# baiyang4/D-LSG-Video-Caption

Hardware: AMD Instinct MI355X
Metric: clips/sec (train step, 26x(2048+4096) feats) (higher is better)
Workload: dtype f32; 1 GPU; vocab 1000, dropout on, tf eps 0.952, batch 64/GPU; MSVD-shaped 26x(2048+4096) + 16x2048 regions; train step; batch_per_gpu=64, global_batch=64, parallelism=dp1, launch=hipGraph replay, gemm_arithmetic=fp32

## Files before the change

d-lsg-video-caption_amd/csrc/decstep.hip:

```cpp
#include "common.hpp"
#include "dlsg.h"

using namespace dlsg;

namespace {

constexpr int DT = 1024;
constexpr int MAXW = 2048;
constexpr int MAXP = 72;

template <int V> struct Vec;
template <> struct Vec<4> { using T = float4; };
template <> struct Vec<1> { using T = float; };
template <int V> __device__ __forceinline__ void vload(float (&r)[V], const float* p) {
    if constexpr (V == 4) { const float4 t = *reinterpret_cast<const float4*>(p); r[0] = t.x; r[1] = t.y; r[2] = t.z; r[3] = t.w; }
    else r[0] = *p;
}
template <int V> __device__ __forceinline__ void vstore(float* p, const float (&r)[V]) {
    if constexpr (V == 4) *reinterpret_cast<float4*>(p) = make_float4(r[0], r[1], r[2], r[3]);
    else *p = r[0];
}

__device__ __forceinline__ void block_sum2(float& a, float& b, float* red) {
    a = wave_sum(a); b = wave_sum(b);
    const int lane = threadIdx.x & 63, w = threadIdx.x >> 6;
    __syncthreads();
    if (lane == 0) { red[w] = a; red[16 + w] = b; }
    __syncthreads();
    float ra = 0.f, rb = 0.f;
#pragma unroll
    for (int i = 0; i < DT / 64; ++i) { ra += red[i]; rb += red[16 + i]; }
    a = ra; b = rb;
}

template <int V>
__device__ __forceinline__ void cell_row(int b, int N, const float* slabs, int nslab, int64_t slab_stride, const float* addend,
                                         int64_t ldadd, const float* b_ih, const float* b_hh, const float* c_prev, float* c_out,
                                         float* h_out, float* gates, float p, uint32_t site, uint64_t seed, float* gb, float* hb) {
    float cpv[MAXW / DT];
#pragma unroll
    for (int i = 0; i < MAXW / DT; ++i) {
        const int j = threadIdx.x + i * DT;
        cpv[i] = (c_prev && j < N) ? c_prev[(int64_t)b * N + j] : 0.f;
    }
    for (int col = threadIdx.x * V; col < 4 * N; col += DT * V) {
        float acc[V], t[4][V];
#pragma unroll
        for (int e = 0; e < V; ++e) acc[e] = 0.f;
        const float* sp = slabs + (int64_t)b * 4 * N + col;
        int k = 0;
        for (; k + 4 <= nslab; k += 4) {
#pragma unroll
            for (int u = 0; u < 4; ++u) vload<V>(t[u], sp + (k + u) * slab_stride);
#pragma unroll
// ... 2 lines not shown
                for (int e = 0; e < V; ++e) acc[e] += t[u][e];
        }
        if (k < nslab) {
            const int rem = nslab - k;
#pragma unroll
            for (int u = 0; u < 3; ++u)
                if (u < rem) vload<V>(t[u], sp + (k + u) * slab_stride);
#pragma unroll
            for (int u = 0; u < 3; ++u)
                if (u < rem)
#pragma unroll
                    for (int e = 0; e < V; ++e) acc[e] += t[u][e];
        }
        if (addend) { vload<V>(t[0], addend + (int64_t)b * ldadd + col);
#pragma unroll
            for (int e = 0; e < V; ++e) acc[e] += t[0][e]; }
        if (b_ih) { vload<V>(t[1], b_ih + col);
#pragma unroll
            for (int e = 0; e < V; ++e) acc[e] += t[1][e]; }
        if (b_hh) { vload<V>(t[2], b_hh + col);
#pragma unroll
            for (int e = 0; e < V; ++e) acc[e] += t[2][e]; }
        const bool is_g = (col / N) == 2;
#pragma unroll
        for (int e = 0; e < V; ++e) acc[e] = is_g ? tanhf(acc[e]) : sigmoidf_(acc[e]);
        vstore<V>(gates + (int64_t)b * 4 * N + col, acc);
        vstore<V>(gb + col, acc);
    }
    __syncthreads();
#pragma unroll
    for (int i = 0; i < MAXW / DT; ++i) {
        const int j = threadIdx.x + i * DT;
        if (j >= N) break;
        const float cp = cpv[i];
        const float c = gb[N + j] * cp + gb[j] * gb[2 * N + j];
        float h = gb[3 * N + j] * tanhf(c);
        c_out[(int64_t)b * N + j] = c;
        if (p > 0.f) h *= drop_scale(seed, site, (uint64_t)b * N + j, p);
        h_out[(int64_t)b * N + j] = h;
        hb[j] = h;
    }
    __syncthreads();
}

__device__ __forceinline__ void ln_stats(const float* v, int n, float eps, float* red, float& mean, float& rstd) {
    float s = 0.f;
    for (int j = threadIdx.x; j < n; j += DT) s += v[j];
    mean = block_sum(s, red) / n;
    float q = 0.f;
    for (int j = threadIdx.x; j < n; j += DT) { const float d = v[j] - mean; q += d * d; }
    rstd = rsqrtf(block_sum(q, red) / n + eps);
}

template <int V>
__global__ __launch_bounds__(DT) void dec_mid_fwd_kernel(const dlsg_dec_mid_args a) {
    __shared__ __attribute__((aligned(16))) float gb[4 * MAXW];
    __shared__ __attribute__((aligned(16))) float hb[MAXW];
    __shared__ __attribute__((aligned(16))) float qb[MAXW];
    __shared__ float sc[2 * MAXP], wt[2 * MAXP];
    __shared__ float red[32];
    const int b = blockIdx.x;
    const int bk = a.kv_div > 1 ? b / a.kv_div : b;
    const int Q = a.Q, H = a.H, P = a.P, ns = a.nstream;
    const int lane = threadIdx.x & 63, w = threadIdx.x >> 6;
    const uint64_t seed = a.seed + (a.seed_ptr ? *a.seed_ptr : 0ull);

    cell_row<V>(b, Q, a.slabs, a.nslab, a.slab_stride, a.addend, a.ldadd, a.b_ih, a.b_hh, a.c_prev, a.c, a.h, a.gates, 0.f, 0,
                seed, gb, hb);
    float mean, rstd;
    ln_stats(hb, Q, a.eps, red, mean, rstd);
    if (threadIdx.x == 0) { a.st_q[2 * b] = mean; a.st_q[2 * b + 1] = rstd; }
    for (int j = threadIdx.x; j < Q; j += DT) {
        float v = (hb[j] - mean) * rstd * a.lnq_g[j] + a.lnq_b[j];
        if (a.p_q > 0.f) v *= drop_scale(seed, a.site_q, (uint64_t)b * Q + j, a.p_q);
        a.qcur[(int64_t)b * Q + j] = v;
        qb[j] = v;
    }
    __syncthreads();
    for (int d = w; d < ns * P; d += DT / 64) {
        const int s = d / P, p = d % P;
        const float* kp = a.Kp[s] + ((int64_t)bk * P + p) * Q;
        float acc = 0.f;
#pragma unroll 4
        for (int j = lane * V; j < Q; j += 64 * V) {
            float kv[V];
            vload<V>(kv, kp + j);
#pragma unroll
            for (int e = 0; e < V; ++e) acc += kv[e] * qb[j + e];
        }
        acc = wave_sum(acc);
        if (lane == 0) sc[s * MAXP + p] = acc * a.scale;
    }
    __syncthreads();
    if (threadIdx.x < ns * P) {
        const int s = threadIdx.x / P, p = threadIdx.x % P;
        float m = -INFINITY;
        for (int i = 0; i < P; ++i) m = fmaxf(m, sc[s * MAXP + i]);
        float l = 0.f;
        for (int i = 0; i < P; ++i) l += __expf(sc[s * MAXP + i] - m);
        const float wv = __expf(sc[s * MAXP + p] - m) / l;
        wt[s * MAXP + p] = wv;
        a.alpha[(int64_t)b * ns * P + s * P + p] = wv;
    }
    __syncthreads();
    float* cb = gb;
    for (int it = threadIdx.x * V; it < ns * H; it += DT * V) {
        const int s = it / H, j = it % H;
        const float* vp = a.Vp[s] + (int64_t)bk * P * H + j;
        float acc[V], t[4][V];
#pragma unroll
        for (int e = 0; e < V; ++e) acc[e] = 0.f;
        int p = 0;
        for (; p + 4 <= P; p += 4) {
#pragma unroll
            for (int u = 0; u < 4; ++u) vload<V>(t[u], vp + (int64_t)(p + u) * H);
#pragma unroll
            for (int u = 0; u < 4; ++u)
#pragma unroll
                for (int e = 0; e < V; ++e) acc[e] += wt[s * MAXP + p + u] * t[u][e];
        }
        for (; p < P; ++p) {
            vload<V>(t[0], vp + (int64_t)p * H);
#pragma unroll
            for (int e = 0; e < V; ++e) acc[e] += wt[s * MAXP + p] * t[0][e];
        }
        vstore<V>(a.cpre[s] + (int64_t)b * H + j, acc);
#pragma unroll
        for (int e = 0; e < V; ++e) acc[e] = tanhf(acc[e]);
        vstore<V>(cb + s * MAXW + j, acc);
    }
    __syncthreads();
    float s0 = 0.f, s1 = 0.f;
    for (int j = threadIdx.x; j < H; j += DT) { s0 += cb[j]; if (ns > 1) s1 += cb[MAXW + j]; }
    block_sum2(s0, s1, red);
    const float m0 = s0 / H, m1 = s1 / H;
    float q0 = 0.f, q1 = 0.f;
    for (int j = threadIdx.x; j < H; j += DT) {
        const float d0 = cb[j] - m0; q0 += d0 * d0;
        if (ns > 1) { const float d1 = cb[MAXW + j] - m1; q1 += d1 * d1; }
    }
    block_sum2(q0, q1, red);
    const float r0 = rsqrtf(q0 / H + a.eps), r1 = rsqrtf(q1 / H + a.eps);
    if (threadIdx.x == 0) {
        a.st_c[0][2 * b] = m0; a.st_c[0][2 * b + 1] = r0;
        if (ns > 1) { a.st_c[1][2 * b] = m1; a.st_c[1][2 * b + 1] = r1; }
    }
    for (int it = threadIdx.x; it < ns * H; it += DT) {
        const int s = it / H, j = it % H;
        float v = (cb[s * MAXW + j] - (s ? m1 : m0)) * (s ? r1 : r0) * a.lnc_g[s][j] + a.lnc_b[s][j];
        if (a.p_att[s] > 0.f) v *= drop_scale(seed, a.site_att[s], (uint64_t)b * H + j, a.p_att[s]);
        a.ctx[s][(int64_t)b * H + j] = v;
    }
}

template <int V>
__global__ __launch_bounds__(DT) void dec_tail_fwd_kernel(const dlsg_dec_tail_args a) {
    __shared__ __attribute__((aligned(16))) float gb[4 * MAXW];
    __shared__ __attribute__((aligned(16))) float hb[MAXW];
    __shared__ float red[32];
    const int b = blockIdx.x;
    const int D = a.D;
    const uint64_t seed = a.seed + (a.seed_ptr ? *a.seed_ptr : 0ull);
    constexpr int ND = MAXW / DT;
    float lg[ND], lb[ND];
#pragma unroll
    for (int i = 0; i < ND; ++i) {
        const int j = threadIdx.x + i * DT;
        lg[i] = j < D ? a.ln_g[j] : 0.f; lb[i] = j < D ? a.ln_b[j] : 0.f;
    }
    cell_row<V>(b, D, a.slabs, a.nslab, a.slab_stride, nullptr, 0, a.b_ih, a.b_hh, a.c_prev, a.c, a.hd, a.gates, a.p, a.site,
                seed, gb, hb);
    float mean, rstd;
    ln_stats(hb, D, a.eps, red, mean, rstd);
    if (threadIdx.x == 0) { a.st_l[2 * b] = mean; a.st_l[2 * b + 1] = rstd; }
    const bool sample = a.s_coins != nullptr && a.s_coins[a.s_t] == 0;
    float dv[ND];
#pragma unroll
    for (int i = 0; i < ND; ++i) {
        const int j = threadIdx.x + i * DT;
        dv[i] = 0.f;
        if (j >= D) break;
        dv[i] = tanhf((hb[j] - mean) * rstd * lg[i] + lb[i]);
        a.dout[(int64_t)b * D + j] = dv[i];
    }
    if (!sample) return;
    __syncthreads();
#pragma unroll
    for (int i = 0; i < ND; ++i) {
        const int j = threadIdx.x + i * DT;
        if (j < D) hb[j] = dv[i];
    }
    __syncthreads();
    __shared__ int s_bi[DT / 64];
    __shared__ int64_t s_chosen;
    const int lane = threadIdx.x & 63, w = threadIdx.x >> 6;
    float best = -INFINITY;
    int bidx = 0x7fffffff;
    constexpr int CU4 = 4;
    for (int v0 = w * CU4; v0 < a.s_V; v0 += (DT / 64) * CU4) {
        float acc[CU4];
#pragma unroll
        for (int u = 0; u < CU4; ++u) {
            acc[u] = 0.f;
            const int v = min(v0 + u, a.s_V - 1);
            const float* wr = a.s_W + (int64_t)v * D;
            if (V == 4) {
                for (int j = 4 * lane; j < D; j += 256) {
                    const f32x4 x = *reinterpret_cast<const f32x4*>(hb + j);
                    const f32x4 y = *reinterpret_cast<const f32x4*>(wr + j);
                    acc[u] += x[0] * y[0] + x[1] * y[1] + x[2] * y[2] + x[3] * y[3];
                }
            } else {
                for (int j = lane; j < D; j += 64) acc[u] += hb[j] * wr[j];
            }
        }
#pragma unroll
        for (int u = 0; u < CU4; ++u) {
            const int v = v0 + u;
            float s_ = wave_sum(acc[u]);
            if (a.s_b) s_ += a.s_b[min(v, a.s_V - 1)];
            if (v < a.s_V && (s_ > best || (s_ == best && v < bidx))) { best = s_; bidx = v; }
        }
    }
    if (lane == 0) { red[w] = best; s_bi[w] = bidx; }
    __syncthreads();
    if (threadIdx.x == 0) {
        for (int k = 1; k < DT / 64; ++k)
            if (red[k] > best || (red[k] == best && s_bi[k] < bidx)) { best = red[k]; bidx = s_bi[k]; }
        if (bidx == 0x7fffffff) bidx = 0;
        s_chosen = bidx;
        a.s_ids[b] = bidx;
    }
    __syncthreads();
    const int64_t id = s_chosen;
    for (int j = threadIdx.x; j < a.s_Wd; j += DT) {
        float e = a.s_E[id * a.s_Wd + j];
        if (a.s_p > 0.f) e *= drop_scale(seed, a.s_site, (uint64_t)(a.s_row0 + b) * a.s_Wd + j, a.s_p);
        a.s_we[(int64_t)b * a.s_ldwe + j] = e;
    }
}


template <int N>
__device__ __forceinline__ void block_sumN(float (&v)[N], float* red) {
#pragma unroll
    for (int i = 0; i < N; ++i) v[i] = wave_sum(v[i]);
    const int lane = threadIdx.x & 63, w = threadIdx.x >> 6;
    __syncthreads();
    if (lane == 0)
#pragma unroll
        for (int i = 0; i < N; ++i) red[16 * i + w] = v[i];
    __syncthreads();
#pragma unroll
    for (int i = 0; i < N; ++i) {
        float r = 0.f;
#pragma unroll
        for (int k = 0; k < DT / 64; ++k) r += red[16 * i + k];
        v[i] = r;
    }
}

template <int V>
__global__ __launch_bounds__(DT) void dec_mid_bwd_kernel(const dlsg_dec_mid_bwd_args a) {
    __shared__ __attribute__((aligned(16))) float dxb[3 * MAXW];
    __shared__ __attribute__((aligned(16))) float dcp[2 * MAXW];
    __shared__ __attribute__((aligned(16))) float dqb[2 * MAXW];
    __shared__ float dwb[2 * MAXP], dsb[2 * MAXP], wb[2 * MAXP];
    __shared__ float red[64];
    constexpr int IC = 2 * MAXW / DT, IQ = MAXW / DT;
    const int b = blockIdx.x;
    const int Q = a.Q, H = a.H, D = a.D, P = a.P, ns = a.nstream;
    const int NX = ns * H + Q, WT = NX + D;
    const int lane = threadIdx.x & 63, w = threadIdx.x >> 6;
    const uint64_t seed = a.seed + (a.seed_ptr ? *a.seed_ptr : 0ull);

    float yv[IC], xq[IQ], rec[IQ];
#pragma unroll
    for (int i = 0; i < IC; ++i) {
        const int it = threadIdx.x + i * DT;
        yv[i] = 0.f;
        if (it < ns * H) { const int s = it / H, j = it % H; yv[i] = a.cpre[s][(int64_t)b * H + j]; }
    }
#pragma unroll
    for (int i = 0; i < IQ; ++i) {
        const int j = threadIdx.x + i * DT;
        xq[i] = 0.f; rec[i] = 0.f;
        if (j < Q) {
            xq[i] = a.qh[(int64_t)b * Q + j];
            if (a.rec_slabs) {
                const float* rp = a.rec_slabs + (int64_t)b * a.rec_ld + j;
                int k = 0;
                for (; k + 4 <= a.rec_nslab; k += 4) {
                    const float t0 = rp[(int64_t)k * a.rec_slab_stride], t1 = rp[(int64_t)(k + 1) * a.rec_slab_stride],
                                t2 = rp[(int64_t)(k + 2) * a.rec_slab_stride], t3 = rp[(int64_t)(k + 3) * a.rec_slab_stride];
                    rec[i] += t0; rec[i] += t1; rec[i] += t2; rec[i] += t3;
                }
                for (; k < a.rec_nslab; ++k) rec[i] += rp[(int64_t)k * a.rec_slab_stride];
            }
        }
    }
    if (threadIdx.x < ns * P) {
        const int s = threadIdx.x / P, p = threadIdx.x % P;
        wb[s * MAXP + p] = a.alpha[(int64_t)b * ns * P + threadIdx.x];
    }
    const int ncol = a.write_rec ? WT : NX;
    for (int col = threadIdx.x * V; col < ncol; col += DT * V) {
        float acc[V], t[4][V];
#pragma unroll
        for (int e = 0; e < V; ++e) acc[e] = 0.f;
        const float* sp = a.slabs + (int64_t)b * WT + col;
        int k = 0;
        for (; k + 4 <= a.nslab; k += 4) {
#pragma unroll
            for (int u = 0; u < 4; ++u) vload<V>(t[u], sp + (k + u) * a.slab_stride);
#pragma unroll
            for (int u = 0; u < 4; ++u)
#pragma unroll
                for (int e = 0; e < V; ++e) acc[e] += t[u][e];
        }
        if (k < a.nslab) {
            const int rem = a.nslab - k;
#pragma unroll
            for (int u = 0; u < 3; ++u)
// ... 83 lines not shown
#pragma unroll
                for (int e = 0; e < V; ++e) acc[e] += dsb[s * MAXP + p + u] * t[u][e];
        }
        for (; p < P; ++p) {
            vload<V>(t[0], kp + (int64_t)p * Q);
#pragma unroll
            for (int e = 0; e < V; ++e) acc[e] += dsb[s * MAXP + p] * t[0][e];
        }
        vstore<V>(dqb + s * MAXW + j, acc);
    }
    __syncthreads();
    float gq[IQ], xhq[IQ];
    float s2[2] = {0.f, 0.f};
    const float meanq = a.st_q[2 * b], rstdq = a.st_q[2 * b + 1];
#pragma unroll
    for (int i = 0; i < IQ; ++i) {
        const int j = threadIdx.x + i * DT;
        gq[i] = 0.f; xhq[i] = 0.f;
        if (j < Q) {
            float g = dxb[ns * H + j] + dqb[j];
            if (ns > 1) g += dqb[MAXW + j];
            if (a.p_q > 0.f) g *= drop_scale(seed, a.site_q, (uint64_t)b * Q + j, a.p_q);
            xhq[i] = (xq[i] - meanq) * rstdq;
            float* pq = a.part_q + (int64_t)b * 2 * Q;
            pq[j] = g * xhq[i];
            pq[Q + j] = g;
            gq[i] = g * a.lnq_g[j];
            s2[0] += gq[i]; s2[1] += gq[i] * xhq[i];
        }
    }
    block_sumN<2>(s2, red);
    const float m1 = s2[0] / Q, m2 = s2[1] / Q;
#pragma unroll
    for (int i = 0; i < IQ; ++i) {
        const int j = threadIdx.x + i * DT;
        if (j < Q) {
            const float dh = rstdq * (gq[i] - m1 - xhq[i] * m2) + rec[i];
            const float* gp = a.gates + (int64_t)b * 4 * Q;
            const float ig = gp[j], fg = gp[Q + j], gg = gp[2 * Q + j], og = gp[3 * Q + j];
            const float c = a.c[(int64_t)b * Q + j];
            const float cp = a.c_prev ? a.c_prev[(int64_t)b * Q + j] : 0.f;
            const float tc = tanhf(c);
            const float dc = dh * og * (1.f - tc * tc) + a.dc[(int64_t)b * Q + j];
            float* dgp = a.dgates + (int64_t)b * 4 * Q;
            dgp[j] = dc * gg * ig * (1.f - ig);
            dgp[Q + j] = dc * cp * fg * (1.f - fg);
            dgp[2 * Q + j] = dc * ig * (1.f - gg * gg);
            dgp[3 * Q + j] = dh * tc * og * (1.f - og);
            a.dc[(int64_t)b * Q + j] = dc * fg;
        }
    }
}

constexpr int CG_PC = 8;
template <int V>
__global__ __launch_bounds__(256) void decatt_cache_grads_kernel(const dlsg_decatt_cache_grads_args a) {
    const int b = blockIdx.x, s = blockIdx.y >> 1, kind = blockIdx.y & 1;
    const int N = kind ? a.Q : a.H, P = a.P, nsP = a.nstream * a.P;
    const float* coef = (kind ? a.ds : a.alpha) + (int64_t)b * nsP + s * P;
    const float* src = (kind ? a.qcur : a.dcpre[s]) + (int64_t)b * N;
    float* dst = (kind ? a.dKp[s] : a.dVp[s]) + (int64_t)b * P * N;
    for (int p0 = 0; p0 < P; p0 += CG_PC)
        for (int j = threadIdx.x * V; j < N; j += 256 * V) {
            float acc[CG_PC][V];
#pragma unroll
            for (int p = 0; p < CG_PC; ++p)
#pragma unroll
                for (int e = 0; e < V; ++e) acc[p][e] = 0.f;
#pragma unroll 2
            for (int t = 0; t < a.L; ++t) {
                float x[V];
                vload<V>(x, src + (int64_t)t * a.B * N + j);
                const float* cf = coef + (int64_t)t * a.B * nsP + p0;
#pragma unroll
                for (int p = 0; p < CG_PC; ++p) {
                    const float cv = (p0 + p < P) ? cf[p] : 0.f;
#pragma unroll
                    for (int e = 0; e < V; ++e) acc[p][e] += cv * x[e];
                }
            }
#pragma unroll
            for (int p = 0; p < CG_PC; ++p)
                if (p0 + p < P) vstore<V>(dst + (int64_t)(p0 + p) * N + j, acc[p]);
        }
}

bool vec_ok(const void* p) { return (reinterpret_cast<uintptr_t>(p) & 15) == 0; }

}

extern "C" int dlsg_dec_mid_fwd(const dlsg_dec_mid_args* a, void* stream) {
    if (!a || a->Q < 1 || a->Q > MAXW || a->H < 1 || a->H > MAXW || a->P < 1 || a->P > MAXP || a->nstream < 1 || a->nstream > 2)
        return DLSG_EINVAL;
    if (a->B == 0) return DLSG_OK;
    bool v4 = a->Q % 4 == 0 && a->H % 4 == 0 && a->slab_stride % 4 == 0 && a->ldadd % 4 == 0 && vec_ok(a->slabs) &&
              vec_ok(a->addend) && vec_ok(a->b_ih) && vec_ok(a->b_hh) && vec_ok(a->gates);
    for (int s = 0; s < a->nstream; ++s) v4 = v4 && vec_ok(a->Kp[s]) && vec_ok(a->Vp[s]) && vec_ok(a->cpre[s]);
    hipLaunchKernelGGL(v4 ? dec_mid_fwd_kernel<4> : dec_mid_fwd_kernel<1>, dim3(a->B), dim3(DT), 0,
                       reinterpret_cast<hipStream_t>(stream), *a);
    DLSG_CHECK_LAUNCH();
    return DLSG_OK;
}
extern "C" int dlsg_dec_tail_fwd(const dlsg_dec_tail_args* a, void* stream) {
    if (!a || a->D < 1 || a->D > MAXW) return DLSG_EINVAL;
    if (a->B == 0) return DLSG_OK;
    if (a->s_coins && (!a->s_W || !a->s_E || !a->s_ids || !a->s_we || a->s_V < 1 || a->s_Wd < 1)) return DLSG_EINVAL;
    const bool v4 = a->D % 4 == 0 && a->slab_stride % 4 == 0 && vec_ok(a->slabs) && vec_ok(a->b_ih) && vec_ok(a->b_hh) &&
                    vec_ok(a->gates) && (!a->s_coins || vec_ok(a->s_W));
    hipLaunchKernelGGL(v4 ? dec_tail_fwd_kernel<4> : dec_tail_fwd_kernel<1>, dim3(a->B), dim3(DT), 0,
                       reinterpret_cast<hipStream_t>(stream), *a);
    DLSG_CHECK_LAUNCH();
    return DLSG_OK;
}
extern "C" int dlsg_dec_mid_bwd(const dlsg_dec_mid_bwd_args* a, void* stream) {
    if (!a || a->Q < 1 || a->Q > MAXW || a->H < 1 || a->H > MAXW || a->D < 0 || a->P < 1 || a->P > MAXP || a->nstream < 1 ||
        a->nstream > 2)
        return DLSG_EINVAL;
    if (a->B == 0) return DLSG_OK;
    bool v4 = a->Q % 4 == 0 && a->H % 4 == 0 && a->D % 4 == 0 && a->slab_stride % 4 == 0 && vec_ok(a->slabs) && vec_ok(a->dlh_rec);
    for (int s = 0; s < a->nstream; ++s) v4 = v4 && vec_ok(a->Kp[s]) && vec_ok(a->Vp[s]);
    hipLaunchKernelGGL(v4 ? dec_mid_bwd_kernel<4> : dec_mid_bwd_kernel<1>, dim3(a->B), dim3(DT), 0,
                       reinterpret_cast<hipStream_t>(stream), *a);
    DLSG_CHECK_LAUNCH();
    return DLSG_OK;
}
extern "C" int dlsg_decatt_cache_grads(const dlsg_decatt_cache_grads_args* a, void* stream) {
    if (!a || a->L < 0 || a->P < 1 || a->nstream < 1 || a->nstream > 2) return DLSG_EINVAL;
    if (a->B == 0) return DLSG_OK;
    bool v4 = a->Q % 4 == 0 && a->H % 4 == 0 && vec_ok(a->qcur);
    for (int s = 0; s < a->nstream; ++s) v4 = v4 && vec_ok(a->dcpre[s]) && vec_ok(a->dKp[s]) && vec_ok(a->dVp[s]);
    hipLaunchKernelGGL(v4 ? decatt_cache_grads_kernel<4> : decatt_cache_grads_kernel<1>, dim3(a->B, 2 * a->nstream), dim3(256), 0,
                       reinterpret_cast<hipStream_t>(stream), *a);
    DLSG_CHECK_LAUNCH();
    return DLSG_OK;
}
```

d-lsg-video-caption_amd/csrc/gemm.hip:

```cpp
#include <cstdlib>
#include <mutex>

#include "common.hpp"
#include "dlsg.h"

namespace {

constexpr int NT = 256;

template <int ROWS, bool T, int BK>
struct TileGeom {
    static constexpr int NV = ROWS * BK / 4 / NT;
    static constexpr int LD = T ? (ROWS + 4) : (BK + 4);
    static constexpr int ELEMS = T ? BK * (ROWS + 4) : ROWS * (BK + 4);
    static constexpr int KQ = BK / 4;
};

template <int ROWS, bool T, int BK>
__device__ __forceinline__ void load_tile_fast(const float* __restrict__ base, int64_t ld, int row0, int k0, int rmax,
                                               f32x4 (&regs)[TileGeom<ROWS, T, BK>::NV]) {
    constexpr int NV = TileGeom<ROWS, T, BK>::NV;
#pragma unroll
    for (int j = 0; j < NV; ++j) {
        const int f = threadIdx.x + NT * j;
        const float* ptr;
        if (!T) {
            const int gr = min(row0 + f / (BK / 4), rmax - 1);
            ptr = base + (int64_t)gr * ld + k0 + 4 * (f % (BK / 4));
        } else {
            ptr = base + (int64_t)(k0 + f / (ROWS / 4)) * ld + row0 + 4 * (f % (ROWS / 4));
        }
        regs[j] = *reinterpret_cast<const f32x4*>(ptr);
    }
}
template <int ROWS, bool T, int BK>
__device__ __forceinline__ void load_tile_slow(const float* __restrict__ base, int64_t ld, int row0, int k0, int rmax,
                                               int K, f32x4 (&regs)[TileGeom<ROWS, T, BK>::NV]) {
    constexpr int NV = TileGeom<ROWS, T, BK>::NV;
#pragma unroll
    for (int j = 0; j < NV; ++j) {
        const int f = threadIdx.x + NT * j;
        int gr, gk, nvalid;
        const float* ptr;
        if (!T) {
            const int row = f / (BK / 4), kq = f % (BK / 4);
            gr = row0 + row;
            gk = k0 + 4 * kq;
            ptr = base + (int64_t)gr * ld + gk;
            nvalid = (gr < rmax) ? min(max(K - gk, 0), 4) : 0;
        } else {
            const int k = f / (ROWS / 4), mq = f % (ROWS / 4);
            gk = k0 + k;
            gr = row0 + 4 * mq;
            ptr = base + (int64_t)gk * ld + gr;
            nvalid = (gk < K) ? min(max(rmax - gr, 0), 4) : 0;
        }
        f32x4 v = {0.f, 0.f, 0.f, 0.f};
// ... 300 lines not shown
#pragma unroll
        for (int mi = 0; mi < MI; ++mi) {
            const float* ap = ldsA + (r + 32 * mi) * SLD + 32 * w + 16 * h;
#pragma unroll
            for (int q = 0; q < 4; ++q) {
                const f32x4 v = *reinterpret_cast<const f32x4*>(ap + 4 * q);
                fa[mi][4 * q] = v[0]; fa[mi][4 * q + 1] = v[1]; fa[mi][4 * q + 2] = v[2]; fa[mi][4 * q + 3] = v[3];
            }
        }
        if (!BT) {
            const float* bp = ldsB + r * SLD + 32 * w + 16 * h;
#pragma unroll
            for (int q = 0; q < 4; ++q) {
                const f32x4 v = *reinterpret_cast<const f32x4*>(bp + 4 * q);
                bcur[4 * q] = v[0]; bcur[4 * q + 1] = v[1]; bcur[4 * q + 2] = v[2]; bcur[4 * q + 3] = v[3];
            }
        }
#pragma unroll
        for (int s2 = 0; s2 < 16; ++s2)
#pragma unroll
            for (int mi = 0; mi < MI; ++mi) acc[mi] = __builtin_amdgcn_mfma_f32_32x32x2f32(fa[mi][s2], bcur[s2], acc[mi], 0, 0, 0);
        __syncthreads();
    }
    float* red = lds;
#pragma unroll
    for (int mi = 0; mi < MI; ++mi)
#pragma unroll
        for (int e = 0; e < 16; ++e) red[((w * MI + mi) * 16 + e) * 64 + lane] = acc[mi][e];
    __syncthreads();
    const float* biasp = grp.bias ? grp.bias : p.bias;
    const bool accum = p.flags & DLSG_GEMM_ACCUM, use_bias = (p.flags & DLSG_GEMM_BIAS) && biasp != nullptr;
    const bool do_tanh = p.flags & DLSG_GEMM_TANH;
    if (col < N) {
        const float bv = use_bias ? biasp[col] : 0.f;
#pragma unroll
        for (int mi = 0; mi < MI; ++mi)
#pragma unroll
            for (int ee = 0; ee < 4; ++ee) {
                const int e = 4 * w + ee;
                const int row = 32 * mi + (e & 3) + 8 * (e >> 2) + 4 * h;
                if (row >= M) continue;
                float v = 0.f;
#pragma unroll
                for (int ww = 0; ww < 4; ++ww) v += red[((ww * MI + mi) * 16 + e) * 64 + lane];
                v = p.alpha * v + bv;
                float* cp = C + (int64_t)row * (grp.ldc ? grp.ldc : (int64_t)p.ldc) + col;
                if (accum) v += *cp;
                if (do_tanh) v = tanhf(v);
                *cp = v;
            }
    }
}

constexpr int S2_STAGE = 16;
constexpr int S2_DEPTH = 3;
constexpr int S2_B_BYTES = 32 * 64;
constexpr int s2_lds_bytes(int MI, int NJ) { return 4 * S2_DEPTH * (MI + NJ) * S2_B_BYTES; }

template <int VB>
__device__ __forceinline__ void s2_glds(const char* src, char* dst) {
#if defined(__HIP_DEVICE_COMPILE__)
    typedef __attribute__((address_space(3))) void* lp_t;
    typedef const __attribute__((address_space(1))) void* gp_t;
    __builtin_amdgcn_global_load_lds((gp_t)src, (lp_t)dst, 16, 0, 0);
#endif
}

template <int MI, int NJ, bool BT = false>
__global__ __launch_bounds__(NT) void skinny2_nt_kernel(const KArgs p) {
    constexpr int S2_A_BYTES = MI * S2_B_BYTES;
    constexpr int SLOT = S2_A_BYTES + NJ * S2_B_BYTES;
    extern __shared__ __attribute__((aligned(16))) char s2_lds[];
    if (p.skip_if && *p.skip_if) return;
    const int z = blockIdx.y;
    const int gi = z % p.ngroups, bi = z / p.ngroups;
    const dlsg_gemm_group grp = p.g[gi];
    const float* A = grp.A + (int64_t)bi * p.bsa;
    const float* B = grp.B + (int64_t)bi * p.bsb;
    float* C = grp.C + (int64_t)bi * p.bsc;
    const int K = grp.K, M = p.M, N = grp.N > 0 ? grp.N : p.N;
    const int n0 = blockIdx.x * 32 * NJ;
    if (n0 >= N) return;
    const int lane = threadIdx.x & 63, w = threadIdx.x >> 6;
    const int r = lane & 31, h = lane >> 5;
    char* ring = s2_lds + w * (S2_DEPTH * SLOT);

    const int rho = lane >> 2, sig = lane & 3;
    const float* srcA[2 * MI];
    const float* srcB[2 * NJ];
#pragma unroll
    for (int pc = 0; pc < 2 * MI; ++pc) {
        const int R = 16 * pc + rho;
        srcA[pc] = A + (int64_t)min(R, M - 1) * grp.lda + 4 * (sig ^ ((R >> 2) & 3));
    }
#pragma unroll
    for (int pc = 0; pc < 2 * NJ; ++pc) {
        if (!BT) {
            const int R = 16 * pc + rho;
            srcB[pc] = B + (int64_t)min(n0 + R, N - 1) * grp.ldb + 4 * (sig ^ ((R >> 2) & 3));
        } else {
            const int kr = 8 * (pc & 1) + (lane >> 3), c = n0 + 32 * (pc >> 1) + 4 * (lane & 7);
            srcB[pc] = B + (int64_t)kr * grp.ldb + min(c, N - 4);
        }
    }
    const int nst = (K + S2_STAGE - 1) / S2_STAGE;
    const int mine = (nst - w + 3) / 4;
    auto issue = [&](int i) {
        const int k0 = (4 * i + w) * S2_STAGE;
        char* slot = ring + (i % S2_DEPTH) * SLOT;
        const int koff = (k0 + S2_STAGE <= K) ? k0 : (K - S2_STAGE);
#pragma unroll
        for (int pc = 0; pc < 2 * MI; ++pc) s2_glds<16>(reinterpret_cast<const char*>(srcA[pc] + koff), slot + pc * 1024);
#pragma unroll
        for (int pc = 0; pc < 2 * NJ; ++pc)
            s2_glds<16>(reinterpret_cast<const char*>(BT ? srcB[pc] + (int64_t)koff * grp.ldb : srcB[pc] + koff), slot + S2_A_BYTES + pc * 1024);
    };

    f32x16 acc[MI][NJ];
#pragma unroll
    for (int i = 0; i < MI; ++i)
#pragma unroll
        for (int nj = 0; nj < NJ; ++nj)
#pragma unroll
            for (int e = 0; e < 16; ++e) acc[i][nj][e] = 0.f;

    int offA[MI][2], offB[NJ][2];
#pragma unroll
    for (int q = 0; q < 2; ++q) {
        const int ks = 2 * q + h;
#pragma unroll
        for (int mi = 0; mi < MI; ++mi) {
            const int R = 32 * mi + r;
            offA[mi][q] = (R >> 4) * 1024 + (R & 15) * 64 + ((ks ^ ((R >> 2) & 3)) * 16);
        }
#pragma unroll
        for (int nj = 0; nj < NJ; ++nj) {
            const int R = 32 * nj + r;
            offB[nj][q] = BT ? S2_A_BYTES + nj * 2048 + (4 * ks) * 128 + r * 4
                             : S2_A_BYTES + (R >> 4) * 1024 + (R & 15) * 64 + ((ks ^ ((R >> 2) & 3)) * 16);
        }
    }
    constexpr int PCS = 2 * MI + 2 * NJ;

    if (mine > 0) issue(0);
    if (mine > 1) issue(1);
    for (int i = 0; i < mine; ++i) {
        if (i + 2 < mine) {
            issue(i + 2);
            asm volatile("s_waitcnt vmcnt(%0)" ::"n"(2 * PCS) : "memory");
        } else if (i + 1 < mine) {
            asm volatile("s_waitcnt vmcnt(%0)" ::"n"(PCS) : "memory");
        } else {
            asm volatile("s_waitcnt vmcnt(0)" ::: "memory");
        }
        const char* slot = ring + (i % S2_DEPTH) * SLOT;
        const int k0 = (4 * i + w) * S2_STAGE;
        const bool part = k0 + S2_STAGE > K;
        const int kbase = part ? K - S2_STAGE : k0;
        f32x4 fa[MI][2], fb[NJ][2];
#pragma unroll
        for (int q = 0; q < 2; ++q) {
#pragma unroll
            for (int mi = 0; mi < MI; ++mi) fa[mi][q] = *reinterpret_cast<const f32x4*>(slot + offA[mi][q]);
#pragma unroll
            for (int nj = 0; nj < NJ; ++nj) {
                if (!BT) fb[nj][q] = *reinterpret_cast<const f32x4*>(slot + offB[nj][q]);
                else {
#pragma unroll
                    for (int j = 0; j < 4; ++j) fb[nj][q][j] = *reinterpret_cast<const float*>(slot + offB[nj][q] + j * 128);
                }
            }
        }
        if (part) {
#pragma unroll
            for (int q = 0; q < 2; ++q)
#pragma unroll
                for (int j = 0; j < 4; ++j) {
                    const int k = kbase + 4 * (2 * q + h) + j;
                    const bool keep = k >= k0 && k < K;
#pragma unroll
                    for (int mi = 0; mi < MI; ++mi) fa[mi][q][j] = keep ? fa[mi][q][j] : 0.f;
#pragma unroll
                    for (int nj = 0; nj < NJ; ++nj) fb[nj][q][j] = keep ? fb[nj][q][j] : 0.f;
                }
        }
#pragma unroll
        for (int q = 0; q < 2; ++q)
#pragma unroll
            for (int j = 0; j < 4; ++j)
#pragma unroll
                for (int nj = 0; nj < NJ; ++nj)
#pragma unroll
                    for (int mi = 0; mi < MI; ++mi)
                        acc[mi][nj] = __builtin_amdgcn_mfma_f32_32x32x2f32(fa[mi][q][j], fb[nj][q][j], acc[mi][nj], 0, 0, 0);
    }
    __syncthreads();
    float* red = reinterpret_cast<float*>(s2_lds);
#pragma unroll
    for (int mi = 0; mi < MI; ++mi)
#pragma unroll
        for (int nj = 0; nj < NJ; ++nj)
#pragma unroll
            for (int e = 0; e < 16; ++e) red[(((w * MI + mi) * NJ + nj) * 16 + e) * 64 + lane] = acc[mi][nj][e];
    __syncthreads();
    const float* biasp = grp.bias ? grp.bias : p.bias;
    const bool accum = p.flags & DLSG_GEMM_ACCUM, use_bias = (p.flags & DLSG_GEMM_BIAS) && biasp != nullptr;
    const bool do_tanh = p.flags & DLSG_GEMM_TANH;
#pragma unroll
    for (int nj = 0; nj < NJ; ++nj) {
        const int col = n0 + 32 * nj + r;
        if (col >= N) continue;
        const float bv = use_bias ? biasp[col] : 0.f;
#pragma unroll
        for (int mi = 0; mi < MI; ++mi)
#pragma unroll
            for (int ee = 0; ee < 4; ++ee) {
                const int e = 4 * w + ee;
                const int row = 32 * mi + (e & 3) + 8 * (e >> 2) + 4 * h;
                if (row >= M) continue;
                float v = 0.f;
#pragma unroll
                for (int ww = 0; ww < 4; ++ww) v += red[(((ww * MI + mi) * NJ + nj) * 16 + e) * 64 + lane];
                v = p.alpha * v + bv;
                float* cp = C + (int64_t)row * (grp.ldc ? grp.ldc : (int64_t)p.ldc) + col;
                if (accum) v += *cp;
                if (do_tanh) v = tanhf(v);
                *cp = v;
            }
    }
}

template <int MI>
int launch_skinny_mi(const dlsg_gemm_args* a, const KArgs& k, hipStream_t st) {
    dim3 grid((a->N + 31) / 32, a->ngroups * a->nbatch, 1), block(NT, 1, 1);
    static std::once_flag once;
    std::call_once(once, [] {
        (void)hipFuncSetAttribute(reinterpret_cast<const void*>(&skinny2_nt_kernel<MI, 1>), hipFuncAttributeMaxDynamicSharedMemorySize,
                                  s2_lds_bytes(MI, 1));
        (void)hipFuncSetAttribute(reinterpret_cast<const void*>(&skinny2_nt_kernel<MI, 2>), hipFuncAttributeMaxDynamicSharedMemorySize,
                                  s2_lds_bytes(MI, 2));
        (void)hipFuncSetAttribute(reinterpret_cast<const void*>(&skinny2_nt_kernel<MI, 1, true>), hipFuncAttributeMaxDynamicSharedMemorySize,
                                  s2_lds_bytes(MI, 1));
        (void)hipFuncSetAttribute(reinterpret_cast<const void*>(&skinny2_nt_kernel<MI, 2, true>), hipFuncAttributeMaxDynamicSharedMemorySize,
                                  s2_lds_bytes(MI, 2));
        (void)hipFuncSetAttribute(reinterpret_cast<const void*>(&skinny_kernel<false, MI>), hipFuncAttributeMaxDynamicSharedMemorySize,
                                  skinny_lds_bytes(MI));
        (void)hipFuncSetAttribute(reinterpret_cast<const void*>(&skinny_kernel<true, MI>), hipFuncAttributeMaxDynamicSharedMemorySize,
                                  skinny_lds_bytes(MI));
    });
    if (a->mode == 0) {
        bool ok = a->nbatch == 1;
        for (int i = 0; i < a->ngroups && ok; ++i) {
            const dlsg_gemm_group& g = a->g[i];
            ok = (g.K % 4 == 0) && g.K >= S2_STAGE && (g.lda % 4 == 0) && (g.ldb % 4 == 0) &&
                 ((reinterpret_cast<uintptr_t>(g.A) & 15) == 0) && ((reinterpret_cast<uintptr_t>(g.B) & 15) == 0);
        }
        if (ok) {
            const int wg64 = ((a->N + 63) / 64) * a->ngroups * a->nbatch;
            if (wg64 >= 224) {
                dim3 grid2((a->N + 63) / 64, a->ngroups * a->nbatch, 1);
                hipLaunchKernelGGL((skinny2_nt_kernel<MI, 2>), grid2, block, s2_lds_bytes(MI, 2), st, k);
            } else {
                hipLaunchKernelGGL((skinny2_nt_kernel<MI, 1>), grid, block, s2_lds_bytes(MI, 1), st, k);
            }
        } else {
            hipLaunchKernelGGL((skinny_kernel<false, MI>), grid, block, skinny_lds_bytes(MI), st, k);
        }
    } else {
        bool ok = a->nbatch == 1;
        for (int i = 0; i < a->ngroups && ok; ++i) {
            const dlsg_gemm_group& g = a->g[i];
            const int gn = g.N > 0 ? g.N : a->N;
            ok = (g.K % 4 == 0) && g.K >= S2_STAGE && (g.lda % 4 == 0) && (g.ldb % 4 == 0) && (gn % 4 == 0) && gn >= 4 &&
                 ((reinterpret_cast<uintptr_t>(g.A) & 15) == 0) && ((reinterpret_cast<uintptr_t>(g.B) & 15) == 0);
        }
        if (ok) {
            bool same_n = true;
            for (int i = 0; i < a->ngroups; ++i) same_n = same_n && (a->g[i].N == 0 || a->g[i].N == a->N);
            const int wg64 = ((a->N + 63) / 64) * a->ngroups * a->nbatch;
            if (wg64 >= 224 && same_n) {
                dim3 grid2((a->N + 63) / 64, a->ngroups * a->nbatch, 1);
                hipLaunchKernelGGL((skinny2_nt_kernel<MI, 2, true>), grid2, block, s2_lds_bytes(MI, 2), st, k);
            } else {
                hipLaunchKernelGGL((skinny2_nt_kernel<MI, 1, true>), grid, block, s2_lds_bytes(MI, 1), st, k);
            }
        } else {
            hipLaunchKernelGGL((skinny_kernel<true, MI>), grid, block, skinny_lds_bytes(MI), st, k);
        }
    }
    DLSG_CHECK_LAUNCH();
    return DLSG_OK;
}

int launch_skinny(const dlsg_gemm_args* a, hipStream_t st) {
    KArgs k;
    k.M = a->M; k.N = a->N; k.ldc = a->ldc; k.ngroups = a->ngroups; k.flags = a->flags;
    k.bsa = a->bsa; k.bsb = a->bsb; k.bsc = a->bsc; k.alpha = a->alpha; k.bias = a->bias; k.skip_if = a->skip_if;
    for (int i = 0; i < a->ngroups; ++i) k.g[i] = a->g[i];
    return a->M <= 64 ? launch_skinny_mi<2>(a, k, st) : launch_skinny_mi<4>(a, k, st);
}

template <int BM, int BN, int BK>
int launch(const dlsg_gemm_args* a, hipStream_t st) {
    KArgs k;
    k.M = a->M; k.N = a->N; k.ldc = a->ldc; k.ngroups = a->ngroups; k.flags = a->flags;
    k.bsa = a->bsa; k.bsb = a->bsb; k.bsc = a->bsc; k.alpha = a->alpha; k.bias = a->bias; k.skip_if = a->skip_if;
    for (int i = 0; i < a->ngroups; ++i) k.g[i] = a->g[i];
    const int tiles = ((a->M + BM - 1) / BM) * ((a->N + BN - 1) / BN);
    dim3 grid(tiles, a->ngroups * a->nbatch, 1), block(NT, 1, 1);
    switch (a->mode) {
        case 0:
            if constexpr (BM == 128) hipLaunchKernelGGL((gemm_kernel_w3<BM, BN, false, false, BK>), grid, block, 0, st, k);
            else hipLaunchKernelGGL((gemm_kernel<BM, BN, false, false, BK>), grid, block, 0, st, k);
            break;
        case 1:
            if constexpr (BM == 128) hipLaunchKernelGGL((gemm_kernel_w3<BM, BN, false, true, BK>), grid, block, 0, st, k);
            else hipLaunchKernelGGL((gemm_kernel<BM, BN, false, true, BK>), grid, block, 0, st, k);
            break;
        case 2:
            if constexpr (BM == 128) hipLaunchKernelGGL((gemm_kernel_w3<BM, BN, true, true, BK>), grid, block, 0, st, k);
            else hipLaunchKernelGGL((gemm_kernel<BM, BN, true, true, BK>), grid, block, 0, st, k);
            break;
        default: return DLSG_EINVAL;
    }
    DLSG_CHECK_LAUNCH();
    return DLSG_OK;
}
// ... 124 lines not shown
```

d-lsg-video-caption_amd/csrc/rowops.hip:

```cpp
#include "common.hpp"
#include "dlsg.h"

using namespace dlsg;

namespace {

constexpr int LN_THREADS = 256;
constexpr int LN_MAXPT = 8;

struct RowLnPack { dlsg_rowln_args s[DLSG_ROWLN_MAXMULTI]; };
struct RowLnBwdPack { dlsg_rowln_bwd_args s[DLSG_ROWLN_MAXMULTI]; };

__global__ __launch_bounds__(LN_THREADS) void rowln_fwd_kernel(const RowLnPack pk) {
    __shared__ float red[16];
    const dlsg_rowln_args& a = pk.s[blockIdx.y];
    const int n = a.n;
    const uint64_t seed = a.seed + (a.seed_ptr ? *a.seed_ptr : 0ull);
    float gam[LN_MAXPT], bet[LN_MAXPT];
#pragma unroll
    for (int i = 0; i < LN_MAXPT; ++i) {
        const int j = threadIdx.x + i * LN_THREADS;
        gam[i] = j < n ? a.gamma[j] : 0.f; bet[i] = j < n ? a.beta[j] : 0.f;
    }
    for (int row = blockIdx.x; row < a.rows; row += gridDim.x) {
// ... 310 lines not shown
struct PwFwdSet { dlsg_lstm_pw_args a[2]; };
struct PwBwdSet { dlsg_lstm_pw_bwd_args a[2]; };

__global__ __launch_bounds__(256) void lstm_pw_fwd_kernel(const PwFwdSet set) {
    const dlsg_lstm_pw_args& a = set.a[blockIdx.z];
    const int j = blockIdx.x * blockDim.x + threadIdx.x;
    const int b = blockIdx.y;
    if (j >= a.H) return;
    const int H = a.H;
    float pre[4] = {0.f, 0.f, 0.f, 0.f};
    const float* sp = a.slabs + (int64_t)b * 4 * H + j;
    int k = 0;
    for (; k + 2 <= a.nslab; k += 2) {
        float t[2][4];
#pragma unroll
        for (int u = 0; u < 2; ++u)
#pragma unroll
            for (int g = 0; g < 4; ++g) t[u][g] = sp[(k + u) * a.slab_stride + g * H];
#pragma unroll
        for (int u = 0; u < 2; ++u)
#pragma unroll
            for (int g = 0; g < 4; ++g) pre[g] += t[u][g];
    }
    if (k < a.nslab) {
#pragma unroll
        for (int g = 0; g < 4; ++g) pre[g] += sp[k * a.slab_stride + g * H];
    }
#pragma unroll
    for (int g = 0; g < 4; ++g) {
        const int col = g * H + j;
        float s = pre[g];
        if (a.addend) s += a.addend[(int64_t)b * a.ldadd + col];
        if (a.b_ih) s += a.b_ih[col];
        if (a.b_hh) s += a.b_hh[col];
        pre[g] = s;
    }
    const float ig = sigmoidf_(pre[0]), fg = sigmoidf_(pre[1]), gg = tanhf(pre[2]), og = sigmoidf_(pre[3]);
    const float cp = a.c_prev ? a.c_prev[(int64_t)b * a.ldcp + j] : 0.f;
    const float c = fg * cp + ig * gg;
    const float h = og * tanhf(c);
    a.c[(int64_t)b * a.ldc_ + j] = c;
    if (a.h) a.h[(int64_t)b * a.ldh + j] = h;
    if (a.h2) {
        float h2 = h;
        if (a.p > 0.f) h2 *= drop_scale(a.seed + (a.seed_ptr ? *a.seed_ptr : 0ull), a.site, (uint64_t)b * H + j, a.p);
        a.h2[(int64_t)b * a.ldh2 + j] = h2;
    }
    if (a.gates) {
        float* gp = a.gates + (int64_t)b * a.ldg;
        gp[j] = ig; gp[H + j] = fg; gp[2 * H + j] = gg; gp[3 * H + j] = og;
    }
}

__global__ __launch_bounds__(256) void lstm_pw_bwd_kernel(const PwBwdSet set) {
    const dlsg_lstm_pw_bwd_args& a = set.a[blockIdx.z];
    const int j = blockIdx.x * blockDim.x + threadIdx.x;
    const int b = blockIdx.y;
    if (j >= a.H) return;
    const int H = a.H;
    const float* gp = a.gates + (int64_t)b * a.ldg;
    const float ig = gp[j], fg = gp[H + j], gg = gp[2 * H + j], og = gp[3 * H + j];
    const float c = a.c[(int64_t)b * a.ldc_ + j];
    const float cp = a.c_prev ? a.c_prev[(int64_t)b * a.ldcp + j] : 0.f;
    float dh = a.dh ? a.dh[(int64_t)b * a.lddh + j] : 0.f;
    if (a.dh2 || a.dh3 || a.dh4) {
        float d2 = a.dh2 ? a.dh2[(int64_t)b * a.lddh2 + j] : 0.f;
        if (a.dh3) d2 += a.dh3[(int64_t)b * a.lddh3 + j];
        if (a.dh4) {
            const int ns4 = a.dh4_nslab > 1 ? a.dh4_nslab : 1;
            const float* hp = a.dh4 + (int64_t)b * a.lddh4 + j;
            int k = 0;
            for (; k + 4 <= ns4; k += 4) {
                const float t0 = hp[(int64_t)k * a.dh4_slab_stride], t1 = hp[(int64_t)(k + 1) * a.dh4_slab_stride],
                            t2 = hp[(int64_t)(k + 2) * a.dh4_slab_stride], t3 = hp[(int64_t)(k + 3) * a.dh4_slab_stride];
                d2 += t0; d2 += t1; d2 += t2; d2 += t3;
            }
            for (; k < ns4; ++k) d2 += hp[(int64_t)k * a.dh4_slab_stride];
        }
        if (a.p > 0.f) d2 *= drop_scale(a.seed + (a.seed_ptr ? *a.seed_ptr : 0ull), a.site, (uint64_t)b * H + j, a.p);
        dh += d2;
    }
    const float tc = tanhf(c);
    float dc = dh * og * (1.f - tc * tc);
    if (a.dc_next) dc += a.dc_next[(int64_t)b * a.lddcn + j];
    float* dgp = a.dgates + (int64_t)b * a.lddg;
    dgp[j] = dc * gg * ig * (1.f - ig);
    dgp[H + j] = dc * cp * fg * (1.f - fg);
    dgp[2 * H + j] = dc * ig * (1.f - gg * gg);
    dgp[3 * H + j] = dh * tc * og * (1.f - og);
    if (a.dc_prev) a.dc_prev[(int64_t)b * a.lddcp + j] = dc * fg;
}

__global__ void mean_rows_fwd_kernel(const float* __restrict__ x, float* __restrict__ out, int64_t ldo, int P, int H) {
    const int b = blockIdx.y;
    const int h = blockIdx.x * blockDim.x + threadIdx.x;
    if (h >= H) return;
    float s = 0.f;
    for (int p = 0; p < P; ++p) s += x[((int64_t)b * P + p) * H + h];
    out[(int64_t)b * ldo + h] = s / P;
}
__global__ void mean_rows_bwd_kernel(const float* __restrict__ dout, int64_t lddo, float* __restrict__ dx, int P, int H,
                                     int accum) {
    const int b = blockIdx.y;
    const int h = blockIdx.x * blockDim.x + threadIdx.x;
    if (h >= H) return;
    const float g = dout[(int64_t)b * lddo + h] / P;
    for (int p = 0; p < P; ++p) {
        float* d = dx + ((int64_t)b * P + p) * H + h;
        *d = accum ? *d + g : g;
    }
}

__global__ void embed_fwd_kernel(const float* __restrict__ E, const int64_t* __restrict__ ids, float* __restrict__ out,
                                 int64_t ldo, int W, float p, uint64_t seed, uint32_t site, int64_t row0, const uint64_t* seed_ptr) {
    if (seed_ptr) seed += *seed_ptr;
    const int r = blockIdx.x;
    const int64_t id = ids[r];
    for (int j = threadIdx.x; j < W; j += blockDim.x) {
        float v = E[id * W + j];
        if (p > 0.f) v *= drop_scale(seed, site, (uint64_t)(row0 + r) * W + j, p);
// ... 592 lines not shown
        if (d[i].out_b && !d[i].dup && (d[i].split < 0 || d[i].split > d[i].n)) return DLSG_EINVAL;
        pk.d[i] = d[i];
        maxn = d[i].n > maxn ? d[i].n : maxn;
    }
    hipLaunchKernelGGL(colsum_multi_kernel, dim3((maxn + 63) / 64, count), dim3(1024), 0, ST(stream), pk);
    DLSG_CHECK_LAUNCH();
    return DLSG_OK;
}
extern "C" int64_t dlsg_colsum_ws_floats(int rows, int n) {
    const int chunks = colsum_chunks(rows);
    return chunks > 1 ? (int64_t)chunks * n : 0;
}
extern "C" int dlsg_colsum(const float* part, int64_t ld, int rows, int n, float* out, int accum, float* ws, void* stream) {
    return colsum_launch(part, ld, rows, n, out, nullptr, n, 0, accum, ws, stream);
}
extern "C" int dlsg_colsum2(const float* part, int64_t ld, int rows, int n, float* out_a, float* out_b, int split, int dup,
                            int accum, float* ws, void* stream) {
    if (!out_b || (!dup && (split < 0 || split > n))) return DLSG_EINVAL;
    return colsum_launch(part, ld, rows, n, out_a, out_b, dup ? n : split, dup ? 1 : 0, accum, ws, stream);
}
extern "C" int dlsg_softmax_fwd(const float* x, const float* mask, float* y, int64_t outer, int n, int inner, void* stream) {
    const int64_t lines = outer * inner;
    if (lines == 0) return DLSG_OK;
    hipLaunchKernelGGL(softmax_fwd_kernel, dim3((unsigned)((lines + 3) / 4)), dim3(256), 0, ST(stream), x, mask, y, outer, n,
                       inner);
    DLSG_CHECK_LAUNCH();
    return DLSG_OK;
}
extern "C" int dlsg_softmax_bwd(const float* y, const float* dy, float* dx, int64_t outer, int n, int inner, void* stream) {
    const int64_t lines = outer * inner;
    if (lines == 0) return DLSG_OK;
    hipLaunchKernelGGL(softmax_bwd_kernel, dim3((unsigned)((lines + 3) / 4)), dim3(256), 0, ST(stream), y, dy, dx, outer, n,
                       inner);
    DLSG_CHECK_LAUNCH();
    return DLSG_OK;
}
extern "C" int dlsg_lstm_pw_fwd_n(const dlsg_lstm_pw_args* a, int count, void* stream) {
    if (!a || count < 1 || count > 2 || a[0].H < 1) return DLSG_EINVAL;
    if (count == 2 && (a[1].H != a[0].H || a[1].B != a[0].B)) return DLSG_EINVAL;
    if (a[0].B == 0) return DLSG_OK;
    PwFwdSet set;
    for (int i = 0; i < 2; ++i) set.a[i] = a[i < count ? i : 0];
    hipLaunchKernelGGL(lstm_pw_fwd_kernel, dim3((a[0].H + 255) / 256, a[0].B, count), dim3(256), 0, ST(stream), set);
    DLSG_CHECK_LAUNCH();
    return DLSG_OK;
}
extern "C" int dlsg_lstm_pw_fwd(const dlsg_lstm_pw_args* a, void* stream) { return dlsg_lstm_pw_fwd_n(a, 1, stream); }
extern "C" int dlsg_lstm_pw_bwd_n(const dlsg_lstm_pw_bwd_args* a, int count, void* stream) {
    if (!a || count < 1 || count > 2 || a[0].H < 1) return DLSG_EINVAL;
    if (count == 2 && (a[1].H != a[0].H || a[1].B != a[0].B)) return DLSG_EINVAL;
    if (a[0].B == 0) return DLSG_OK;
    PwBwdSet set;
    for (int i = 0; i < 2; ++i) set.a[i] = a[i < count ? i : 0];
    hipLaunchKernelGGL(lstm_pw_bwd_kernel, dim3((a[0].H + 255) / 256, a[0].B, count), dim3(256), 0, ST(stream), set);
    DLSG_CHECK_LAUNCH();
    return DLSG_OK;
}
extern "C" int dlsg_lstm_pw_bwd(const dlsg_lstm_pw_bwd_args* a, void* stream) { return dlsg_lstm_pw_bwd_n(a, 1, stream); }
extern "C" int dlsg_mean_rows_fwd(const float* x, float* out, int64_t ldo, int B, int P, int H, void* stream) {
    if (B == 0) return DLSG_OK;
    hipLaunchKernelGGL(mean_rows_fwd_kernel, dim3((H + 255) / 256, B), dim3(256), 0, ST(stream), x, out, ldo, P, H);
    DLSG_CHECK_LAUNCH();
    return DLSG_OK;
}
extern "C" int dlsg_mean_rows_bwd(const float* dout, int64_t lddo, float* dx, int B, int P, int H, int accum, void* stream) {
    if (B == 0) return DLSG_OK;
    hipLaunchKernelGGL(mean_rows_bwd_kernel, dim3((H + 255) / 256, B), dim3(256), 0, ST(stream), dout, lddo, dx, P, H, accum);
    DLSG_CHECK_LAUNCH();
    return DLSG_OK;
}
extern "C" int dlsg_embed_fwd(const float* E, const int64_t* ids, float* out, int64_t ldo, int rows, int W, float p,
                              uint64_t seed, uint32_t site, int64_t row0, const uint64_t* seed_ptr, void* stream) {
    if (rows == 0) return DLSG_OK;
    hipLaunchKernelGGL(embed_fwd_kernel, dim3(rows), dim3(128), 0, ST(stream), E, ids, out, ldo, W, p, seed, site, row0, seed_ptr);
    DLSG_CHECK_LAUNCH();
    return DLSG_OK;
}
extern "C" int dlsg_embed_bwd(const float* dout, int64_t lddo, const int64_t* ids, float* dE, int rows, int W, float p,
                              uint64_t seed, uint32_t site, int64_t row0, const uint64_t* seed_ptr, void* stream) {
    if (rows == 0) return DLSG_OK;
    const int threads = W >= 1024 ? 1024 : (W + 63) / 64 * 64;
    hipLaunchKernelGGL(embed_bwd_kernel, dim3(rows), dim3(threads), 0, ST(stream), dout, lddo, ids, dE, rows, W, p, seed, site, row0,
                       seed_ptr);
    DLSG_CHECK_LAUNCH();
    return DLSG_OK;
}
extern "C" int dlsg_select_embed(const float* logits, int64_t ld, int V, const int64_t* captions, int L, int t,
                                 const int32_t* coins, const float* E, int64_t* ids_out, float* out, int64_t ldo, int rows, int W,
                                 float p, uint64_t seed, uint32_t site, int64_t row0, const uint64_t* seed_ptr, int prefilled,
                                 void* stream) {
    if (rows == 0) return DLSG_OK;
    hipLaunchKernelGGL(select_embed_kernel, dim3(rows), dim3(256), 0, ST(stream), logits, ld, V, captions, L, t, coins, E, ids_out,
                       out, ldo, W, p, seed, site, row0, seed_ptr, prefilled);
    DLSG_CHECK_LAUNCH();
    return DLSG_OK;
}
extern "C" int dlsg_sample_embed(const float* logits, int64_t ld, int V, float temperature, const float* E, int64_t* ids_out, float* out,
                                 int64_t ldo, int W, float* logp, int64_t* lens, int t, int64_t end_id, int rows, float p, uint64_t seed,
                                 uint32_t site_word, uint32_t site_sample, int64_t row0, const uint64_t* seed_ptr, void* stream) {
    if (rows == 0) return DLSG_OK;
    if (V < 1 || W < 0 || !(temperature >= 0.f)) return DLSG_EINVAL;
    hipLaunchKernelGGL(sample_embed_kernel, dim3(rows), dim3(256), 0, ST(stream), logits, ld, V, temperature, E, ids_out, out, ldo, W,
                       logp, lens, t, end_id, p, seed, site_word, site_sample, row0, seed_ptr);
    DLSG_CHECK_LAUNCH();
    return DLSG_OK;
}
extern "C" int dlsg_argmax(const float* logits, int64_t ld, int64_t* ids, int rows, int V, void* stream) {
    if (rows == 0) return DLSG_OK;
    hipLaunchKernelGGL(argmax_kernel, dim3(rows), dim3(256), 0, ST(stream), logits, ld, ids, V);
    DLSG_CHECK_LAUNCH();
    return DLSG_OK;
// ... 98 lines not shown
```

d-lsg-video-caption_amd/dlsg_amd/engine.py:

```python
import math

import torch

from .hip import GEMM_NT, GEMM_NN, GEMM_TN, F_ACCUM, F_TANH, F_BF16X3, F_FORCE128

V_SK = 7

SITE_PSL_OBJ, SITE_PSL_MOT, SITE_LSTM, SITE_PE, SITE_SA, SITE_WORD, SITE_QUERY, SITE_ATT1, SITE_ATT2, SITE_LANG = range(1, 11)
STEP_SITE = 64
SITE_SAMPLE = 11


def _empty(ref, *shape, dtype=torch.float32):
    return torch.empty(*shape, dtype=dtype, device=ref.device)


def _zeros(ref, *shape, dtype=torch.float32):
    return torch.zeros(*shape, dtype=dtype, device=ref.device)


def _ksplit_bounds(K, nsplit, align=32):
    nsplit = max(1, min(nsplit, K // 512))
    step = ((K + nsplit - 1) // nsplit + align - 1) // align * align
    out, k = [], 0
# ... 70 lines not shown
            ops.gemm(GEMM_TN, [(dy, x, gout)], flags=_accum_flag(ops, gout))
    if deep and getattr(ops, 'stream_k', False) and all(ops.gemm(GEMM_TN, [it], flags=F_ACCUM, plan_only=True) == V_SK for it in deep):
        parts = {0: [], F_ACCUM: []}
        for it in deep:
            parts[_accum_flag(ops, it[2])].append(it)
        for fl, part in parts.items():
            for i0 in range(0, len(part), 16):
                ops.gemm(GEMM_TN, part[i0:i0 + 16], flags=fl)
        return
    by_shape = {}
    for it in deep:
        by_shape.setdefault((it[0].shape, it[1].shape), []).append(it)
    ks = DEEP_TN_CHUNKS
    per_launch = max(1, min(2, 16 // ks))
    for grp in by_shape.values():
        for i0 in range(0, len(grp), per_launch):
            part = grp[i0:i0 + per_launch]
            rows = part[0][0].shape[0]
            step = ((rows + ks - 1) // ks + 31) // 32 * 32
            bounds = [(k, min(rows, k + step)) for k in range(0, rows, step)]
            assert len(bounds) * len(part) <= 16
            slabs = [_empty(ref, len(bounds), gout.shape[0], gout.shape[1]) for _, _, gout in part]
            ops.gemm(GEMM_TN, [(dy[k0:k1], x[k0:k1], sl[i]) for (dy, x, _), sl in zip(part, slabs)
                               for i, (k0, k1) in enumerate(bounds)])
            for (_, _, gout), sl in zip(part, slabs):
                ops.slab_reduce(sl, gout, flags=_accum_always(ops, gout))


def _accum_flag_peek(ops, gout):
    seen = getattr(ops, 'grad_written', None)
    if seen is None or (gout.data_ptr(), tuple(gout.shape), tuple(gout.stride())) in seen:
        return F_ACCUM
    return 0


def gemm_nn_multi(ops, dy, Ws, out, ref):
    M, Nn = dy.shape
    widths = [W.shape[1] for W in Ws]
    tot = sum(widths)
    assert out.shape[1] == tot
    ns = _nsplit_for(M, tot, 1)
    ns = max(1, min(ns, 16 // len(Ws)))
    bounds = _bwd_bounds(Nn, M, ns)
    slabs = _empty(ref, len(bounds), M, tot)
    groups, c0 = [], 0
    for W, wd in zip(Ws, widths):
        for i, (k0, k1) in enumerate(bounds):
            groups.append((dy[:, k0:k1], W[k0:k1, :], slabs[i][:, c0:c0 + wd]))
        c0 += wd
    ops.gemm(GEMM_NN, groups)
    ops.slab_reduce(slabs, out)


def gemm_nn_multi_slabs(ops, dy, Ws, width, ref):
    M, Nn = dy.shape
    widths = [W.shape[1] for W in Ws]
    tot = sum(widths)
    assert tot <= width
    ns = _nsplit_for(M, tot, 1)
    ns = max(1, min(ns, 16 // len(Ws)))
    bounds = _bwd_bounds(Nn, M, ns)
    if M <= SKINNY_M and len(set(widths)) > 1:
        wmin = min(widths)
        if all(wd % wmin == 0 for wd in widths) and (tot // wmin) * len(bounds) <= 16:
            Ws = [W[:, c:c + wmin] for W, wd in zip(Ws, widths) for c in range(0, wd, wmin)]
            widths = [wmin] * len(Ws)
    slabs = _empty(ref, len(bounds), M, width)
    groups, c0 = [], 0
    for W, wd in zip(Ws, widths):
        for i, (k0, k1) in enumerate(bounds):
            groups.append((dy[:, k0:k1], W[k0:k1, :], slabs[i][:, c0:c0 + wd]))
        c0 += wd
    ops.gemm(GEMM_NN, groups)
    return slabs


def tn_grouped(ops, items, defer=None):
    if defer is not None:
        defer.extend(items)
        return
    by_m = {}
    for dy, x, gout in items:
        by_m.setdefault((dy.shape[1], dy.shape[0]), []).append((dy, x, gout))
    for grp in by_m.values():
        waves, seen = [[]], [set()]
        for it in grp:
            key = (it[2].data_ptr(), tuple(it[2].shape))
            for w_, sn in zip(waves, seen):
                if key not in sn and len(w_) < 16:
                    w_.append(it); sn.add(key)
                    break
            else:
                waves.append([it]); seen.append({key})
        for w_ in waves:
            first = [it for it in w_ if _accum_flag_peek(ops, it[2]) == 0]
            rest = [it for it in w_ if _accum_flag_peek(ops, it[2]) != 0]
            for it in first:
                _accum_flag(ops, it[2])
            if first:
                ops.gemm(GEMM_TN, first, flags=0)
            if rest:
                ops.gemm(GEMM_TN, rest, flags=F_ACCUM)


def gemm_bucketed(ops, mode, groups, flags=0):
    by_m = {}
    for g in groups:
        by_m.setdefault(g[2].shape[-2], []).append(g)
    for grp in by_m.values():
        for i in range(0, len(grp), 16):
            ops.gemm(mode, grp[i:i + 16], flags=flags)


def lin(ops, x, W, out, bias=None, tanh=False, accum=False, skip_if=None):
    ops.gemm(GEMM_NT, [(x, W, out)], flags=(F_TANH if tanh else 0) | (F_ACCUM if accum else 0), bias=bias, skip_if=skip_if)


class Grads(object):

    def __init__(self, named_params, arena, offsets):
        self.arena, self.offsets = arena, offsets
        self.views = {}
        for name, p in named_params:
            o = offsets[name]
            self.views[name] = arena[o:o + p.numel()].view(p.shape)
# ... 558 lines not shown


class DecPlan(object):

    def __init__(self, dec, n_global):
        self.H, self.W = dec.visual_hidden_size, dec.word_size
        self.Q, self.D = dec.query_hidden_size, dec.decode_hidden_size
        self.G = n_global
        self.ns = 2 if dec.multi_modal else 1
        self.q_lang = (0, self.D)
        self.q_glob = (self.D, self.D + self.G)
        self.q_word = (self.D + self.G, self.D + self.G + self.W)
        self.l_ctx = [(i * self.H, (i + 1) * self.H) for i in range(self.ns)]
        self.l_q = (self.ns * self.H, self.ns * self.H + self.Q)


def _att_modules(dec):
    return [dec.context_att] + ([dec.context_att_2] if dec.multi_modal else [])


def dec_prepare(ops, dec, mems, sv, training, seed):
    s = sv['dec'] = {}
    gsrc = sv['dec_gsrc']
    ref = mems[0]
    B = ref.shape[0]
    H = dec.visual_hidden_size
    plan = DecPlan(dec, H * len(gsrc))
    Q = plan.Q
    if sv.get('step_feats') is not None:
        gfeat = sv['step_feats']
        assert gfeat.shape == (B, plan.G), (tuple(gfeat.shape), (B, plan.G))
    else:
        gfeat = _empty(ref, B, plan.G)
        for i, g in enumerate(gsrc):
            ops.mean_rows_fwd(g, gfeat[:, i * H:(i + 1) * H])
    Wq = dec.query_lstm.weight_ih
    gq = _empty(ref, B, 4 * Q)
    lin(ops, gfeat, Wq[:, plan.q_glob[0]:plan.q_glob[1]], gq)
    atts = _att_modules(dec)
    m2s = [mem.reshape(mem.shape[0] * mem.shape[1], H) for mem in mems]
    Kc = [_empty(ref, m2.shape[0], H) for m2 in m2s]
    Vc = [_empty(ref, m2.shape[0], H) for m2 in m2s]
    kps = [_empty(ref, m2.shape[0], Q) for m2 in m2s]
    vps = [_empty(ref, m2.shape[0], H) for m2 in m2s]
    gemm_bucketed(ops, GEMM_NT, [g for att, m2, K, V in zip(atts, m2s, Kc, Vc) for g in ((m2, att.K.weight, K), (m2, att.V.weight, V))])
    gemm_bucketed(ops, GEMM_NN, [(K, att.Q.weight, kp) for att, K, kp in zip(atts, Kc, kps)])
    gemm_bucketed(ops, GEMM_NT, [(V, att.output_layer[0].weight, vp) for att, V, vp in zip(atts, Vc, vps)])
    Kp = [kp.view(mem.shape[0], mem.shape[1], Q) for kp, mem in zip(kps, mems)]
    Vp = [vp.view(mem.shape[0], mem.shape[1], H) for vp, mem in zip(vps, mems)]
    s.update(plan=plan, gfeat=gfeat, gq=gq, K=Kc, V=Vc, Kp=Kp, Vp=Vp, mems=mems)
    return s


def dec_step(ops, dec, s, t, ref, training, seed, B, word_dropout=True, sample=None):
    plan = s['plan']
    H, Q, D = plan.H, plan.Q, plan.D
    ql, ll = dec.query_lstm, dec.lang_lstm
    pd = dec.p_drop if training else 0.0
    site = STEP_SITE * (t + 1)
    segs = [(s['WE'][t], ql.weight_ih[:, plan.q_word[0]:plan.q_word[1]])]
    if t > 0 or s.get('warm', False):
        segs += [(s['LHP'][t], ql.weight_ih[:, plan.q_lang[0]:plan.q_lang[1]]), (s['QH'][t], ql.weight_hh)]
    slabs = seg_gemm_nt(ops, segs, B, 4 * Q, ref)
    ns = plan.ns
    lnq = dec.query_lstm_layernorm
    atts = _att_modules(dec)
    ops.dec_mid_fwd(slabs, s['gq'], ql.bias_ih, ql.bias_hh, s['QC'][t], s['QC'][t + 1], s['QH'][t + 1], s['GQ'][t],
                    (lnq.weight, lnq.bias), s['QCUR'][t], s['ST_Q'][t], pd, site + SITE_QUERY, s['Kp'], s['Vp'],
                    [(a.output_layer[2].weight, a.output_layer[2].bias) for a in atts],
                    [s['CPRE'][i][t] for i in range(ns)], [s['CTX'][i][t] for i in range(ns)],
                    [s['ST_C'][i][t] for i in range(ns)], s['ALPHA'][t],
                    [a.dropout if training else 0.0 for a in atts], [site + SITE_ATT1 + i for i in range(ns)],
                    1.0 / math.sqrt(H), seed=seed, **({'kv_div': s['kv_div']} if s.get('kv_div', 1) > 1 else {}))
    segs = [(s['CTX'][i][t], ll.weight_ih[:, plan.l_ctx[i][0]:plan.l_ctx[i][1]]) for i in range(ns)]
    segs.append((s['QCUR'][t], ll.weight_ih[:, plan.l_q[0]:plan.l_q[1]]))
    if t > 0 or s.get('warm', False):
        segs.append((s['LHP'][t], ll.weight_hh))
    slabs = seg_gemm_nt(ops, segs, B, 4 * D, ref)
    lnl = dec.lang_lstm_layernorm
    ops.dec_tail_fwd(slabs, ll.bias_ih, ll.bias_hh, s['LC'][t], s['LC'][t + 1], s['LHP'][t + 1], s['GL'][t],
                     (lnl.weight, lnl.bias), s['DOUT'][t], s['ST_L'][t], pd, site + SITE_LANG, seed=seed,
                     **({'sample': sample} if sample is not None else {}))


def plan_D(s):
    return s['plan'].D


def dec_logits(ops, dec, s, t0, t1, skip_if=None):
    plan = s['plan']
    D = plan.D
    B = s['LHP'].shape[1]
    V = dec.vocab_size
    n = (t1 - t0) * B
    lin(ops, s['DOUT'][t0:t1].view(n, D), dec.word_restore.weight, s['LOGITS'][t0:t1].view(n, V), dec.word_restore.bias,
        skip_if=skip_if)


def dec_alloc(dec, s, ref, B, L):
    plan = s['plan']
    H, W, Q, D, ns = plan.H, plan.W, plan.Q, plan.D, plan.ns
    V = dec.vocab_size
    P = s['Kp'][0].shape[1]
    zst = _zeros(ref, (L + 1) * B * (2 * D + 2 * Q))
    o = 0
    for key, wd in (('LHP', D), ('QH', Q), ('QC', Q), ('LC', D)):
        s[key] = zst[o:o + (L + 1) * B * wd].view(L + 1, B, wd)
        o += (L + 1) * B * wd
    s['WE'] = _empty(ref, L + 1, B, W)
    s['IDS'] = _zeros(ref, L + 1, B, dtype=torch.int64)
    s['QCUR'] = _empty(ref, L, B, Q)
    s['ST_Q'] = _empty(ref, L, B, 2)
    s['CPRE'] = [_empty(ref, L, B, H) for _ in range(ns)]
    s['CTX'] = [_empty(ref, L, B, H) for _ in range(ns)]
    s['ST_C'] = [_empty(ref, L, B, 2) for _ in range(ns)]
    s['GQ'] = _empty(ref, L, B, 4 * Q)
    s['GL'] = _empty(ref, L, B, 4 * D)
    s['ALPHA'] = _empty(ref, L, B, ns * P)
    s['DOUT'] = _empty(ref, L, B, D)
    s['ST_L'] = _empty(ref, L, B, 2)
    s['LOGITS'] = _empty(ref, L, B, V)


def dec_fwd(ops, dec, mems, sv, captions, L, coins, training, seed, dev_coins=None):
    s = dec_prepare(ops, dec, mems, sv, training, seed)
    ref = mems[0]
    B = ref.shape[0]
    dec_alloc(dec, s, ref, B, L)
    E = dec.word_embed.weight
    pw = dec.p_drop if training else 0.0
    ids = s['IDS']
    ids[0].fill_(dec.vocab('<start>'))
    s['pw'] = pw
    if dev_coins is not None:
        ops.embed_fwd(E, ids[0], s['WE'][0], p=pw, seed=seed, site=SITE_WORD, row0=0)
        pre = captions is not None and L > 1
        if pre:
            ids[1:L].copy_(captions[:, :L - 1].t())
            ops.embed_fwd(E, ids[1:L].reshape(-1), s['WE'][1:L].view((L - 1) * B, -1), p=pw, seed=seed, site=SITE_WORD, row0=B)
        fused_sample = pre and getattr(ops, 'dec_tail_sample_supported', None) is not None and \
            ops.dec_tail_sample_supported(dec.vocab_size, plan_D(s))
        for t in range(L):
            if fused_sample and t + 1 < L:
                dec_step(ops, dec, s, t, ref, training, seed, B,
                         sample=dict(coins=dev_coins, t=t, W=dec.word_restore.weight, b=dec.word_restore.bias, E=E, ids_out=ids[t + 1],
                                     we_out=s['WE'][t + 1], p=pw, site=SITE_WORD, row0=(t + 1) * B))
                continue
            dec_step(ops, dec, s, t, ref, training, seed, B)
            if t + 1 < L:
                dec_logits(ops, dec, s, t, t + 1, skip_if=dev_coins[t:t + 1])
                ops.select_embed(s['LOGITS'][t], captions, t, dev_coins, E, ids[t + 1], s['WE'][t + 1], p=pw, seed=seed,
                                 site=SITE_WORD, row0=(t + 1) * B, prefilled=pre)
        dec_logits(ops, dec, s, 0, L)
        return s
    if captions is not None:
        tf_steps = [i for i in range(L) if coins[i]]
        for i in tf_steps:
            ids[i + 1].copy_(captions[:, i])
    ops.embed_fwd(E, ids.view(-1), s['WE'].view((L + 1) * B, -1), p=pw, seed=seed, site=SITE_WORD)
    for t in range(L):
        dec_step(ops, dec, s, t, ref, training, seed, B)
        if not coins[t]:
            dec_logits(ops, dec, s, t, t + 1)
            ops.argmax(s['LOGITS'][t], ids[t + 1])
            ops.embed_fwd(E, ids[t + 1], s['WE'][t + 1], p=pw, seed=seed, site=SITE_WORD, row0=(t + 1) * B)
    if any(coins[t] for t in range(L)):
        dec_logits(ops, dec, s, 0, L)
    return s


def dec_sample(ops, dec, mems, sv, L, training, seed, temperature):
    s = dec_prepare(ops, dec, mems, sv, training, seed)
    ref = mems[0]
    B = ref.shape[0]
    dec_alloc(dec, s, ref, B, L)
    E = dec.word_embed.weight
    pw = dec.p_drop if training else 0.0
    ids = s['IDS']
    ids[0].fill_(dec.vocab('<start>'))
    s['pw'] = pw
    s['LOGP'] = _empty(ref, L, B)
    s['LENS'] = torch.full((B,), L, dtype=torch.int64, device=ref.device)
    end = dec.vocab('<end>')
    ops.embed_fwd(E, ids[0], s['WE'][0], p=pw, seed=seed, site=SITE_WORD, row0=0)
    for t in range(L):
        dec_step(ops, dec, s, t, ref, training, seed, B)
        dec_logits(ops, dec, s, t, t + 1)
        ops.sample_embed(s['LOGITS'][t], E, ids[t + 1], s['WE'][t + 1], s['LOGP'][t], s['LENS'], t, end, temperature=temperature,
                         p=pw, seed=seed, site=SITE_WORD, site_sample=SITE_SAMPLE, row0=(t + 1) * B)
    return s


def dec_bwd(ops, dec, sv, G, dlogits_tm, seed, training, dalpha_tm=None):
    s = sv['dec']
    plan = s['plan']
    H, W, Q, D, ns = plan.H, plan.W, plan.Q, plan.D, plan.ns
    L, B, V = dlogits_tm.shape
    ref = dlogits_tm
    ql, ll = dec.query_lstm, dec.lang_lstm
    pd = dec.p_drop if training else 0.0
    n = L * B
    dl2 = dlogits_tm.view(n, V)
    tn_grouped(ops, [(dl2, s['DOUT'].view(n, D), G['decoder.word_restore.weight'])], sv.get('tn_defer'))
    ops.colsum(dl2, G['decoder.word_restore.bias'], accum=True)
    ddout = _empty(ref, n, D)
    k32 = V // 32 * 32
    if V - k32 and k32 >= 4096 and getattr(ops, 'stream_k', False):
        ops.gemm(GEMM_NN, [(dl2[:, :k32], dec.word_restore.weight[:k32], ddout)])
        ops.gemm(GEMM_NN, [(dl2[:, k32:], dec.word_restore.weight[k32:], ddout)], flags=F_ACCUM)
    else:
        ops.gemm(GEMM_NN, [(dl2, dec.word_restore.weight, ddout)])
    lnl = dec.lang_lstm_layernorm
    nb = ops.rowln_bwd_nblk(n)
    part = _empty(ref, nb, 2, D)
    dLHo = _empty(ref, L, B, D)
    ops.rowln_bwd(ddout, s['LHP'][1:].view(n, D), lnl.weight, lnl.bias, dLHo.view(n, D), stats=s['ST_L'].view(n, 2),
                  post_tanh=1, dgb_part=part)
    ln_grads(ops, part, G, 'decoder.lang_lstm_layernorm', D)

    dGQ = _empty(ref, L, B, 4 * Q)
    dGL = _empty(ref, L, B, 4 * D)
    dQC = _zeros(ref, B, Q)
    dLC = _zeros(ref, B, D)
    dLHrec = _empty(ref, B, D)
    P = s['Kp'][0].shape[1]
    dCPRE = [_empty(ref, L, B, H) for _ in range(ns)]
    dS = _empty(ref, L, B, ns * P)
    atts = _att_modules(dec)
    part_q = _empty(ref, L, B, 2, Q)
    part_c = [_empty(ref, L, B, 2, H) for _ in range(ns)]
    lnq = dec.query_lstm_layernorm
    lnc_g = [att.output_layer[2].weight for att in atts]
    p_att = [att.dropout if training else 0.0 for att in atts]
    scale = 1.0 / math.sqrt(H)
    Wl_in = ll.weight_ih
    Wq_rec = [ql.weight_hh, ql.weight_ih[:, plan.q_lang[0]:plan.q_lang[1]]]
    wx = ns * H + Q + D
    ql_slabs = None
    for t in range(L - 1, -1, -1):
        site = STEP_SITE * (t + 1)
        rec = t < L - 1
        ops.lstm_pw_bwd(s['GL'][t], s['LC'][t + 1], dGL[t], B, D, c_prev=s['LC'][t], dh2=dLHo[t],
                        dh3=dLHrec if rec else None, dh4=ql_slabs[:, :, Q:] if rec else None, dc_next=dLC, dc_prev=dLC,
                        p=pd, site=site + SITE_LANG, seed=seed)
        xl_slabs = gemm_nn_multi_slabs(ops, dGL[t], [Wl_in, ll.weight_hh] if t > 0 else [Wl_in], wx, ref)
        ops.dec_mid_bwd(xl_slabs, dLHrec if t > 0 else None, [s['CPRE'][i][t] for i in range(ns)],
                        [s['ST_C'][i][t] for i in range(ns)], lnc_g, [part_c[i][t] for i in range(ns)],
                        [dCPRE[i][t] for i in range(ns)], p_att, [site + SITE_ATT1 + i for i in range(ns)], s['Kp'], s['Vp'],
                        s['ALPHA'][t], dalpha_tm[t] if dalpha_tm is not None else None, dS[t], s['QH'][t + 1], s['ST_Q'][t],
                        lnq.weight, part_q[t], pd, site + SITE_QUERY, ql_slabs[:, :, :Q] if rec else None, s['GQ'][t],
                        s['QC'][t + 1], s['QC'][t], dQC, dGQ[t], scale, seed=seed)
        if t > 0:
            ql_slabs = gemm_nn_multi_slabs(ops, dGQ[t], Wq_rec, Q + D, ref)
    dKp = [torch.empty_like(k) for k in s['Kp']]
    dVp = [torch.empty_like(v) for v in s['Vp']]
    ops.decatt_cache_grads(s['ALPHA'], dS, s['QCUR'], dCPRE, dKp, dVp)
    ln_grads(ops, part_q.view(L * B, 2, Q), G, 'decoder.query_lstm_layernorm', Q)
    att_names = ['decoder.context_att', 'decoder.context_att_2']
    for i in range(ns):
        ln_grads(ops, part_c[i].view(L * B, 2, H), G, att_names[i] + '.output_layer.2', H)
    dgq2, dgl2 = dGQ.view(n, 4 * Q), dGL.view(n, 4 * D)
    Gq_ih, Gl_ih = G['decoder.query_lstm.weight_ih'], G['decoder.lang_lstm.weight_ih']
    dgq_sum = _empty(ref, B, 4 * Q)
    ops.slab_reduce(dGQ, dgq_sum)
    lhp, qh = s['LHP'][:L].view(n, D), s['QH'][:L].view(n, Q)
    tn_grouped(ops, [(dgq2, lhp, Gq_ih[:, plan.q_lang[0]:plan.q_lang[1]]),
                     (dgq2, s['WE'][:L].view(n, W), Gq_ih[:, plan.q_word[0]:plan.q_word[1]]),
                     (dgq2, qh, G['decoder.query_lstm.weight_hh'])] +
               [(dgl2, s['CTX'][i].view(n, H), Gl_ih[:, plan.l_ctx[i][0]:plan.l_ctx[i][1]]) for i in range(ns)] +
               [(dgl2, s['QCUR'].view(n, Q), Gl_ih[:, plan.l_q[0]:plan.l_q[1]]),
                (dgl2, lhp, G['decoder.lang_lstm.weight_hh'])], sv.get('tn_defer'))
    gq_glob = Gq_ih[:, plan.q_glob[0]:plan.q_glob[1]]
    ops.gemm(GEMM_TN, [(dgq_sum, s['gfeat'], gq_glob)], flags=_accum_always(ops, gq_glob))
    ops.colsum2(dgq2, G['decoder.query_lstm.bias_ih'], G['decoder.query_lstm.bias_hh'], accum=True)
    ops.colsum2(dgl2, G['decoder.lang_lstm.bias_ih'], G['decoder.lang_lstm.bias_hh'], accum=True)
    dWE = _empty(ref, n, W)
    Wword = ql.weight_ih[:, plan.q_word[0]:plan.q_word[1]]
    if n >= 512 and 4 * Q >= 2048:
        kb = [(k, min(4 * Q, k + 1024)) for k in range(0, 4 * Q, 1024)]
        sl = _empty(ref, len(kb), n, W)
        ops.gemm(GEMM_NN, [(dgq2[:, k0:k1], Wword[k0:k1], sl[i]) for i, (k0, k1) in enumerate(kb)])
        ops.slab_reduce(sl, dWE)
    else:
        ops.gemm(GEMM_NN, [(dgq2, Wword, dWE)])
    ops.embed_bwd(dWE, s['IDS'][:L].view(-1), G['decoder.word_embed.weight'], p=s['pw'], seed=seed, site=SITE_WORD)
    dgfeat = _empty(ref, B, plan.G)
    gemm_nn_split(ops, dgq_sum, ql.weight_ih[:, plan.q_glob[0]:plan.q_glob[1]], dgfeat, ref)
    m2s = [mem.reshape(mem.shape[0] * mem.shape[1], H) for mem in s['mems']]
    dkps = [dKp[i].view(m2s[i].shape[0], Q) for i in range(ns)]
    dvps = [dVp[i].view(m2s[i].shape[0], H) for i in range(ns)]
    dKs = [_empty(ref, m2.shape[0], H) for m2 in m2s]
    dVs = [_empty(ref, m2.shape[0], H) for m2 in m2s]
    dms = [_empty(ref, m2.shape[0], H) for m2 in m2s]
    R = range(ns)
    tn_grouped(ops, [g for i in R for g in ((s['K'][i], dkps[i], G[att_names[i] + '.Q.weight']),
                                            (dvps[i], s['V'][i], G[att_names[i] + '.output_layer.0.weight']))], sv.get('tn_defer'))
    gemm_bucketed(ops, GEMM_NT, [(dkps[i], atts[i].Q.weight, dKs[i]) for i in R])
    gemm_bucketed(ops, GEMM_NN, [(dvps[i], atts[i].output_layer[0].weight, dVs[i]) for i in R])
    tn_grouped(ops, [g for i in R for g in ((dKs[i], m2s[i], G[att_names[i] + '.K.weight']),
                                            (dVs[i], m2s[i], G[att_names[i] + '.V.weight']))], sv.get('tn_defer'))
    gemm_bucketed(ops, GEMM_NN, [(dKs[i], atts[i].K.weight, dms[i]) for i in R])
    gemm_bucketed(ops, GEMM_NN, [(dVs[i], atts[i].V.weight, dms[i]) for i in R], flags=F_ACCUM)
    dmems = [dms[i].view(s['mems'][i].shape) for i in R]
    return dmems, dgfeat
# ... 1 lines not shown
```

d-lsg-video-caption_amd/dlsg_amd/hip.py:

```python
import ctypes as C
import os

import torch

from . import abi

_HERE = os.path.dirname(os.path.abspath(__file__))
LIB_PATH = os.path.join(_HERE, 'libdlsg_hip.so')

_D = abi.defines
ABI_VERSION = _D['DLSG_ABI_VERSION']
MAXG = _D['DLSG_GEMM_MAXG']
GEMM_NT, GEMM_NN, GEMM_TN = _D['DLSG_GEMM_NT'], _D['DLSG_GEMM_NN'], _D['DLSG_GEMM_TN']
F_ACCUM, F_BIAS, F_TANH = _D['DLSG_GEMM_ACCUM'], _D['DLSG_GEMM_BIAS'], _D['DLSG_GEMM_TANH']
F_FORCE64, F_FORCE128, F_TILE256, F_BF16X3 = (_D['DLSG_GEMM_' + n] for n in ('FORCE64', 'FORCE128', 'TILE256', 'BF16X3'))
F_SK, F_NOSK, F_SK_BM128, F_SK_BM256, F_SK_BN128, F_SK_NOXMAP = (_D['DLSG_GEMM_' + n] for n in (
    'SK', 'NOSK', 'SK_BM128', 'SK_BM256', 'SK_BN128', 'SK_NOXMAP'))
F_SK_GIVEAWAY = _D['DLSG_GEMM_SK_GIVEAWAY']

i64, u32, u64, f32 = C.c_int64, C.c_uint32, C.c_uint64, C.c_float


def load_library(path=LIB_PATH):
    if not os.path.exists(path):
# ... 94 lines not shown
                med = ms[len(ms) // 2] if len(ms) % 2 else 0.5 * (ms[len(ms) // 2 - 1] + ms[len(ms) // 2])
                shapes[shp]['ms_total'] = med * len(ms)
            out[key] = dict(launches=len(rec), ms_total=sum(d['ms_total'] for d in shapes.values()),
                            work_total=float(sum(r[2] for r in rec)), shapes=shapes)
        return out

    @staticmethod
    def _stream():
        return C.c_void_p(torch.cuda.current_stream().cuda_stream)

    launches = 0

    def _check(self, rc, what):
        self.launches += 1
        if rc != 0:
            raise RuntimeError('%s failed with code %d' % (what, rc))

    stream_k = True
    sk_cu_budget = 0

    _gemm_ws = {}
    _capture_streams = {}

    @classmethod
    def capture_stream(cls, dev):
        dev = torch.device(dev)
        idx = dev.index if dev.index is not None else torch.cuda.current_device()
        st = cls._capture_streams.get(idx)
        if st is None:
            st = cls._capture_streams[idx] = torch.cuda.Stream(device=idx)
        return st

    def _gemm_workspace(self, dev):
        key = (dev.index, torch.cuda.current_stream(dev).cuda_stream)
        ws = HipOps._gemm_ws.get(key)
        if ws is None:
            n = int(self.lib.dlsg_gemm_ws_bytes())
            if n <= 0:
                raise RuntimeError('dlsg_gemm_ws_bytes() failed: no device?')
            if torch.cuda.is_current_stream_capturing():
                return None
            ws = HipOps._gemm_ws[key] = torch.zeros((n + 3) // 4, dtype=torch.float32, device=dev)
        return ws

    def device_cus(self):
        n = int(self.lib.dlsg_gemm_ws_bytes())
        return max(0, (n - 16384) // (2 * 256 * 256 * 4))

    def comm_rehearsal(self, view, workgroups, passes):
        self._check(self.lib.dlsg_comm_rehearsal(_p(view), i64(view.numel()), int(workgroups), int(passes), self._stream()),
                    'dlsg_comm_rehearsal')

    def gemm(self, mode, groups, alpha=1.0, flags=0, bias=None, skip_if=None, plan_only=False):
        a = abi.dlsg_gemm_args()
        A0, B0, C0 = groups[0][:3]
        batched = A0.dim() == 3
        if batched:
            nb = C0.size(0)
            a.bsa, a.bsb, a.bsc = A0.stride(0), B0.stride(0), C0.stride(0)
        else:
            nb = 1
            a.bsa = a.bsb = a.bsc = 0
        M = C0.shape[-2]
        N = max(g[2].shape[-1] for g in groups)
        a.mode, a.M, a.N, a.ldc = mode, M, N, C0.stride(-2)
        a.ngroups, a.nbatch, a.alpha = len(groups), nb, alpha
        gbias = any(len(g) > 3 and g[3] is not None for g in groups)
        a.flags = flags | self.extra_flags | (F_BIAS if (bias is not None or gbias) else 0)
        a.bias = _p(bias)
        a.skip_if = _p(skip_if)
        if (self.stream_k or (flags & F_SK)) and not ((flags | self.extra_flags) & F_NOSK):
            ws = self._gemm_workspace(C0.device)
            if ws is not None:
                a.ws, a.ws_bytes = _p(ws), ws.numel() * 4
                a.cu_budget = int(self.sk_cu_budget)
        assert len(groups) <= MAXG
        for i, grp_ in enumerate(groups):
            A, B, Cc = grp_[:3]
            Ng = Cc.shape[-1]
            if mode == GEMM_TN:
                K = A.shape[-2]
                assert A.shape[-1] == M and B.shape[-2] == K and B.shape[-1] == Ng, (A.shape, B.shape, Cc.shape)
            elif mode == GEMM_NN:
                K = A.shape[-1]
                assert A.shape[-2] == M and B.shape[-2] == K and B.shape[-1] == Ng, (A.shape, B.shape, Cc.shape)
            else:
                K = A.shape[-1]
                assert A.shape[-2] == M and B.shape[-1] == K and B.shape[-2] == Ng, (A.shape, B.shape, Cc.shape)
            for t in (A, B, Cc):
                assert t.dtype == torch.float32 and (t.stride(-1) == 1 or t.size(-1) == 1), (t.shape, t.stride())
            assert Cc.shape[-2] == M
            if batched:
                assert (A.stride(0), B.stride(0), Cc.stride(0)) == (a.bsa, a.bsb, a.bsc)
            g = a.g[i]
            g.A, g.B, g.C = _p(A), _p(B), _p(Cc)
            g.lda, g.ldb, g.K, g.N = A.stride(-2), B.stride(-2), K, (Ng if Ng != N else 0)
            g.bias = _p(grp_[3]) if len(grp_) > 3 else None
            g.ldc = Cc.stride(-2) if Cc.stride(-2) != a.ldc else 0
        if plan_only:
            return int(self.lib.dlsg_gemm_variant(C.byref(a)))
        e0 = None
        if self.flop_count is not None:
            self.flop_count += 2.0 * M * nb * sum(grp_[2].shape[-1] * a.g[i].K for i, grp_ in enumerate(groups))
        if self.prof is not None:
            flops = 2.0 * M * nb * sum(grp_[2].shape[-1] * a.g[i].K for i, grp_ in enumerate(groups))
            if flops >= self.prof_min_flops:
                e0 = self._prof_begin()
        self._check(self.lib.dlsg_gemm(C.byref(a), self._stream()), 'dlsg_gemm')
        if e0 is not None:
            x3 = bool(a.flags & F_BF16X3)
            if x3:
                tiles_l = ((M + 127) // 128) * ((N + 127) // 128) * nb * len(groups)
                if a.flags & (F_FORCE64 | F_FORCE128):
                    variant = '64x64' if a.flags & F_FORCE64 else '128x128'
                elif M <= 64 and mode != GEMM_TN and N >= 64:
                    variant = 'skinny_64x32'
                else:
                    variant = '128x128' if tiles_l >= 1000 else '64x64'
            else:
                v = self.lib.dlsg_gemm_variant(C.byref(a))
                variant = {0: '64x64', 1: '128x64', 2: '128x128', 3: 'skinny_64x32' if M <= 64 else 'skinny_128x32', 4: '256x256',
                           5: '256x128', 6: '256x256+rest', 7: 'streamk_256x256'}[v]
            ks = sorted(set(a.g[i].K for i in range(len(groups))))
            ns_ = sorted(set(grp_[2].shape[-1] for grp_ in groups))
            shape = '%s M=%d N=%s K=%s groups=%d batch=%d' % (('NT', 'NN', 'TN')[mode], M, '/'.join(map(str, ns_)), '/'.join(map(str, ks)),
                                                              len(groups), nb)
            ob = 0
            for i, grp_ in enumerate(groups):
                Ng = grp_[2].shape[-1]
                Kg = a.g[i].K
                ob += 4 * nb * (M * Kg + Ng * Kg + M * Ng * (2 if (a.flags & F_ACCUM) else 1))
            self._prof_end('gemm_%s_mfma_%s_%s' % ('bf16x3' if x3 else 'f32', variant, ('nt', 'nn', 'tn')[mode]), e0, flops, shape, ob)

    def slab_reduce(self, slabs, out, bias=None, flags=0):
        S, rows, n = slabs.shape
        assert slabs.stride(2) == 1 and slabs.stride(1) == n
        self._check(self.lib.dlsg_slab_reduce(_p(slabs), S, i64(slabs.stride(0)), _p(bias), _p(out), i64(rows), n,
                                              int(out.stride(0)), flags | (F_BIAS if bias is not None else 0),
                                              self._stream()), 'dlsg_slab_reduce')

    def _rowln_args(self, x, gamma, beta, y, stats, res, pe, pre_tanh, post_tanh, p1, site1, p2, site2, seed, eps):
        a = abi.dlsg_rowln_args()
        _chk2(x)
        a.x, a.ldx = _p(x), x.stride(0)
        a.res, a.ldres = _p(res), (res.stride(0) if res is not None else 0)
        a.gamma, a.beta = _p(gamma), _p(beta)
        a.y, a.ldy = _p(y), (y.stride(0) if y is not None else 0)
        a.stats = _p(stats)
        a.pe, a.pe_rows = _p(pe), (pe.size(0) if pe is not None else 1)
        a.rows, a.n = x.size(0), x.size(1)
        a.pre_tanh, a.post_tanh, a.eps = pre_tanh, post_tanh, eps
        a.p1, a.p2, a.site1, a.site2 = p1, p2, site1, site2
        a.seed, a.seed_ptr = _seed(seed)
        return a

    def rowln_fwd(self, x, gamma, beta, y, stats=None, res=None, pe=None, pre_tanh=0, post_tanh=0, p1=0.0, site1=0,
                  p2=0.0, site2=0, seed=0, eps=1e-5):
        a = self._rowln_args(x, gamma, beta, y, stats, res, pe, pre_tanh, post_tanh, p1, site1, p2, site2, seed, eps)
        self._check(self.lib.dlsg_rowln_fwd(C.byref(a), self._stream()), 'dlsg_rowln_fwd')

    def rowln_fwd_multi(self, items):
        n = len(items)
        if n == 1:
            return self.rowln_fwd(**items[0])
        arr = (abi.dlsg_rowln_args * n)()
        for i, it in enumerate(items):
            d = dict(stats=None, res=None, pe=None, pre_tanh=0, post_tanh=0, p1=0.0, site1=0, p2=0.0, site2=0, seed=0, eps=1e-5)
            d.update(it)
            arr[i] = self._rowln_args(d['x'], d['gamma'], d['beta'], d['y'], d['stats'], d['res'], d['pe'], d['pre_tanh'],
                                      d['post_tanh'], d['p1'], d['site1'], d['p2'], d['site2'], d['seed'], d['eps'])
        self._check(self.lib.dlsg_rowln_fwd_multi(arr, n, self._stream()), 'dlsg_rowln_fwd_multi')

    def rowln_bwd_multi(self, items):
        n = len(items)
        if n == 1:
            return self.rowln_bwd(**items[0])
        arr = (abi.dlsg_rowln_bwd_args * n)()
        for i, it in enumerate(items):
            d = dict(stats=None, res=None, pe=None, pre_tanh=0, post_tanh=0, p1=0.0, site1=0, p2=0.0, site2=0, seed=0, eps=1e-5,
                     dgb_part=None, accum_dx=False)
            d.update(it)
            b = arr[i]
            b.f = self._rowln_args(d['x'], d['gamma'], d['beta'], None, d['stats'], d['res'], d['pe'], d['pre_tanh'], d['post_tanh'],
                                   d['p1'], d['site1'], d['p2'], d['site2'], d['seed'], d['eps'])
            b.dy, b.lddy, b.dx, b.lddx = _p(d['dy']), d['dy'].stride(0), _p(d['dx']), d['dx'].stride(0)
# ... 195 lines not shown
            self._psl_bwd_args(arr[i], **it)
        self._check(self.lib.dlsg_latent_psl_bwd_multi(arr, n, self._stream()), 'dlsg_latent_psl_bwd_multi')

    def sa_core_supported(self, T, D):
        return T <= 32 and D % 64 == 0

    def sa_core_fwd(self, K, Q, V, w, out, scale, mask=None):
        B, T, D = K.shape
        for t in (K, Q, V, w, out):
            _chkc(t)
        a = abi.dlsg_sa_core_args()
        a.K, a.Q, a.V, a.mask, a.w, a.out = _p(K), _p(Q), _p(V), _p(mask), _p(w), _p(out)
        a.B, a.T, a.D, a.scale = B, T, D, scale
        self._check(self.lib.dlsg_sa_core_fwd(C.byref(a), self._stream()), 'dlsg_sa_core_fwd')

    def sa_core_bwd(self, w, K, Q, V, dout, dK, dQ, dV, scale):
        B, T, D = K.shape
        for t in (w, K, Q, V, dout, dK, dQ, dV):
            _chkc(t)
        a = abi.dlsg_sa_core_bwd_args()
        a.w, a.K, a.Q, a.V, a.dout, a.dK, a.dQ, a.dV = _p(w), _p(K), _p(Q), _p(V), _p(dout), _p(dK), _p(dQ), _p(dV)
        a.B, a.T, a.D, a.scale = B, T, D, scale
        self._check(self.lib.dlsg_sa_core_bwd(C.byref(a), self._stream()), 'dlsg_sa_core_bwd')

    def _decatt_args(self, Kp, Vp, q, c, alpha, scale):
        a = abi.dlsg_decatt_args()
        ns = len(Kp)
        B, P, Q = Kp[0].shape
        H = Vp[0].shape[2]
        for s in range(ns):
            a.Kp[s], a.Vp[s] = Kp[s].data_ptr(), Vp[s].data_ptr()
            if c is not None:
                a.c[s] = c[s].data_ptr()
        a.q, a.ldq = _p(q), q.stride(0)
        a.ldc = c[0].stride(0) if c is not None else 0
        a.alpha = _p(alpha)
        a.B, a.P, a.Q, a.H, a.nstream, a.scale = B, P, Q, H, ns, scale
        return a

    def decatt_fwd(self, Kp, Vp, q, c, alpha, scale):
        a = self._decatt_args(Kp, Vp, q, c, alpha, scale)
        self._check(self.lib.dlsg_decatt_fwd(C.byref(a), self._stream()), 'dlsg_decatt_fwd')

    def decatt_bwd(self, Kp, Vp, q, alpha, dc, dKp, dVp, dq, scale, accum_dq=False, dalpha=None):
        b = abi.dlsg_decatt_bwd_args()
        b.f = self._decatt_args(Kp, Vp, q, None, alpha, scale)
        for s in range(len(Kp)):
            b.dc[s], b.dKp[s], b.dVp[s] = dc[s].data_ptr(), dKp[s].data_ptr(), dVp[s].data_ptr()
        b.lddc = dc[0].stride(0)
        b.dalpha = _p(dalpha)
        b.dq, b.lddq, b.accum_dq = _p(dq), dq.stride(0), int(accum_dq)
        self._check(self.lib.dlsg_decatt_bwd(C.byref(b), self._stream()), 'dlsg_decatt_bwd')

    def dec_mid_fwd(self, slabs, addend, b_ih, b_hh, c_prev, c, h, gates, lnq, qcur, st_q, p_q, site_q, Kp, Vp, lnc, cpre,
                    ctx, st_c, alpha, p_att, site_att, scale, seed=0, eps=1e-5, kv_div=1):
        a = abi.dlsg_dec_mid_args()
        a.kv_div = kv_div
        assert Kp[0].size(0) * max(1, kv_div) == c.size(0), (Kp[0].shape, c.shape, kv_div)
        a.slabs, a.nslab, a.slab_stride = _p(slabs), slabs.size(0), slabs.stride(0)
        a.addend, a.ldadd = _p(addend), (addend.stride(0) if addend is not None else 0)
        a.b_ih, a.b_hh, a.c_prev, a.c, a.h, a.gates = _p(b_ih), _p(b_hh), _p(c_prev), _p(c), _p(h), _p(gates)
        a.lnq_g, a.lnq_b, a.qcur, a.st_q, a.p_q, a.site_q = _p(lnq[0]), _p(lnq[1]), _p(qcur), _p(st_q), p_q, site_q
        ns = len(Kp)
        for i in range(ns):
            _chkc(Kp[i]); _chkc(Vp[i]); _chkc(cpre[i]); _chkc(ctx[i])
            a.Kp[i], a.Vp[i] = Kp[i].data_ptr(), Vp[i].data_ptr()
            a.lnc_g[i], a.lnc_b[i] = lnc[i][0].data_ptr(), lnc[i][1].data_ptr()
            a.cpre[i], a.ctx[i], a.st_c[i] = cpre[i].data_ptr(), ctx[i].data_ptr(), st_c[i].data_ptr()
            a.p_att[i], a.site_att[i] = p_att[i], site_att[i]
        for t in (c, h, gates, qcur, alpha):
            _chkc(t)
        a.alpha = _p(alpha)
        a.B, a.Q, a.H, a.P, a.nstream = c.size(0), c.size(1), Vp[0].size(2), Kp[0].size(1), ns
        a.scale, a.eps = scale, eps
        a.seed, a.seed_ptr = _seed(seed)
        self._check(self.lib.dlsg_dec_mid_fwd(C.byref(a), self._stream()), 'dlsg_dec_mid_fwd')

    DEC_TAIL_SAMPLE_MAX_WEIGHTS = 1 << 21

    def dec_tail_sample_supported(self, V, D):
        return V * D <= self.DEC_TAIL_SAMPLE_MAX_WEIGHTS

    def dec_tail_fwd(self, slabs, b_ih, b_hh, c_prev, c, hd, gates, ln, dout, st_l, p, site, seed=0, eps=1e-5, sample=None):
        a = abi.dlsg_dec_tail_args()
        if sample is not None:
            sm = sample
            for t_ in (sm['W'], sm['E'], sm['ids_out']):
                _chkc(t_)
            assert sm['W'].shape[1] == c.size(1) and sm['we_out'].stride(1) == 1 and sm['ids_out'].dtype == torch.int64
            a.s_coins, a.s_t, a.s_V = _p(sm['coins']), int(sm['t']), sm['W'].shape[0]
            a.s_W, a.s_b, a.s_E, a.s_Wd = _p(sm['W']), _p(sm.get('b')), _p(sm['E']), sm['E'].shape[1]
            a.s_site, a.s_ids, a.s_we, a.s_ldwe = sm.get('site', 0), _p(sm['ids_out']), _p(sm['we_out']), sm['we_out'].stride(0)
            a.s_row0, a.s_p = int(sm.get('row0', 0)), float(sm.get('p', 0.0))
        a.slabs, a.nslab, a.slab_stride = _p(slabs), slabs.size(0), slabs.stride(0)
        a.b_ih, a.b_hh, a.c_prev, a.c, a.hd, a.gates = _p(b_ih), _p(b_hh), _p(c_prev), _p(c), _p(hd), _p(gates)
        for t in (c, hd, gates, dout):
            _chkc(t)
        a.ln_g, a.ln_b, a.dout, a.st_l, a.p, a.site = _p(ln[0]), _p(ln[1]), _p(dout), _p(st_l), p, site
        a.B, a.D, a.eps = c.size(0), c.size(1), eps
        a.seed, a.seed_ptr = _seed(seed)
        self._check(self.lib.dlsg_dec_tail_fwd(C.byref(a), self._stream()), 'dlsg_dec_tail_fwd')

    def dec_mid_bwd(self, slabs, dlh_rec, cpre, st_c, lnc_g, part_c, dcpre, p_att, site_att, Kp, Vp, alpha, dalpha, ds, qh,
                    st_q, lnq_g, part_q, p_q, site_q, rec_slabs, gates, c, c_prev, dc, dgates, scale, seed=0):
        a = abi.dlsg_dec_mid_bwd_args()
        ns = len(Kp)
        B, Q = c.shape
        H, P = Vp[0].size(2), Kp[0].size(1)
        D = slabs.size(2) - ns * H - Q
        _chkc(slabs)
        a.slabs, a.nslab, a.slab_stride = _p(slabs), slabs.size(0), slabs.stride(0)
        a.write_rec, a.dlh_rec = int(dlh_rec is not None), _p(dlh_rec)
        for i in range(ns):
            for t in (cpre[i], part_c[i], dcpre[i], Kp[i], Vp[i]):
                _chkc(t)
            a.cpre[i], a.st_c[i], a.lnc_g[i] = cpre[i].data_ptr(), st_c[i].data_ptr(), lnc_g[i].data_ptr()
            a.part_c[i], a.dcpre[i] = part_c[i].data_ptr(), dcpre[i].data_ptr()
            a.p_att[i], a.site_att[i] = p_att[i], site_att[i]
            a.Kp[i], a.Vp[i] = Kp[i].data_ptr(), Vp[i].data_ptr()
        for t in (alpha, ds, qh, part_q, gates, c, dc, dgates) + ((dlh_rec,) if dlh_rec is not None else ()):
            _chkc(t)
        a.alpha, a.dalpha, a.ds = _p(alpha), _p(dalpha), _p(ds)
        a.qh, a.st_q, a.lnq_g, a.part_q, a.p_q, a.site_q = _p(qh), _p(st_q), _p(lnq_g), _p(part_q), p_q, site_q
        if rec_slabs is not None:
            a.rec_slabs, a.rec_nslab = _p(rec_slabs), rec_slabs.size(0)
            a.rec_slab_stride, a.rec_ld = rec_slabs.stride(0), rec_slabs.stride(1)
        a.gates, a.c, a.c_prev, a.dc, a.dgates = _p(gates), _p(c), _p(c_prev), _p(dc), _p(dgates)
        a.B, a.Q, a.H, a.D, a.P, a.nstream, a.scale = B, Q, H, D, P, ns, scale
        a.seed, a.seed_ptr = _seed(seed)
        self._check(self.lib.dlsg_dec_mid_bwd(C.byref(a), self._stream()), 'dlsg_dec_mid_bwd')

    def decatt_cache_grads(self, alpha, ds, qcur, dcpre, dKp, dVp):
        a = abi.dlsg_decatt_cache_grads_args()
        L, B, Q = qcur.shape
        ns = len(dKp)
        for t in (alpha, ds, qcur):
            _chkc(t)
        a.alpha, a.ds, a.qcur = _p(alpha), _p(ds), _p(qcur)
        for i in range(ns):
            for t in (dcpre[i], dKp[i], dVp[i]):
                _chkc(t)
            a.dcpre[i], a.dKp[i], a.dVp[i] = dcpre[i].data_ptr(), dKp[i].data_ptr(), dVp[i].data_ptr()
        a.L, a.B, a.Q, a.H, a.P, a.nstream = L, B, Q, dVp[0].size(2), dKp[0].size(1), ns
        self._check(self.lib.dlsg_decatt_cache_grads(C.byref(a), self._stream()), 'dlsg_decatt_cache_grads')

    def _persist_word(self, dev):
        w = getattr(self, '_persist_err', None)
        if w is None or w.device != dev:
            w = self._persist_err = torch.zeros(1, dtype=torch.int32, device=dev)
        return w

    guard_word = _persist_word

    def persist_word_or_none(self):
        return getattr(self, '_persist_err', None)

    def check_persistent(self, code=None):
        w = getattr(self, '_persist_err', None)
        if w is None:
            return
        if code is None:
            code = int(w.item())
        if code:
            w.zero_()
            self.persistent_bilstm = False
            self.persist_timeouts = getattr(self, 'persist_timeouts', 0) + 1
            raise RuntimeError('persistent kernel hand-off timed out (code %d): the launch was not co-resident on this device.  '
                               'No parameter was updated by the steps since; the BiLSTM now runs step by step '
                               '(ops.persistent_bilstm = False)%s.  The critic\'s LSTM has no step-by-step form: GAN training needs '
                               'the device to itself.  Is the GPU shared with another process?' % (code, ''))

    persistent_bilstm = True
    persistent_bilstm_bwd = True

    def bilstm_supported(self, B, T, H):
        return self.persistent_bilstm and bool(self.lib.dlsg_bilstm_supported(B, T, H))

    def bilstm_fwd(self, xg, w_hh, b_ih, b_hh, out, hprev, c, gates):
        B, T, H2 = out.shape
        H = H2 // 2
        a = abi.dlsg_bilstm_args()
        dev = out.device
# ... 71 lines not shown

    def lstm_seq_bwd(self, As, Cs, W, dHs, dAs, dCs, DA, DH, DC):
        return self._lstm_seq(1, W, As=As, Cs=Cs, dHs=dHs, dAs=dAs, dCs=dCs, DA=DA, DH=DH, DC=DC)

    def lstm_seq_bwd2(self, As, Cs, W, DH, DC, ubar, gA, gC, gDH, gDHprev, gDC):
        return self._lstm_seq(2, W, As=As, Cs=Cs, DH=DH, DC=DC, addend=ubar, gA=gA, gC=gC, gDH=gDH, gDC=gDC, gDHprev=gDHprev)

    @staticmethod
    def _pw_fwd_args(a, slabs, c, B, H, addend=None, b_ih=None, b_hh=None, c_prev=None, h=None, h2=None, gates=None,
                     p=0.0, site=0, seed=0):
        if slabs is not None:
            a.slabs, a.nslab, a.slab_stride = _p(slabs), slabs.size(0), slabs.stride(0)
        else:
            a.slabs, a.nslab, a.slab_stride = None, 0, 0
        a.addend, a.ldadd = _p(addend), (addend.stride(0) if addend is not None else 0)
        a.b_ih, a.b_hh = _p(b_ih), _p(b_hh)
        a.c_prev, a.ldcp = _p(c_prev), (c_prev.stride(0) if c_prev is not None else 0)
        a.c, a.ldc_ = _p(c), c.stride(0)
        a.h, a.ldh = _p(h), (h.stride(0) if h is not None else 0)
        a.h2, a.ldh2 = _p(h2), (h2.stride(0) if h2 is not None else 0)
        a.gates, a.ldg = _p(gates), (gates.stride(0) if gates is not None else 0)
        a.B, a.H, a.p, a.site = B, H, p, site
        a.seed, a.seed_ptr = _seed(seed)

    def lstm_pw_fwd(self, slabs, c, B, H, **kw):
        a = abi.dlsg_lstm_pw_args()
        self._pw_fwd_args(a, slabs, c, B, H, **kw)
        self._check(self.lib.dlsg_lstm_pw_fwd(C.byref(a), self._stream()), 'dlsg_lstm_pw_fwd')

    def lstm_pw_fwd_multi(self, calls):
        arr = (abi.dlsg_lstm_pw_args * len(calls))()
        for a, kw in zip(arr, calls):
            self._pw_fwd_args(a, **kw)
        self._check(self.lib.dlsg_lstm_pw_fwd_n(arr, len(calls), self._stream()), 'dlsg_lstm_pw_fwd_n')

    @staticmethod
    def _pw_bwd_args(a, gates, c, dgates, B, H, c_prev=None, dh=None, dh2=None, dc_next=None, dc_prev=None, p=0.0,
                     site=0, seed=0, dh3=None, dh4=None):
        a.gates, a.ldg, a.c, a.ldc_ = _p(gates), gates.stride(0), _p(c), c.stride(0)
        a.c_prev, a.ldcp = _p(c_prev), (c_prev.stride(0) if c_prev is not None else 0)
        a.dh, a.lddh = _p(dh), (dh.stride(0) if dh is not None else 0)
        a.dh2, a.lddh2 = _p(dh2), (dh2.stride(0) if dh2 is not None else 0)
        a.dh3, a.lddh3 = _p(dh3), (dh3.stride(0) if dh3 is not None else 0)
        if dh4 is not None and dh4.dim() == 3:
            a.dh4, a.lddh4, a.dh4_nslab, a.dh4_slab_stride = _p(dh4), dh4.stride(1), dh4.size(0), dh4.stride(0)
        else:
            a.dh4, a.lddh4 = _p(dh4), (dh4.stride(0) if dh4 is not None else 0)
        a.dc_next, a.lddcn = _p(dc_next), (dc_next.stride(0) if dc_next is not None else 0)
        a.dgates, a.lddg = _p(dgates), dgates.stride(0)
        a.dc_prev, a.lddcp = _p(dc_prev), (dc_prev.stride(0) if dc_prev is not None else 0)
        a.B, a.H, a.p, a.site = B, H, p, site
        a.seed, a.seed_ptr = _seed(seed)

    def lstm_pw_bwd(self, gates, c, dgates, B, H, **kw):
        a = abi.dlsg_lstm_pw_bwd_args()
        self._pw_bwd_args(a, gates, c, dgates, B, H, **kw)
        self._check(self.lib.dlsg_lstm_pw_bwd(C.byref(a), self._stream()), 'dlsg_lstm_pw_bwd')

    def lstm_pw_bwd_multi(self, calls):
        arr = (abi.dlsg_lstm_pw_bwd_args * len(calls))()
        for a, kw in zip(arr, calls):
            self._pw_bwd_args(a, **kw)
        self._check(self.lib.dlsg_lstm_pw_bwd_n(arr, len(calls), self._stream()), 'dlsg_lstm_pw_bwd_n')

    def mean_rows_fwd(self, x, out):
        B, P, H = x.shape
        self._check(self.lib.dlsg_mean_rows_fwd(_p(x), _p(out), i64(out.stride(0)), B, P, H, self._stream()), 'mean_rows_fwd')

    def mean_rows_bwd(self, dout, dx, accum=False):
        B, P, H = dx.shape
        self._check(self.lib.dlsg_mean_rows_bwd(_p(dout), i64(dout.stride(0)), _p(dx), B, P, H, int(accum), self._stream()),
                    'mean_rows_bwd')

    def embed_fwd(self, E, ids, out, p=0.0, seed=0, site=0, row0=0):
        rows, W = out.shape
        sd, sp = _seed(seed)
        self._check(self.lib.dlsg_embed_fwd(_p(E), _p(ids), _p(out), i64(out.stride(0)), rows, W, f32(p), u64(sd), u32(site),
                                            i64(row0), sp, self._stream()), 'embed_fwd')

    def select_embed(self, logits, captions, t, coins, E, ids_out, out, p=0.0, seed=0, site=0, row0=0, prefilled=False):
        rows, V = logits.shape
        sd, sp = _seed(seed)
        self._check(self.lib.dlsg_select_embed(_p(logits), i64(logits.stride(0)), V, _p(captions), captions.shape[1], int(t),
                                               _p(coins), _p(E), _p(ids_out), _p(out), i64(out.stride(0)), rows, out.shape[1],
                                               f32(p), u64(sd), u32(site), i64(row0), sp, int(bool(prefilled)), self._stream()), 'select_embed')

    def embed_bwd(self, dout, ids, dE, p=0.0, seed=0, site=0, row0=0):
        rows, W = dout.shape
        sd, sp = _seed(seed)
        self._check(self.lib.dlsg_embed_bwd(_p(dout), i64(dout.stride(0)), _p(ids), _p(dE), rows, W, f32(p), u64(sd),
                                            u32(site), i64(row0), sp, self._stream()), 'embed_bwd')

    def argmax(self, logits, ids):
        rows, V = logits.shape
        self._check(self.lib.dlsg_argmax(_p(logits), i64(logits.stride(0)), _p(ids), rows, V, self._stream()), 'argmax')

    def sample_embed(self, logits, E, ids_out, out, logp, lens, t, end_id, temperature=1.0, p=0.0, seed=0, site=0, site_sample=0,
                     row0=0):
        rows, V = logits.shape
        assert E.shape[0] >= V and E.is_contiguous() and ids_out.numel() == rows and logp.numel() == rows and lens.numel() == rows
        assert ids_out.dtype == torch.int64 and lens.dtype == torch.int64 and out.shape == (rows, E.shape[1])
        sd, sp = _seed(seed)
        self._check(self.lib.dlsg_sample_embed(_p(logits), i64(logits.stride(0)), V, f32(temperature), _p(E), _p(ids_out), _p(out),
                                               i64(out.stride(0)), out.shape[1], _p(logp), _p(lens), int(t), i64(end_id), rows, f32(p),
                                               u64(sd), u32(site), u32(site_sample), i64(row0), sp, self._stream()), 'sample_embed')

    def copy2d(self, src, dst, accum=False):
        rows, n = src.shape
        self._check(self.lib.dlsg_copy2d(_p(src), i64(src.stride(0)), _p(dst), i64(dst.stride(0)), rows, n, int(accum),
# ... 342 lines not shown
```

include/dlsg.h:

```cpp
#ifndef DLSG_H
#define DLSG_H
#include <stdint.h>
#ifdef __cplusplus
extern "C" {
#endif

#define DLSG_ABI_VERSION 8
int dlsg_abi_version(void);

#define DLSG_OK 0
#define DLSG_EINVAL (-1)
#define DLSG_ELAUNCH (-2)
#define DLSG_EALIGN (-3)
#define DLSG_ENOCOMM (-4)
int dlsg_struct_size(int which);

#define DLSG_GEMM_NT 0
#define DLSG_GEMM_NN 1
#define DLSG_GEMM_TN 2
#define DLSG_GEMM_MAXG 16
#define DLSG_GEMM_ACCUM 1
#define DLSG_GEMM_BIAS 2
#define DLSG_GEMM_TANH 4
#define DLSG_GEMM_FORCE64 256
// ... 139 lines not shown
    const float* K; const float* Q; const float* V; const float* mask;
    float* w; float* out;
    int32_t B, T, D; float scale;
} dlsg_sa_core_args;
int dlsg_sa_core_fwd(const dlsg_sa_core_args* a, void* stream);
typedef struct {
    const float* w; const float* K; const float* Q; const float* V; const float* dout;
    float* dK; float* dQ; float* dV;
    int32_t B, T, D; float scale;
} dlsg_sa_core_bwd_args;
int dlsg_sa_core_bwd(const dlsg_sa_core_bwd_args* a, void* stream);

int dlsg_softmax_fwd(const float* x, const float* mask, float* y, int64_t outer, int n, int inner, void* stream);
int dlsg_softmax_bwd(const float* y, const float* dy, float* dx, int64_t outer, int n, int inner, void* stream);

typedef struct {
    const float* Kp[2]; const float* Vp[2];
    const float* q; int64_t ldq;
    float* c[2]; int64_t ldc;
    float* alpha;
    int32_t B, P, Q, H, nstream;
    float scale;
} dlsg_decatt_args;
int dlsg_decatt_fwd(const dlsg_decatt_args* a, void* stream);
typedef struct {
    dlsg_decatt_args f;
    const float* dc[2]; int64_t lddc;
    const float* dalpha;
    float* dKp[2]; float* dVp[2];
    float* dq; int64_t lddq; int32_t accum_dq;
} dlsg_decatt_bwd_args;
int dlsg_decatt_bwd(const dlsg_decatt_bwd_args* a, void* stream);

typedef struct {
    const float* slabs; int32_t nslab; int32_t pad_; int64_t slab_stride;
    const float* addend; int64_t ldadd;
    const float* b_ih; const float* b_hh;
    const float* c_prev;
    float* c; float* h; float* gates;
    const float* lnq_g; const float* lnq_b;
    float* qcur; float* st_q;
    float p_q; uint32_t site_q;
    const float* Kp[2]; const float* Vp[2];
    const float* lnc_g[2]; const float* lnc_b[2];
    float* cpre[2]; float* ctx[2]; float* st_c[2];
    float* alpha;
    float p_att[2]; uint32_t site_att[2];
    int32_t B, Q, H, P, nstream;
    float scale, eps;
    int32_t kv_div;
    uint64_t seed; const uint64_t* seed_ptr;
} dlsg_dec_mid_args;
int dlsg_dec_mid_fwd(const dlsg_dec_mid_args* a, void* stream);
typedef struct {
    const float* slabs; int32_t nslab; int32_t pad_; int64_t slab_stride;
    const float* b_ih; const float* b_hh;
    const float* c_prev; float* c; float* hd; float* gates;
    const float* ln_g; const float* ln_b;
    float* dout; float* st_l;
    float p; uint32_t site;
    int32_t B, D;
    float eps;
    uint64_t seed; const uint64_t* seed_ptr;
    const int32_t* s_coins; int32_t s_t; int32_t s_V;
    const float* s_W; const float* s_b;
    const float* s_E; int32_t s_Wd; uint32_t s_site;
    int64_t* s_ids; float* s_we; int64_t s_ldwe;
    int64_t s_row0; float s_p; float pad2_;
} dlsg_dec_tail_args;
int dlsg_dec_tail_fwd(const dlsg_dec_tail_args* a, void* stream);
typedef struct {
    const float* slabs; int32_t nslab; int32_t write_rec; int64_t slab_stride;
    float* dlh_rec;
    const float* cpre[2]; const float* st_c[2]; const float* lnc_g[2];
    float* part_c[2];
    float* dcpre[2];
    float p_att[2]; uint32_t site_att[2];
    const float* Kp[2]; const float* Vp[2];
    const float* alpha; const float* dalpha;
    float* ds;
    const float* qh; const float* st_q; const float* lnq_g;
    float* part_q;
    float p_q; uint32_t site_q;
    const float* rec_slabs; int32_t rec_nslab; int32_t pad_; int64_t rec_slab_stride; int64_t rec_ld;
    const float* gates; const float* c; const float* c_prev;
    float* dc;
    float* dgates;
    int32_t B, Q, H, D, P, nstream;
    float scale; float pad2_;
    uint64_t seed; const uint64_t* seed_ptr;
} dlsg_dec_mid_bwd_args;
int dlsg_dec_mid_bwd(const dlsg_dec_mid_bwd_args* a, void* stream);
typedef struct {
    const float* alpha; const float* ds;
    const float* qcur;
    const float* dcpre[2];
    float* dKp[2]; float* dVp[2];
    int32_t L, B, Q, H, P, nstream;
} dlsg_decatt_cache_grads_args;
int dlsg_decatt_cache_grads(const dlsg_decatt_cache_grads_args* a, void* stream);

typedef struct {
    const float* slabs; int32_t nslab; int32_t pad_; int64_t slab_stride;
    const float* addend; int64_t ldadd;
    const float* b_ih; const float* b_hh;
    const float* c_prev; int64_t ldcp;
    float* c; int64_t ldc_;
    float* h; int64_t ldh;
    float* h2; int64_t ldh2;
    float* gates; int64_t ldg;
    int32_t B, H;
    float p; uint32_t site; uint64_t seed;
    const uint64_t* seed_ptr;
} dlsg_lstm_pw_args;
int dlsg_lstm_pw_fwd(const dlsg_lstm_pw_args* a, void* stream);
int dlsg_lstm_pw_fwd_n(const dlsg_lstm_pw_args* a, int count, void* stream);
typedef struct {
    const float* gates; int64_t ldg;
    const float* c; int64_t ldc_;
    const float* c_prev; int64_t ldcp;
    const float* dh; int64_t lddh;
    const float* dh2; int64_t lddh2;
    const float* dh3; int64_t lddh3;
    const float* dh4; int64_t lddh4;
    int32_t dh4_nslab; int32_t pad4_; int64_t dh4_slab_stride;
    const float* dc_next; int64_t lddcn;
    float* dgates; int64_t lddg;
    float* dc_prev; int64_t lddcp;
    int32_t B, H;
    float p; uint32_t site; uint64_t seed;
    const uint64_t* seed_ptr;
} dlsg_lstm_pw_bwd_args;
int dlsg_lstm_pw_bwd(const dlsg_lstm_pw_bwd_args* a, void* stream);
int dlsg_lstm_pw_bwd_n(const dlsg_lstm_pw_bwd_args* a, int count, void* stream);

int dlsg_mean_rows_fwd(const float* x, float* out, int64_t ldo, int B, int P, int H, void* stream);
int dlsg_mean_rows_bwd(const float* dout, int64_t lddo, float* dx, int B, int P, int H, int accum, void* stream);
int dlsg_embed_fwd(const float* E, const int64_t* ids, float* out, int64_t ldo, int rows, int W, float p, uint64_t seed,
                   uint32_t site, int64_t row0, const uint64_t* seed_ptr, void* stream);
int dlsg_embed_bwd(const float* dout, int64_t lddo, const int64_t* ids, float* dE, int rows, int W, float p,
                   uint64_t seed, uint32_t site, int64_t row0, const uint64_t* seed_ptr, void* stream);
int dlsg_select_embed(const float* logits, int64_t ld, int V, const int64_t* captions, int L, int t, const int32_t* coins,
                      const float* E, int64_t* ids_out, float* out, int64_t ldo, int rows, int W, float p, uint64_t seed,
                      uint32_t site, int64_t row0, const uint64_t* seed_ptr, int prefilled, void* stream);
int dlsg_argmax(const float* logits, int64_t ld, int64_t* ids, int rows, int V, void* stream);
int dlsg_sample_embed(const float* logits, int64_t ld, int V, float temperature, const float* E, int64_t* ids_out, float* out,
                      int64_t ldo, int W, float* logp, int64_t* lens, int t, int64_t end_id, int rows, float p, uint64_t seed,
                      uint32_t site_word, uint32_t site_sample, int64_t row0, const uint64_t* seed_ptr, void* stream);
int dlsg_copy2d(const float* src, int64_t lds, float* dst, int64_t ldd, int rows, int n, int accum, void* stream);
int dlsg_dropout(const float* x, int64_t ldx, float* y, int64_t ldy, int rows, int n, float p, uint64_t seed,
                 uint32_t site, const uint64_t* seed_ptr, void* stream);
int dlsg_fill(float* dst, int64_t n, float value, void* stream);
int dlsg_gather_rows(const float* src, int64_t lds, const int64_t* idx, float* dst, int64_t ldd, int rows, int n, void* stream);
int dlsg_permute_tb(const float* src, float* dst, int T, int B, int n, void* stream);

#define DLSG_CRIT_C 512
#define DLSG_CRIT_LMAX 32
#define DLSG_CRIT_TMAX 8

int dlsg_crit_embed_mix(const float* proj_tm, const int64_t* ids, const float* W, const float* bias, const float* eps, float* h,
                        int ng, int B, int L, int V, void* stream);
int dlsg_crit_embed_mix_bwd(const float* ch, const float* eps, float* dhr, float* dhf_tm, int ng, int B, int L, void* stream);
int dlsg_crit_vocab_scatter(const float* dhr, const int64_t* ids, float* dW, int rows, int V, void* stream);

int dlsg_crit_relu_taps(const float* x, const float* ref, const float* bias, float bias_scale, float* y, float* taps, int n, int L,
                        void* stream);
int dlsg_crit_relu_taps_bwd(const float* dy, const float* dtaps, const float* ref, float* dx, int n, int L, void* stream);

#define DLSG_CLN_MAXG 4
typedef struct {
    const float* x[DLSG_CLN_MAXG]; const float* gamma[DLSG_CLN_MAXG]; const float* beta[DLSG_CLN_MAXG];
    float* y[DLSG_CLN_MAXG];
    const float* dy[3][DLSG_CLN_MAXG]; float* dx[DLSG_CLN_MAXG];
    float* dgamma[DLSG_CLN_MAXG]; float* dbeta[DLSG_CLN_MAXG]; const float* extra[DLSG_CLN_MAXG];
    const float* U[DLSG_CLN_MAXG]; float* gx[DLSG_CLN_MAXG]; float* gdy[DLSG_CLN_MAXG]; float* gpart[DLSG_CLN_MAXG];
    float* ws;
    int32_t rows, N, groups, pre_tanh, ndy, acc_lo, acc_hi;
    int32_t defer;
    float eps, p_pre, p_post; uint32_t site_pre, site_post, pad2_;
    uint64_t seed; const uint64_t* seed_ptr; int64_t row0;
} dlsg_cln_args;
int64_t dlsg_cln_ws_floats(int rows, int N);
int dlsg_cln_fwd(const dlsg_cln_args* a, void* stream);
int dlsg_cln_bwd(const dlsg_cln_args* a, void* stream);
int dlsg_cln_bwd2(const dlsg_cln_args* a, void* stream);

typedef struct {
// ... 177 lines not shown
```

Before: 4978 clips/s.

## Co-schedule skinny GEMM tiles with decoder step row kernels in one launch

Refactors the decoder mid/tail forward and mid backward kernels into per-row device functions that use a single LDS buffer. New fused 'co' kernels launch B row blocks plus skinny GEMM tile blocks in the same grid, so an independent small-M GEMM runs on the idle CUs while the latency-bound per-row decoder work proceeds. It also adds a pw_bwd variant that reads recurrent slabs. Dynamic LDS is sized to the larger of the row and GEMM needs, which may lower occupancy, and correctness depends on the co-tenant GEMM being independent of the row kernel's outputs.

```diff
diff --git a/d-lsg-video-caption_amd/csrc/decstep.hip b/d-lsg-video-caption_amd/csrc/decstep.hip
--- a/d-lsg-video-caption_amd/csrc/decstep.hip
+++ b/d-lsg-video-caption_amd/csrc/decstep.hip
@@ -1,5 +1,6 @@
 #include "common.hpp"
 #include "dlsg.h"
+#include "skinny_tile.hpp"
 
 using namespace dlsg;
 
@@ -108,14 +109,15 @@
     rstd = rsqrtf(block_sum(q, red) / n + eps);
 }
 
-template <int V>
-__global__ __launch_bounds__(DT) void dec_mid_fwd_kernel(const dlsg_dec_mid_args a) {
-    __shared__ __attribute__((aligned(16))) float gb[4 * MAXW];
-    __shared__ __attribute__((aligned(16))) float hb[MAXW];
-    __shared__ __attribute__((aligned(16))) float qb[MAXW];
-    __shared__ float sc[2 * MAXP], wt[2 * MAXP];
-    __shared__ float red[32];
-    const int b = blockIdx.x;
+constexpr int MID_FWD_LDS = 4 * MAXW + MAXW + MAXW + 4 * MAXP + 32;
+template <int V>
+__device__ __forceinline__ void dec_mid_fwd_row(const dlsg_dec_mid_args& a, const int b, float* lds) {
+    float* gb = lds;
+    float* hb = gb + 4 * MAXW;
+    float* qb = hb + MAXW;
+    float* sc = qb + MAXW;
+    float* wt = sc + 2 * MAXP;
+    float* red = wt + 2 * MAXP;
     const int bk = a.kv_div > 1 ? b / a.kv_div : b;
     const int Q = a.Q, H = a.H, P = a.P, ns = a.nstream;
     const int lane = threadIdx.x & 63, w = threadIdx.x >> 6;
@@ -210,11 +212,19 @@
 }
 
 template <int V>
-__global__ __launch_bounds__(DT) void dec_tail_fwd_kernel(const dlsg_dec_tail_args a) {
-    __shared__ __attribute__((aligned(16))) float gb[4 * MAXW];
-    __shared__ __attribute__((aligned(16))) float hb[MAXW];
-    __shared__ float red[32];
-    const int b = blockIdx.x;
+__global__ __launch_bounds__(DT) void dec_mid_fwd_kernel(const dlsg_dec_mid_args a) {
+    __shared__ __attribute__((aligned(16))) float lds[MID_FWD_LDS];
+    dec_mid_fwd_row<V>(a, blockIdx.x, lds);
+}
+
+constexpr int TAIL_FWD_LDS = 4 * MAXW + MAXW + 32 + DT / 64 + 4;
+template <int V>
+__device__ __forceinline__ void dec_tail_fwd_row(const dlsg_dec_tail_args& a, const int b, float* lds) {
+    float* gb = lds;
+    float* hb = gb + 4 * MAXW;
+    float* red = hb + MAXW;
+    int* s_bi = reinterpret_cast<int*>(red + 32);
+    int64_t& s_chosen = *reinterpret_cast<int64_t*>(s_bi + DT / 64);
     const int D = a.D;
     const uint64_t seed = a.seed + (a.seed_ptr ? *a.seed_ptr : 0ull);
     constexpr int ND = MAXW / DT;
@@ -247,8 +257,6 @@
         if (j < D) hb[j] = dv[i];
     }
     __syncthreads();
-    __shared__ int s_bi[DT / 64];
-    __shared__ int64_t s_chosen;
     const int lane = threadIdx.x & 63, w = threadIdx.x >> 6;
     float best = -INFINITY;
     int bidx = 0x7fffffff;
@@ -296,6 +304,11 @@
     }
 }
 
+template <int V>
+__global__ __launch_bounds__(DT) void dec_tail_fwd_kernel(const dlsg_dec_tail_args a) {
+    __shared__ __attribute__((aligned(16))) float lds[TAIL_FWD_LDS];
+    dec_tail_fwd_row<V>(a, blockIdx.x, lds);
+}
 
 template <int N>
 __device__ __forceinline__ void block_sumN(float (&v)[N], float* red) {
@@ -316,15 +329,17 @@
     }
 }
 
-template <int V>
-__global__ __launch_bounds__(DT) void dec_mid_bwd_kernel(const dlsg_dec_mid_bwd_args a) {
-    __shared__ __attribute__((aligned(16))) float dxb[3 * MAXW];
-    __shared__ __attribute__((aligned(16))) float dcp[2 * MAXW];
-    __shared__ __attribute__((aligned(16))) float dqb[2 * MAXW];
-    __shared__ float dwb[2 * MAXP], dsb[2 * MAXP], wb[2 * MAXP];
-    __shared__ float red[64];
+constexpr int MID_BWD_LDS = 7 * MAXW + 6 * MAXP + 64;
+template <int V>
+__device__ __forceinline__ void dec_mid_bwd_row(const dlsg_dec_mid_bwd_args& a, const int b, float* lds) {
+    float* dxb = lds;
+    float* dcp = dxb + 3 * MAXW;
+    float* dqb = dcp + 2 * MAXW;
+    float* dwb = dqb + 2 * MAXW;
+    float* dsb = dwb + 2 * MAXP;
+    float* wb = dsb + 2 * MAXP;
+    float* red = wb + 2 * MAXP;
     constexpr int IC = 2 * MAXW / DT, IQ = MAXW / DT;
-    const int b = blockIdx.x;
     const int Q = a.Q, H = a.H, D = a.D, P = a.P, ns = a.nstream;
     const int NX = ns * H + Q, WT = NX + D;
     const int lane = threadIdx.x & 63, w = threadIdx.x >> 6;
@@ -514,6 +529,12 @@
     }
 }
 
+template <int V>
+__global__ __launch_bounds__(DT) void dec_mid_bwd_kernel(const dlsg_dec_mid_bwd_args a) {
+    __shared__ __attribute__((aligned(16))) float lds[MID_BWD_LDS];
+    dec_mid_bwd_row<V>(a, blockIdx.x, lds);
+}
+
 constexpr int CG_PC = 8;
 template <int V>
 __global__ __launch_bounds__(256) void decatt_cache_grads_kernel(const dlsg_decatt_cache_grads_args a) {
@@ -549,43 +570,118 @@
 
 bool vec_ok(const void* p) { return (reinterpret_cast<uintptr_t>(p) & 15) == 0; }
 
-}
-
-extern "C" int dlsg_dec_mid_fwd(const dlsg_dec_mid_args* a, void* stream) {
+constexpr int CO_MAX_M = 64;
+constexpr int co_lds_bytes(int row_floats, int MI) {
+    return row_floats * 4 > skinny::s2_lds_bytes(MI, 1) ? row_floats * 4 : skinny::s2_lds_bytes(MI, 1);
+}
+extern __shared__ __attribute__((aligned(16))) char co_lds[];
+
+template <int MI>
+__global__ __launch_bounds__(DT) void dec_mid_fwd_co_kernel(const dlsg_dec_mid_args a, const skinny::CoArgs co) {
+    if ((int)blockIdx.x < a.B) dec_mid_fwd_row<4>(a, blockIdx.x, reinterpret_cast<float*>(co_lds));
+    else skinny::co_tile<MI, false>(co, blockIdx.x - a.B, co_lds);
+}
+template <int MI>
+__global__ __launch_bounds__(DT) void dec_tail_fwd_co_kernel(const dlsg_dec_tail_args a, const skinny::CoArgs co) {
+    if ((int)blockIdx.x < a.B) dec_tail_fwd_row<4>(a, blockIdx.x, reinterpret_cast<float*>(co_lds));
+    else skinny::co_tile<MI, false>(co, blockIdx.x - a.B, co_lds);
+}
+template <int MI>
+__global__ __launch_bounds__(DT) void dec_mid_bwd_co_kernel(const dlsg_dec_mid_bwd_args a, const skinny::CoArgs co) {
+    if ((int)blockIdx.x < a.B) dec_mid_bwd_row<4>(a, blockIdx.x, reinterpret_cast<float*>(co_lds));
+    else skinny::co_tile<MI, true>(co, blockIdx.x - a.B, co_lds);
+}
+
+int device_cus() {
+    static const int cus = [] {
+        int dev = 0, n = 0;
+        if (hipGetDevice(&dev) != hipSuccess || hipDeviceGetAttribute(&n, hipDeviceAttributeMultiprocessorCount, dev) != hipSuccess) n = 0;
+        return n;
+    }();
+    return cus;
+}
+
+template <typename K, typename A>
+int launch_co(K kern, int lds_bytes, const A& a, const skinny::CoArgs& c, int B, void* stream) {
+    static const hipError_t attr =
+        hipFuncSetAttribute(reinterpret_cast<const void*>(kern), hipFuncAttributeMaxDynamicSharedMemorySize, lds_bytes);
+    if (attr != hipSuccess) return DLSG_ELAUNCH;
+    hipLaunchKernelGGL(kern, dim3(B + c.ntn * c.ngroups), dim3(DT), lds_bytes, reinterpret_cast<hipStream_t>(stream), a, c);
+    DLSG_CHECK_LAUNCH();
+    return DLSG_OK;
+}
+
+int mid_fwd_check(const dlsg_dec_mid_args* a, bool* v4_out) {
     if (!a || a->Q < 1 || a->Q > MAXW || a->H < 1 || a->H > MAXW || a->P < 1 || a->P > MAXP || a->nstream < 1 || a->nstream > 2)
         return DLSG_EINVAL;
-    if (a->B == 0) return DLSG_OK;
     bool v4 = a->Q % 4 == 0 && a->H % 4 == 0 && a->slab_stride % 4 == 0 && a->ldadd % 4 == 0 && vec_ok(a->slabs) &&
               vec_ok(a->addend) && vec_ok(a->b_ih) && vec_ok(a->b_hh) && vec_ok(a->gates);
     for (int s = 0; s < a->nstream; ++s) v4 = v4 && vec_ok(a->Kp[s]) && vec_ok(a->Vp[s]) && vec_ok(a->cpre[s]);
+    *v4_out = v4;
+    return DLSG_OK;
+}
+int tail_fwd_check(const dlsg_dec_tail_args* a, bool* v4_out) {
+    if (!a || a->D < 1 || a->D > MAXW) return DLSG_EINVAL;
+    if (a->B != 0 && a->s_coins && (!a->s_W || !a->s_E || !a->s_ids || !a->s_we || a->s_V < 1 || a->s_Wd < 1)) return DLSG_EINVAL;
+    *v4_out = a->D % 4 == 0 && a->slab_stride % 4 == 0 && vec_ok(a->slabs) && vec_ok(a->b_ih) && vec_ok(a->b_hh) &&
+              vec_ok(a->gates) && (!a->s_coins || vec_ok(a->s_W));
+    return DLSG_OK;
+}
+int mid_bwd_check(const dlsg_dec_mid_bwd_args* a, bool* v4_out) {
+    if (!a || a->Q < 1 || a->Q > MAXW || a->H < 1 || a->H > MAXW || a->D < 0 || a->P < 1 || a->P > MAXP || a->nstream < 1 ||
+        a->nstream > 2)
+        return DLSG_EINVAL;
+    bool v4 = a->Q % 4 == 0 && a->H % 4 == 0 && a->D % 4 == 0 && a->slab_stride % 4 == 0 && vec_ok(a->slabs) && vec_ok(a->dlh_rec);
+    for (int s = 0; s < a->nstream; ++s) v4 = v4 && vec_ok(a->Kp[s]) && vec_ok(a->Vp[s]);
+    *v4_out = v4;
+    return DLSG_OK;
+}
+
+}
+
+extern "C" int dlsg_dec_mid_fwd(const dlsg_dec_mid_args* a, void* stream) {
+    bool v4;
+    if (mid_fwd_check(a, &v4) != DLSG_OK) return DLSG_EINVAL;
+    if (a->B == 0) return DLSG_OK;
     hipLaunchKernelGGL(v4 ? dec_mid_fwd_kernel<4> : dec_mid_fwd_kernel<1>, dim3(a->B), dim3(DT), 0,
                        reinterpret_cast<hipStream_t>(stream), *a);
     DLSG_CHECK_LAUNCH();
     return DLSG_OK;
 }
 extern "C" int dlsg_dec_tail_fwd(const dlsg_dec_tail_args* a, void* stream) {
-    if (!a || a->D < 1 || a->D > MAXW) return DLSG_EINVAL;
+    bool v4;
+    if (tail_fwd_check(a, &v4) != DLSG_OK) return DLSG_EINVAL;
     if (a->B == 0) return DLSG_OK;
-    if (a->s_coins && (!a->s_W || !a->s_E || !a->s_ids || !a->s_we || a->s_V < 1 || a->s_Wd < 1)) return DLSG_EINVAL;
-    const bool v4 = a->D % 4 == 0 && a->slab_stride % 4 == 0 && vec_ok(a->slabs) && vec_ok(a->b_ih) && vec_ok(a->b_hh) &&
-                    vec_ok(a->gates) && (!a->s_coins || vec_ok(a->s_W));
     hipLaunchKernelGGL(v4 ? dec_tail_fwd_kernel<4> : dec_tail_fwd_kernel<1>, dim3(a->B), dim3(DT), 0,
                        reinterpret_cast<hipStream_t>(stream), *a);
     DLSG_CHECK_LAUNCH();
     return DLSG_OK;
 }
 extern "C" int dlsg_dec_mid_bwd(const dlsg_dec_mid_bwd_args* a, void* stream) {
-    if (!a || a->Q < 1 || a->Q > MAXW || a->H < 1 || a->H > MAXW || a->D < 0 || a->P < 1 || a->P > MAXP || a->nstream < 1 ||
-        a->nstream > 2)
-        return DLSG_EINVAL;
+    bool v4;
+    if (mid_bwd_check(a, &v4) != DLSG_OK) return DLSG_EINVAL;
     if (a->B == 0) return DLSG_OK;
-    bool v4 = a->Q % 4 == 0 && a->H % 4 == 0 && a->D % 4 == 0 && a->slab_stride % 4 == 0 && vec_ok(a->slabs) && vec_ok(a->dlh_rec);
-    for (int s = 0; s < a->nstream; ++s) v4 = v4 && vec_ok(a->Kp[s]) && vec_ok(a->Vp[s]);
     hipLaunchKernelGGL(v4 ? dec_mid_bwd_kernel<4> : dec_mid_bwd_kernel<1>, dim3(a->B), dim3(DT), 0,
                        reinterpret_cast<hipStream_t>(stream), *a);
     DLSG_CHECK_LAUNCH();
     return DLSG_OK;
 }
+
+#define DLSG_CO_ENTRY(NAME, ARGS, CHECK, KERN, ROW_LDS, BT)                                                             \
+    extern "C" int NAME##_co(const ARGS* a, const dlsg_gemm_args* co, void* stream) {                                  \
+        bool v4;                                                                                                       \
+        if (CHECK(a, &v4) != DLSG_OK) return DLSG_EINVAL;                                                              \
+        skinny::CoArgs c;                                                                                              \
+        if (a->B > 0 && v4 && co && co->M <= CO_MAX_M && skinny::co_fill(co, BT, a->B, device_cus(), &c))              \
+            return launch_co(KERN<2>, co_lds_bytes(ROW_LDS, 2), *a, c, a->B, stream);                                  \
+        const int rc = NAME(a, stream);                                                                                \
+        return (rc != DLSG_OK || !co) ? rc : dlsg_gemm(co, stream);                                                    \
+    }
+DLSG_CO_ENTRY(dlsg_dec_mid_fwd, dlsg_dec_mid_args, mid_fwd_check, dec_mid_fwd_co_kernel, MID_FWD_LDS, false)
+DLSG_CO_ENTRY(dlsg_dec_tail_fwd, dlsg_dec_tail_args, tail_fwd_check, dec_tail_fwd_co_kernel, TAIL_FWD_LDS, false)
+DLSG_CO_ENTRY(dlsg_dec_mid_bwd, dlsg_dec_mid_bwd_args, mid_bwd_check, dec_mid_bwd_co_kernel, MID_BWD_LDS, true)
+#undef DLSG_CO_ENTRY
+
 extern "C" int dlsg_decatt_cache_grads(const dlsg_decatt_cache_grads_args* a, void* stream) {
     if (!a || a->L < 0 || a->P < 1 || a->nstream < 1 || a->nstream > 2) return DLSG_EINVAL;
     if (a->B == 0) return DLSG_OK;
diff --git a/d-lsg-video-caption_amd/csrc/gemm.hip b/d-lsg-video-caption_amd/csrc/gemm.hip
--- a/d-lsg-video-caption_amd/csrc/gemm.hip
+++ b/d-lsg-video-caption_amd/csrc/gemm.hip
@@ -3,6 +3,7 @@
 
 #include "common.hpp"
 #include "dlsg.h"
+#include "skinny_tile.hpp"
 
 namespace {
 
@@ -409,182 +410,21 @@
     }
 }
 
-constexpr int S2_STAGE = 16;
-constexpr int S2_DEPTH = 3;
-constexpr int S2_B_BYTES = 32 * 64;
-constexpr int s2_lds_bytes(int MI, int NJ) { return 4 * S2_DEPTH * (MI + NJ) * S2_B_BYTES; }
-
-template <int VB>
-__device__ __forceinline__ void s2_glds(const char* src, char* dst) {
-#if defined(__HIP_DEVICE_COMPILE__)
-    typedef __attribute__((address_space(3))) void* lp_t;
-    typedef const __attribute__((address_space(1))) void* gp_t;
-    __builtin_amdgcn_global_load_lds((gp_t)src, (lp_t)dst, 16, 0, 0);
-#endif
-}
+using skinny::S2_STAGE;
+using skinny::s2_lds_bytes;
 
 template <int MI, int NJ, bool BT = false>
 __global__ __launch_bounds__(NT) void skinny2_nt_kernel(const KArgs p) {
-    constexpr int S2_A_BYTES = MI * S2_B_BYTES;
-    constexpr int SLOT = S2_A_BYTES + NJ * S2_B_BYTES;
     extern __shared__ __attribute__((aligned(16))) char s2_lds[];
     if (p.skip_if && *p.skip_if) return;
     const int z = blockIdx.y;
     const int gi = z % p.ngroups, bi = z / p.ngroups;
     const dlsg_gemm_group grp = p.g[gi];
-    const float* A = grp.A + (int64_t)bi * p.bsa;
-    const float* B = grp.B + (int64_t)bi * p.bsb;
-    float* C = grp.C + (int64_t)bi * p.bsc;
-    const int K = grp.K, M = p.M, N = grp.N > 0 ? grp.N : p.N;
+    const int N = grp.N > 0 ? grp.N : p.N;
     const int n0 = blockIdx.x * 32 * NJ;
     if (n0 >= N) return;
-    const int lane = threadIdx.x & 63, w = threadIdx.x >> 6;
-    const int r = lane & 31, h = lane >> 5;
-    char* ring = s2_lds + w * (S2_DEPTH * SLOT);
-
-    const int rho = lane >> 2, sig = lane & 3;
-    const float* srcA[2 * MI];
-    const float* srcB[2 * NJ];
-#pragma unroll
-    for (int pc = 0; pc < 2 * MI; ++pc) {
-        const int R = 16 * pc + rho;
-        srcA[pc] = A + (int64_t)min(R, M - 1) * grp.lda + 4 * (sig ^ ((R >> 2) & 3));
-    }
-#pragma unroll
-    for (int pc = 0; pc < 2 * NJ; ++pc) {
-        if (!BT) {
-            const int R = 16 * pc + rho;
-            srcB[pc] = B + (int64_t)min(n0 + R, N - 1) * grp.ldb + 4 * (sig ^ ((R >> 2) & 3));
-        } else {
-            const int kr = 8 * (pc & 1) + (lane >> 3), c = n0 + 32 * (pc >> 1) + 4 * (lane & 7);
-            srcB[pc] = B + (int64_t)kr * grp.ldb + min(c, N - 4);
-        }
-    }
-    const int nst = (K + S2_STAGE - 1) / S2_STAGE;
-    const int mine = (nst - w + 3) / 4;
-    auto issue = [&](int i) {
-        const int k0 = (4 * i + w) * S2_STAGE;
-        char* slot = ring + (i % S2_DEPTH) * SLOT;
-        const int koff = (k0 + S2_STAGE <= K) ? k0 : (K - S2_STAGE);
-#pragma unroll
-        for (int pc = 0; pc < 2 * MI; ++pc) s2_glds<16>(reinterpret_cast<const char*>(srcA[pc] + koff), slot + pc * 1024);
-#pragma unroll
-        for (int pc = 0; pc < 2 * NJ; ++pc)
-            s2_glds<16>(reinterpret_cast<const char*>(BT ? srcB[pc] + (int64_t)koff * grp.ldb : srcB[pc] + koff), slot + S2_A_BYTES + pc * 1024);
-    };
-
-    f32x16 acc[MI][NJ];
-#pragma unroll
-    for (int i = 0; i < MI; ++i)
-#pragma unroll
-        for (int nj = 0; nj < NJ; ++nj)
-#pragma unroll
-            for (int e = 0; e < 16; ++e) acc[i][nj][e] = 0.f;
-
-    int offA[MI][2], offB[NJ][2];
-#pragma unroll
-    for (int q = 0; q < 2; ++q) {
-        const int ks = 2 * q + h;
-#pragma unroll
-        for (int mi = 0; mi < MI; ++mi) {
-            const int R = 32 * mi + r;
-            offA[mi][q] = (R >> 4) * 1024 + (R & 15) * 64 + ((ks ^ ((R >> 2) & 3)) * 16);
-        }
-#pragma unroll
-        for (int nj = 0; nj < NJ; ++nj) {
-            const int R = 32 * nj + r;
-            offB[nj][q] = BT ? S2_A_BYTES + nj * 2048 + (4 * ks) * 128 + r * 4
-                             : S2_A_BYTES + (R >> 4) * 1024 + (R & 15) * 64 + ((ks ^ ((R >> 2) & 3)) * 16);
-        }
-    }
-    constexpr int PCS = 2 * MI + 2 * NJ;
-
-    if (mine > 0) issue(0);
-    if (mine > 1) issue(1);
-    for (int i = 0; i < mine; ++i) {
-        if (i + 2 < mine) {
-            issue(i + 2);
-            asm volatile("s_waitcnt vmcnt(%0)" ::"n"(2 * PCS) : "memory");
-        } else if (i + 1 < mine) {
-            asm volatile("s_waitcnt vmcnt(%0)" ::"n"(PCS) : "memory");
-        } else {
-            asm volatile("s_waitcnt vmcnt(0)" ::: "memory");
-        }
-        const char* slot = ring + (i % S2_DEPTH) * SLOT;
-        const int k0 = (4 * i + w) * S2_STAGE;
-        const bool part = k0 + S2_STAGE > K;
-        const int kbase = part ? K - S2_STAGE : k0;
-        f32x4 fa[MI][2], fb[NJ][2];
-#pragma unroll
-        for (int q = 0; q < 2; ++q) {
-#pragma unroll
-            for (int mi = 0; mi < MI; ++mi) fa[mi][q] = *reinterpret_cast<const f32x4*>(slot + offA[mi][q]);
-#pragma unroll
-            for (int nj = 0; nj < NJ; ++nj) {
-                if (!BT) fb[nj][q] = *reinterpret_cast<const f32x4*>(slot + offB[nj][q]);
-                else {
-#pragma unroll
-                    for (int j = 0; j < 4; ++j) fb[nj][q][j] = *reinterpret_cast<const float*>(slot + offB[nj][q] + j * 128);
-                }
-            }
-        }
-        if (part) {
-#pragma unroll
-            for (int q = 0; q < 2; ++q)
-#pragma unroll
-                for (int j = 0; j < 4; ++j) {
-                    const int k = kbase + 4 * (2 * q + h) + j;
-                    const bool keep = k >= k0 && k < K;
-#pragma unroll
-                    for (int mi = 0; mi < MI; ++mi) fa[mi][q][j] = keep ? fa[mi][q][j] : 0.f;
-#pragma unroll
-                    for (int nj = 0; nj < NJ; ++nj) fb[nj][q][j] = keep ? fb[nj][q][j] : 0.f;
-                }
-        }
-#pragma unroll
-        for (int q = 0; q < 2; ++q)
-#pragma unroll
-            for (int j = 0; j < 4; ++j)
-#pragma unroll
-                for (int nj = 0; nj < NJ; ++nj)
-#pragma unroll
-                    for (int mi = 0; mi < MI; ++mi)
-                        acc[mi][nj] = __builtin_amdgcn_mfma_f32_32x32x2f32(fa[mi][q][j], fb[nj][q][j], acc[mi][nj], 0, 0, 0);
-    }
-    __syncthreads();
-    float* red = reinterpret_cast<float*>(s2_lds);
-#pragma unroll
-    for (int mi = 0; mi < MI; ++mi)
-#pragma unroll
-        for (int nj = 0; nj < NJ; ++nj)
-#pragma unroll
-            for (int e = 0; e < 16; ++e) red[(((w * MI + mi) * NJ + nj) * 16 + e) * 64 + lane] = acc[mi][nj][e];
-    __syncthreads();
-    const float* biasp = grp.bias ? grp.bias : p.bias;
-    const bool accum = p.flags & DLSG_GEMM_ACCUM, use_bias = (p.flags & DLSG_GEMM_BIAS) && biasp != nullptr;
-    const bool do_tanh = p.flags & DLSG_GEMM_TANH;
-#pragma unroll
-    for (int nj = 0; nj < NJ; ++nj) {
-        const int col = n0 + 32 * nj + r;
-        if (col >= N) continue;
-        const float bv = use_bias ? biasp[col] : 0.f;
-#pragma unroll
-        for (int mi = 0; mi < MI; ++mi)
-#pragma unroll
-            for (int ee = 0; ee < 4; ++ee) {
-                const int e = 4 * w + ee;
-                const int row = 32 * mi + (e & 3) + 8 * (e >> 2) + 4 * h;
-                if (row >= M) continue;
-                float v = 0.f;
-#pragma unroll
-                for (int ww = 0; ww < 4; ++ww) v += red[(((ww * MI + mi) * NJ + nj) * 16 + e) * 64 + lane];
-                v = p.alpha * v + bv;
-                float* cp = C + (int64_t)row * (grp.ldc ? grp.ldc : (int64_t)p.ldc) + col;
-                if (accum) v += *cp;
-                if (do_tanh) v = tanhf(v);
-                *cp = v;
-            }
-    }
+    skinny::tile_body<MI, NJ, BT>(grp, grp.A + (int64_t)bi * p.bsa, grp.B + (int64_t)bi * p.bsb, grp.C + (int64_t)bi * p.bsc, p.M, N,
+                                  p.ldc, p.alpha, p.bias, p.flags, n0, threadIdx.x >> 6, threadIdx.x & 63, s2_lds);
 }
 
 template <int MI>
@@ -609,8 +449,7 @@
         bool ok = a->nbatch == 1;
         for (int i = 0; i < a->ngroups && ok; ++i) {
             const dlsg_gemm_group& g = a->g[i];
-            ok = (g.K % 4 == 0) && g.K >= S2_STAGE && (g.lda % 4 == 0) && (g.ldb % 4 == 0) &&
-                 ((reinterpret_cast<uintptr_t>(g.A) & 15) == 0) && ((reinterpret_cast<uintptr_t>(g.B) & 15) == 0);
+            ok = skinny::group_ok(g, 0, false);
         }
         if (ok) {
             const int wg64 = ((a->N + 63) / 64) * a->ngroups * a->nbatch;
@@ -628,8 +467,7 @@
         for (int i = 0; i < a->ngroups && ok; ++i) {
             const dlsg_gemm_group& g = a->g[i];
             const int gn = g.N > 0 ? g.N : a->N;
-            ok = (g.K % 4 == 0) && g.K >= S2_STAGE && (g.lda % 4 == 0) && (g.ldb % 4 == 0) && (gn % 4 == 0) && gn >= 4 &&
-                 ((reinterpret_cast<uintptr_t>(g.A) & 15) == 0) && ((reinterpret_cast<uintptr_t>(g.B) & 15) == 0);
+            ok = skinny::group_ok(g, gn, true);
         }
         if (ok) {
             bool same_n = true;
diff --git a/d-lsg-video-caption_amd/csrc/rowops.hip b/d-lsg-video-caption_amd/csrc/rowops.hip
--- a/d-lsg-video-caption_amd/csrc/rowops.hip
+++ b/d-lsg-video-caption_amd/csrc/rowops.hip
@@ -386,7 +386,9 @@
     }
 }
 
-__global__ __launch_bounds__(256) void lstm_pw_bwd_kernel(const PwBwdSet set) {
+struct PwRec { const float* slabs; int n; int64_t stride, ld; };
+template <bool REC>
+__global__ __launch_bounds__(256) void lstm_pw_bwd_kernel(const PwBwdSet set, const PwRec rec) {
     const dlsg_lstm_pw_bwd_args& a = set.a[blockIdx.z];
     const int j = blockIdx.x * blockDim.x + threadIdx.x;
     const int b = blockIdx.y;
@@ -397,9 +399,21 @@
     const float c = a.c[(int64_t)b * a.ldc_ + j];
     const float cp = a.c_prev ? a.c_prev[(int64_t)b * a.ldcp + j] : 0.f;
     float dh = a.dh ? a.dh[(int64_t)b * a.lddh + j] : 0.f;
-    if (a.dh2 || a.dh3 || a.dh4) {
+    if (a.dh2 || a.dh3 || a.dh4 || REC) {
         float d2 = a.dh2 ? a.dh2[(int64_t)b * a.lddh2 + j] : 0.f;
         if (a.dh3) d2 += a.dh3[(int64_t)b * a.lddh3 + j];
+        if (REC) {
+            const float* rp = rec.slabs + (int64_t)b * rec.ld + j;
+            float d3 = 0.f;
+            int k = 0;
+            for (; k + 4 <= rec.n; k += 4) {
+                const float t0 = rp[(int64_t)k * rec.stride], t1 = rp[(int64_t)(k + 1) * rec.stride],
+                            t2 = rp[(int64_t)(k + 2) * rec.stride], t3 = rp[(int64_t)(k + 3) * rec.stride];
+                d3 += t0; d3 += t1; d3 += t2; d3 += t3;
+            }
+            for (; k < rec.n; ++k) d3 += rp[(int64_t)k * rec.stride];
+            d2 += d3;
+        }
         if (a.dh4) {
             const int ns4 = a.dh4_nslab > 1 ? a.dh4_nslab : 1;
             const float* hp = a.dh4 + (int64_t)b * a.lddh4 + j;
@@ -1098,11 +1112,23 @@
     if (a[0].B == 0) return DLSG_OK;
     PwBwdSet set;
     for (int i = 0; i < 2; ++i) set.a[i] = a[i < count ? i : 0];
-    hipLaunchKernelGGL(lstm_pw_bwd_kernel, dim3((a[0].H + 255) / 256, a[0].B, count), dim3(256), 0, ST(stream), set);
+    hipLaunchKernelGGL(lstm_pw_bwd_kernel<false>, dim3((a[0].H + 255) / 256, a[0].B, count), dim3(256), 0, ST(stream), set, PwRec{});
     DLSG_CHECK_LAUNCH();
     return DLSG_OK;
 }
 extern "C" int dlsg_lstm_pw_bwd(const dlsg_lstm_pw_bwd_args* a, void* stream) { return dlsg_lstm_pw_bwd_n(a, 1, stream); }
+extern "C" int dlsg_lstm_pw_bwd_rec(const dlsg_lstm_pw_bwd_args* a, const float* rec_slabs, int rec_nslab, int64_t rec_slab_stride,
+                                    int64_t rec_ld, void* stream) {
+    if (!rec_slabs || rec_nslab < 1) return dlsg_lstm_pw_bwd(a, stream);
+    if (!a || a->H < 1) return DLSG_EINVAL;
+    if (a->B == 0) return DLSG_OK;
+    PwBwdSet set;
+    set.a[0] = set.a[1] = *a;
+    hipLaunchKernelGGL(lstm_pw_bwd_kernel<true>, dim3((a->H + 255) / 256, a->B, 1), dim3(256), 0, ST(stream), set,
+                       PwRec{rec_slabs, rec_nslab, rec_slab_stride, rec_ld});
+    DLSG_CHECK_LAUNCH();
+    return DLSG_OK;
+}
 extern "C" int dlsg_mean_rows_fwd(const float* x, float* out, int64_t ldo, int B, int P, int H, void* stream) {
     if (B == 0) return DLSG_OK;
     hipLaunchKernelGGL(mean_rows_fwd_kernel, dim3((H + 255) / 256, B), dim3(256), 0, ST(stream), x, out, ldo, P, H);
diff --git a/d-lsg-video-caption_amd/csrc/skinny_tile.hpp b/d-lsg-video-caption_amd/csrc/skinny_tile.hpp
--- /dev/null
+++ b/d-lsg-video-caption_amd/csrc/skinny_tile.hpp
@@ -0,0 +1,216 @@
+#pragma once
+#include <hip/hip_runtime.h>
+
+#include "common.hpp"
+#include "dlsg.h"
+
+namespace skinny {
+
+constexpr int S2_STAGE = 16;
+constexpr int S2_DEPTH = 3;
+constexpr int S2_B_BYTES = 32 * 64;
+constexpr int s2_lds_bytes(int MI, int NJ) { return 4 * S2_DEPTH * (MI + NJ) * S2_B_BYTES; }
+
+inline bool group_ok(const dlsg_gemm_group& g, int gn, bool bt) {
+    return (g.K % 4 == 0) && g.K >= S2_STAGE && (g.lda % 4 == 0) && (g.ldb % 4 == 0) && (!bt || ((gn % 4 == 0) && gn >= 4)) &&
+           ((reinterpret_cast<uintptr_t>(g.A) & 15) == 0) && ((reinterpret_cast<uintptr_t>(g.B) & 15) == 0);
+}
+
+template <int VB>
+__device__ __forceinline__ void s2_glds(const char* src, char* dst) {
+#if defined(__HIP_DEVICE_COMPILE__)
+    typedef __attribute__((address_space(3))) void* lp_t;
+    typedef const __attribute__((address_space(1))) void* gp_t;
+    __builtin_amdgcn_global_load_lds((gp_t)src, (lp_t)dst, 16, 0, 0);
+#endif
+}
+
+template <int MI, int NJ, bool BT>
+__device__ __forceinline__ void tile_body(const dlsg_gemm_group& grp, const float* A, const float* B, float* C, int M, int N,
+                                          int ldc0, float alpha, const float* bias0, int flags, int n0, int w, int lane,
+                                          char* s2_lds) {
+    constexpr int S2_A_BYTES = MI * S2_B_BYTES;
+    constexpr int SLOT = S2_A_BYTES + NJ * S2_B_BYTES;
+    const int K = grp.K;
+    const int r = lane & 31, h = lane >> 5;
+    char* ring = s2_lds + w * (S2_DEPTH * SLOT);
+
+    const int rho = lane >> 2, sig = lane & 3;
+    const float* srcA[2 * MI];
+    const float* srcB[2 * NJ];
+#pragma unroll
+    for (int pc = 0; pc < 2 * MI; ++pc) {
+        const int R = 16 * pc + rho;
+        srcA[pc] = A + (int64_t)min(R, M - 1) * grp.lda + 4 * (sig ^ ((R >> 2) & 3));
+    }
+#pragma unroll
+    for (int pc = 0; pc < 2 * NJ; ++pc) {
+        if (!BT) {
+            const int R = 16 * pc + rho;
+            srcB[pc] = B + (int64_t)min(n0 + R, N - 1) * grp.ldb + 4 * (sig ^ ((R >> 2) & 3));
+        } else {
+            const int kr = 8 * (pc & 1) + (lane >> 3), c = n0 + 32 * (pc >> 1) + 4 * (lane & 7);
+            srcB[pc] = B + (int64_t)kr * grp.ldb + min(c, N - 4);
+        }
+    }
+    const int nst = (K + S2_STAGE - 1) / S2_STAGE;
+    const int mine = (nst - w + 3) / 4;
+    auto issue = [&](int i) {
+        const int k0 = (4 * i + w) * S2_STAGE;
+        char* slot = ring + (i % S2_DEPTH) * SLOT;
+        const int koff = (k0 + S2_STAGE <= K) ? k0 : (K - S2_STAGE);
+#pragma unroll
+        for (int pc = 0; pc < 2 * MI; ++pc) s2_glds<16>(reinterpret_cast<const char*>(srcA[pc] + koff), slot + pc * 1024);
+#pragma unroll
+        for (int pc = 0; pc < 2 * NJ; ++pc)
+            s2_glds<16>(reinterpret_cast<const char*>(BT ? srcB[pc] + (int64_t)koff * grp.ldb : srcB[pc] + koff), slot + S2_A_BYTES + pc * 1024);
+    };
+
+    f32x16 acc[MI][NJ];
+#pragma unroll
+    for (int i = 0; i < MI; ++i)
+#pragma unroll
+        for (int nj = 0; nj < NJ; ++nj)
+#pragma unroll
+            for (int e = 0; e < 16; ++e) acc[i][nj][e] = 0.f;
+
+    int offA[MI][2], offB[NJ][2];
+#pragma unroll
+    for (int q = 0; q < 2; ++q) {
+        const int ks = 2 * q + h;
+#pragma unroll
+        for (int mi = 0; mi < MI; ++mi) {
+            const int R = 32 * mi + r;
+            offA[mi][q] = (R >> 4) * 1024 + (R & 15) * 64 + ((ks ^ ((R >> 2) & 3)) * 16);
+        }
+#pragma unroll
+        for (int nj = 0; nj < NJ; ++nj) {
+            const int R = 32 * nj + r;
+            offB[nj][q] = BT ? S2_A_BYTES + nj * 2048 + (4 * ks) * 128 + r * 4
+                             : S2_A_BYTES + (R >> 4) * 1024 + (R & 15) * 64 + ((ks ^ ((R >> 2) & 3)) * 16);
+        }
+    }
+    constexpr int PCS = 2 * MI + 2 * NJ;
+
+    if (mine > 0) issue(0);
+    if (mine > 1) issue(1);
+    for (int i = 0; i < mine; ++i) {
+        if (i + 2 < mine) {
+            issue(i + 2);
+            asm volatile("s_waitcnt vmcnt(%0)" ::"n"(2 * PCS) : "memory");
+        } else if (i + 1 < mine) {
+            asm volatile("s_waitcnt vmcnt(%0)" ::"n"(PCS) : "memory");
+        } else {
+            asm volatile("s_waitcnt vmcnt(0)" ::: "memory");
+        }
+        const char* slot = ring + (i % S2_DEPTH) * SLOT;
+        const int k0 = (4 * i + w) * S2_STAGE;
+        const bool part = k0 + S2_STAGE > K;
+        const int kbase = part ? K - S2_STAGE : k0;
+        f32x4 fa[MI][2], fb[NJ][2];
+#pragma unroll
+        for (int q = 0; q < 2; ++q) {
+#pragma unroll
+            for (int mi = 0; mi < MI; ++mi) fa[mi][q] = *reinterpret_cast<const f32x4*>(slot + offA[mi][q]);
+#pragma unroll
+            for (int nj = 0; nj < NJ; ++nj) {
+                if (!BT) fb[nj][q] = *reinterpret_cast<const f32x4*>(slot + offB[nj][q]);
+                else {
+#pragma unroll
+                    for (int j = 0; j < 4; ++j) fb[nj][q][j] = *reinterpret_cast<const float*>(slot + offB[nj][q] + j * 128);
+                }
+            }
+        }
+        if (part) {
+#pragma unroll
+            for (int q = 0; q < 2; ++q)
+#pragma unroll
+                for (int j = 0; j < 4; ++j) {
+                    const int k = kbase + 4 * (2 * q + h) + j;
+                    const bool keep = k >= k0 && k < K;
+#pragma unroll
+                    for (int mi = 0; mi < MI; ++mi) fa[mi][q][j] = keep ? fa[mi][q][j] : 0.f;
+#pragma unroll
+                    for (int nj = 0; nj < NJ; ++nj) fb[nj][q][j] = keep ? fb[nj][q][j] : 0.f;
+                }
+        }
+#pragma unroll
+        for (int q = 0; q < 2; ++q)
+#pragma unroll
+            for (int j = 0; j < 4; ++j)
+#pragma unroll
+                for (int nj = 0; nj < NJ; ++nj)
+#pragma unroll
+                    for (int mi = 0; mi < MI; ++mi)
+                        acc[mi][nj] = __builtin_amdgcn_mfma_f32_32x32x2f32(fa[mi][q][j], fb[nj][q][j], acc[mi][nj], 0, 0, 0);
+    }
+    __syncthreads();
+    float* red = reinterpret_cast<float*>(s2_lds);
+#pragma unroll
+    for (int mi = 0; mi < MI; ++mi)
+#pragma unroll
+        for (int nj = 0; nj < NJ; ++nj)
+#pragma unroll
+            for (int e = 0; e < 16; ++e) red[(((w * MI + mi) * NJ + nj) * 16 + e) * 64 + lane] = acc[mi][nj][e];
+    __syncthreads();
+    const float* biasp = grp.bias ? grp.bias : bias0;
+    const bool accum = flags & DLSG_GEMM_ACCUM, use_bias = (flags & DLSG_GEMM_BIAS) && biasp != nullptr;
+    const bool do_tanh = flags & DLSG_GEMM_TANH;
+#pragma unroll
+    for (int nj = 0; nj < NJ; ++nj) {
+        const int col = n0 + 32 * nj + r;
+        if (col >= N) continue;
+        const float bv = use_bias ? biasp[col] : 0.f;
+#pragma unroll
+        for (int mi = 0; mi < MI; ++mi)
+#pragma unroll
+            for (int ee = 0; ee < 4; ++ee) {
+                const int e = 4 * w + ee;
+                const int row = 32 * mi + (e & 3) + 8 * (e >> 2) + 4 * h;
+                if (row >= M) continue;
+                float v = 0.f;
+#pragma unroll
+                for (int ww = 0; ww < 4; ++ww) v += red[(((ww * MI + mi) * NJ + nj) * 16 + e) * 64 + lane];
+                v = alpha * v + bv;
+                float* cp = C + (int64_t)row * (grp.ldc ? grp.ldc : (int64_t)ldc0) + col;
+                if (accum) v += *cp;
+                if (do_tanh) v = tanhf(v);
+                *cp = v;
+            }
+    }
+}
+
+struct CoArgs {
+    int M, N, ldc, ngroups, flags, ntn;
+    float alpha;
+    const float* bias;
+    dlsg_gemm_group g[DLSG_GEMM_MAXG];
+};
+
+template <int MI, bool BT>
+__device__ __forceinline__ void co_tile(const CoArgs& p, int tile, char* lds) {
+    const int w = threadIdx.x >> 6, lane = threadIdx.x & 63;
+    if (w >= 4) return;
+    const int gi = tile / p.ntn;
+    const dlsg_gemm_group grp = p.g[gi];
+    const int N = grp.N > 0 ? grp.N : p.N;
+    const int n0 = (tile % p.ntn) * 32;
+    if (n0 >= N) return;
+    tile_body<MI, 1, BT>(grp, grp.A, grp.B, grp.C, p.M, N, p.ldc, p.alpha, p.bias, p.flags, n0, w, lane, lds);
+}
+
+inline bool co_fill(const dlsg_gemm_args* a, bool bt, int rows, int cus, CoArgs* out) {
+    if (!a || a->mode != (bt ? DLSG_GEMM_NN : DLSG_GEMM_NT) || a->nbatch != 1 || a->ngroups < 1 || a->ngroups > DLSG_GEMM_MAXG) return false;
+    if (a->M < 1 || a->M > 128 || a->N < 64 || a->skip_if) return false;
+    if (a->flags & ~(DLSG_GEMM_ACCUM | DLSG_GEMM_BIAS | DLSG_GEMM_TANH)) return false;
+    for (int i = 0; i < a->ngroups; ++i)
+        if (!group_ok(a->g[i], a->g[i].N > 0 ? a->g[i].N : a->N, bt)) return false;
+    const int ntn = (a->N + 31) / 32;
+    if (rows + ntn * a->ngroups > cus) return false;
+    out->M = a->M; out->N = a->N; out->ldc = a->ldc; out->ngroups = a->ngroups; out->flags = a->flags; out->ntn = ntn;
+    out->alpha = a->alpha; out->bias = a->bias;
+    for (int i = 0; i < a->ngroups; ++i) out->g[i] = a->g[i];
+    return true;
+}
+
+}
diff --git a/d-lsg-video-caption_amd/dlsg_amd/engine.py b/d-lsg-video-caption_amd/dlsg_amd/engine.py
--- a/d-lsg-video-caption_amd/dlsg_amd/engine.py
+++ b/d-lsg-video-caption_amd/dlsg_amd/engine.py
@@ -146,11 +146,12 @@
     ops.slab_reduce(slabs, out)
 
 
-def gemm_nn_multi_slabs(ops, dy, Ws, width, ref):
+def gemm_nn_multi_slabs(ops, dy, Ws, width, ref, hold_last=False):
     M, Nn = dy.shape
     widths = [W.shape[1] for W in Ws]
     tot = sum(widths)
     assert tot <= width
+    last_width = widths[-1]
     ns = _nsplit_for(M, tot, 1)
     ns = max(1, min(ns, 16 // len(Ws)))
     bounds = _bwd_bounds(Nn, M, ns)
@@ -165,6 +166,10 @@
         for i, (k0, k1) in enumerate(bounds):
             groups.append((dy[:, k0:k1], W[k0:k1, :], slabs[i][:, c0:c0 + wd]))
         c0 += wd
+    if hold_last:
+        nheld = (last_width // widths[-1]) * len(bounds)
+        ops.gemm(GEMM_NN, groups[:-nheld])
+        return slabs, groups[-nheld:]
     ops.gemm(GEMM_NN, groups)
     return slabs
 
@@ -829,17 +834,36 @@
     return s
 
 
-def dec_step(ops, dec, s, t, ref, training, seed, B, word_dropout=True, sample=None):
+def _cotenant(ops, B, N, ngroups=1):
+    f = getattr(ops, 'dec_cotenant_supported', None)
+    return f is not None and bool(f(B, (N + 31) // 32 * ngroups))
+
+
+def dec_step(ops, dec, s, t, ref, training, seed, B, word_dropout=True, sample=None, ahead=False):
     plan = s['plan']
     H, Q, D = plan.H, plan.Q, plan.D
     ql, ll = dec.query_lstm, dec.lang_lstm
     pd = dec.p_drop if training else 0.0
     site = STEP_SITE * (t + 1)
+    rec = t > 0 or s.get('warm', False)
     segs = [(s['WE'][t], ql.weight_ih[:, plan.q_word[0]:plan.q_word[1]])]
-    if t > 0 or s.get('warm', False):
+    if rec:
         segs += [(s['LHP'][t], ql.weight_ih[:, plan.q_lang[0]:plan.q_lang[1]]), (s['QH'][t], ql.weight_hh)]
-    slabs = seg_gemm_nt(ops, segs, B, 4 * Q, ref)
+    early = s.pop('q_ahead', None)
+    if early is not None and early[0] == t and rec and early[1].shape == (len(segs), B, 4 * Q):
+        slabs = early[1]
+        ops.gemm(GEMM_NT, [(a, b, slabs[i]) for i, (a, b) in enumerate(segs[:-1])])
+    else:
+        slabs = seg_gemm_nt(ops, segs, B, 4 * Q, ref)
     ns = plan.ns
+    lsegs = [(s['CTX'][i][t], ll.weight_ih[:, plan.l_ctx[i][0]:plan.l_ctx[i][1]]) for i in range(ns)]
+    lsegs.append((s['QCUR'][t], ll.weight_ih[:, plan.l_q[0]:plan.l_q[1]]))
+    lrec = None
+    if rec:
+        lsegs.append((s['LHP'][t], ll.weight_hh))
+        if _cotenant(ops, B, 4 * D):
+            lslabs = _empty(ref, len(lsegs), B, 4 * D)
+            lrec = lsegs[-1] + (lslabs[len(lsegs) - 1],)
     lnq = dec.query_lstm_layernorm
     atts = _att_modules(dec)
     ops.dec_mid_fwd(slabs, s['gq'], ql.bias_ih, ql.bias_hh, s['QC'][t], s['QC'][t + 1], s['QH'][t + 1], s['GQ'][t],
@@ -848,16 +872,21 @@
                     [s['CPRE'][i][t] for i in range(ns)], [s['CTX'][i][t] for i in range(ns)],
                     [s['ST_C'][i][t] for i in range(ns)], s['ALPHA'][t],
                     [a.dropout if training else 0.0 for a in atts], [site + SITE_ATT1 + i for i in range(ns)],
-                    1.0 / math.sqrt(H), seed=seed, **({'kv_div': s['kv_div']} if s.get('kv_div', 1) > 1 else {}))
-    segs = [(s['CTX'][i][t], ll.weight_ih[:, plan.l_ctx[i][0]:plan.l_ctx[i][1]]) for i in range(ns)]
-    segs.append((s['QCUR'][t], ll.weight_ih[:, plan.l_q[0]:plan.l_q[1]]))
-    if t > 0 or s.get('warm', False):
-        segs.append((s['LHP'][t], ll.weight_hh))
-    slabs = seg_gemm_nt(ops, segs, B, 4 * D, ref)
+                    1.0 / math.sqrt(H), seed=seed, **({'kv_div': s['kv_div']} if s.get('kv_div', 1) > 1 else {}),
+                    **({'co': (GEMM_NT, [lrec])} if lrec is not None else {}))
+    if lrec is not None:
+        ops.gemm(GEMM_NT, [(a, b, lslabs[i]) for i, (a, b) in enumerate(lsegs[:-1])])
+        slabs = lslabs
+    else:
+        slabs = seg_gemm_nt(ops, lsegs, B, 4 * D, ref)
+    kw = {'sample': sample} if sample is not None else {}
+    if ahead and _cotenant(ops, B, 4 * Q):
+        qnext = _empty(ref, 3, B, 4 * Q)
+        kw['co'] = (GEMM_NT, [(s['QH'][t + 1], ql.weight_hh, qnext[2])])
+        s['q_ahead'] = (t + 1, qnext)
     lnl = dec.lang_lstm_layernorm
     ops.dec_tail_fwd(slabs, ll.bias_ih, ll.bias_hh, s['LC'][t], s['LC'][t + 1], s['LHP'][t + 1], s['GL'][t],
-                     (lnl.weight, lnl.bias), s['DOUT'][t], s['ST_L'][t], pd, site + SITE_LANG, seed=seed,
-                     **({'sample': sample} if sample is not None else {}))
+                     (lnl.weight, lnl.bias), s['DOUT'][t], s['ST_L'][t], pd, site + SITE_LANG, seed=seed, **kw)
 
 
 def plan_D(s):
@@ -921,9 +950,9 @@
             if fused_sample and t + 1 < L:
                 dec_step(ops, dec, s, t, ref, training, seed, B,
                          sample=dict(coins=dev_coins, t=t, W=dec.word_restore.weight, b=dec.word_restore.bias, E=E, ids_out=ids[t + 1],
-                                     we_out=s['WE'][t + 1], p=pw, site=SITE_WORD, row0=(t + 1) * B))
+                                     we_out=s['WE'][t + 1], p=pw, site=SITE_WORD, row0=(t + 1) * B), ahead=True)
                 continue
-            dec_step(ops, dec, s, t, ref, training, seed, B)
+            dec_step(ops, dec, s, t, ref, training, seed, B, ahead=t + 1 < L)
             if t + 1 < L:
                 dec_logits(ops, dec, s, t, t + 1, skip_if=dev_coins[t:t + 1])
                 ops.select_embed(s['LOGITS'][t], captions, t, dev_coins, E, ids[t + 1], s['WE'][t + 1], p=pw, seed=seed,
@@ -936,7 +965,7 @@
             ids[i + 1].copy_(captions[:, i])
     ops.embed_fwd(E, ids.view(-1), s['WE'].view((L + 1) * B, -1), p=pw, seed=seed, site=SITE_WORD)
     for t in range(L):
-        dec_step(ops, dec, s, t, ref, training, seed, B)
+        dec_step(ops, dec, s, t, ref, training, seed, B, ahead=t + 1 < L)
         if not coins[t]:
             dec_logits(ops, dec, s, t, t + 1)
             ops.argmax(s['LOGITS'][t], ids[t + 1])
@@ -961,7 +990,7 @@
     end = dec.vocab('<end>')
     ops.embed_fwd(E, ids[0], s['WE'][0], p=pw, seed=seed, site=SITE_WORD, row0=0)
     for t in range(L):
-        dec_step(ops, dec, s, t, ref, training, seed, B)
+        dec_step(ops, dec, s, t, ref, training, seed, B, ahead=t + 1 < L)
         dec_logits(ops, dec, s, t, t + 1)
         ops.sample_embed(s['LOGITS'][t], E, ids[t + 1], s['WE'][t + 1], s['LOGP'][t], s['LENS'], t, end, temperature=temperature,
                          p=pw, seed=seed, site=SITE_WORD, site_sample=SITE_SAMPLE, row0=(t + 1) * B)
@@ -1014,19 +1043,27 @@
     Wq_rec = [ql.weight_hh, ql.weight_ih[:, plan.q_lang[0]:plan.q_lang[1]]]
     wx = ns * H + Q + D
     ql_slabs = None
+    co_bwd = L > 1 and _cotenant(ops, B, D, len(_bwd_bounds(4 * D, B, 1)))
+    lh_slabs = None
     for t in range(L - 1, -1, -1):
         site = STEP_SITE * (t + 1)
         rec = t < L - 1
         ops.lstm_pw_bwd(s['GL'][t], s['LC'][t + 1], dGL[t], B, D, c_prev=s['LC'][t], dh2=dLHo[t],
-                        dh3=dLHrec if rec else None, dh4=ql_slabs[:, :, Q:] if rec else None, dc_next=dLC, dc_prev=dLC,
-                        p=pd, site=site + SITE_LANG, seed=seed)
-        xl_slabs = gemm_nn_multi_slabs(ops, dGL[t], [Wl_in, ll.weight_hh] if t > 0 else [Wl_in], wx, ref)
-        ops.dec_mid_bwd(xl_slabs, dLHrec if t > 0 else None, [s['CPRE'][i][t] for i in range(ns)],
+                        dh3=dLHrec if rec and not co_bwd else None, dh4=ql_slabs[:, :, Q:] if rec else None, dc_next=dLC, dc_prev=dLC,
+                        p=pd, site=site + SITE_LANG, seed=seed, **({'rec': lh_slabs} if rec and co_bwd else {}))
+        held = None
+        if co_bwd and t > 0:
+            xl_slabs, held = gemm_nn_multi_slabs(ops, dGL[t], [Wl_in, ll.weight_hh], wx, ref, hold_last=True)
+            lh_slabs = xl_slabs[:, :, ns * H + Q:]
+        else:
+            xl_slabs = gemm_nn_multi_slabs(ops, dGL[t], [Wl_in, ll.weight_hh] if t > 0 else [Wl_in], wx, ref)
+        ops.dec_mid_bwd(xl_slabs, dLHrec if t > 0 and not co_bwd else None, [s['CPRE'][i][t] for i in range(ns)],
                         [s['ST_C'][i][t] for i in range(ns)], lnc_g, [part_c[i][t] for i in range(ns)],
                         [dCPRE[i][t] for i in range(ns)], p_att, [site + SITE_ATT1 + i for i in range(ns)], s['Kp'], s['Vp'],
                         s['ALPHA'][t], dalpha_tm[t] if dalpha_tm is not None else None, dS[t], s['QH'][t + 1], s['ST_Q'][t],
                         lnq.weight, part_q[t], pd, site + SITE_QUERY, ql_slabs[:, :, :Q] if rec else None, s['GQ'][t],
-                        s['QC'][t + 1], s['QC'][t], dQC, dGQ[t], scale, seed=seed)
+                        s['QC'][t + 1], s['QC'][t], dQC, dGQ[t], scale, seed=seed,
+                        **({'co': (GEMM_NN, held)} if held is not None else {}))
         if t > 0:
             ql_slabs = gemm_nn_multi_slabs(ops, dGQ[t], Wq_rec, Q + D, ref)
     dKp = [torch.empty_like(k) for k in s['Kp']]
diff --git a/d-lsg-video-caption_amd/dlsg_amd/hip.py b/d-lsg-video-caption_amd/dlsg_amd/hip.py
--- a/d-lsg-video-caption_amd/dlsg_amd/hip.py
+++ b/d-lsg-video-caption_amd/dlsg_amd/hip.py
@@ -170,6 +170,21 @@
                     'dlsg_comm_rehearsal')
 
     def gemm(self, mode, groups, alpha=1.0, flags=0, bias=None, skip_if=None, plan_only=False):
+        a, M, N, nb = self._gemm_args(mode, groups, alpha, flags, bias, skip_if)
+        if plan_only:
+            return int(self.lib.dlsg_gemm_variant(C.byref(a)))
+        e0 = None
+        if self.flop_count is not None:
+            self.flop_count += 2.0 * M * nb * sum(grp_[2].shape[-1] * a.g[i].K for i, grp_ in enumerate(groups))
+        if self.prof is not None:
+            flops = 2.0 * M * nb * sum(grp_[2].shape[-1] * a.g[i].K for i, grp_ in enumerate(groups))
+            if flops >= self.prof_min_flops:
+                e0 = self._prof_begin()
+        self._check(self.lib.dlsg_gemm(C.byref(a), self._stream()), 'dlsg_gemm')
+        if e0 is not None:
+            self._gemm_prof_end(a, mode, groups, M, N, nb, e0, flops)
+
+    def _gemm_args(self, mode, groups, alpha=1.0, flags=0, bias=None, skip_if=None):
         a = abi.dlsg_gemm_args()
         A0, B0, C0 = groups[0][:3]
         batched = A0.dim() == 3
@@ -215,40 +230,32 @@
             g.lda, g.ldb, g.K, g.N = A.stride(-2), B.stride(-2), K, (Ng if Ng != N else 0)
             g.bias = _p(grp_[3]) if len(grp_) > 3 else None
             g.ldc = Cc.stride(-2) if Cc.stride(-2) != a.ldc else 0
-        if plan_only:
-            return int(self.lib.dlsg_gemm_variant(C.byref(a)))
-        e0 = None
-        if self.flop_count is not None:
-            self.flop_count += 2.0 * M * nb * sum(grp_[2].shape[-1] * a.g[i].K for i, grp_ in enumerate(groups))
-        if self.prof is not None:
-            flops = 2.0 * M * nb * sum(grp_[2].shape[-1] * a.g[i].K for i, grp_ in enumerate(groups))
-            if flops >= self.prof_min_flops:
-                e0 = self._prof_begin()
-        self._check(self.lib.dlsg_gemm(C.byref(a), self._stream()), 'dlsg_gemm')
-        if e0 is not None:
-            x3 = bool(a.flags & F_BF16X3)
-            if x3:
-                tiles_l = ((M + 127) // 128) * ((N + 127) // 128) * nb * len(groups)
-                if a.flags & (F_FORCE64 | F_FORCE128):
-                    variant = '64x64' if a.flags & F_FORCE64 else '128x128'
-                elif M <= 64 and mode != GEMM_TN and N >= 64:
-                    variant = 'skinny_64x32'
-                else:
-                    variant = '128x128' if tiles_l >= 1000 else '64x64'
+        return a, M, N, nb
+
+    def _gemm_prof_end(self, a, mode, groups, M, N, nb, e0, flops):
+        x3 = bool(a.flags & F_BF16X3)
+        if x3:
+            tiles_l = ((M + 127) // 128) * ((N + 127) // 128) * nb * len(groups)
+            if a.flags & (F_FORCE64 | F_FORCE128):
+                variant = '64x64' if a.flags & F_FORCE64 else '128x128'
+            elif M <= 64 and mode != GEMM_TN and N >= 64:
+                variant = 'skinny_64x32'
             else:
-                v = self.lib.dlsg_gemm_variant(C.byref(a))
-                variant = {0: '64x64', 1: '128x64', 2: '128x128', 3: 'skinny_64x32' if M <= 64 else 'skinny_128x32', 4: '256x256',
-                           5: '256x128', 6: '256x256+rest', 7: 'streamk_256x256'}[v]
-            ks = sorted(set(a.g[i].K for i in range(len(groups))))
-            ns_ = sorted(set(grp_[2].shape[-1] for grp_ in groups))
-            shape = '%s M=%d N=%s K=%s groups=%d batch=%d' % (('NT', 'NN', 'TN')[mode], M, '/'.join(map(str, ns_)), '/'.join(map(str, ks)),
-                                                              len(groups), nb)
-            ob = 0
-            for i, grp_ in enumerate(groups):
-                Ng = grp_[2].shape[-1]
-                Kg = a.g[i].K
-                ob += 4 * nb * (M * Kg + Ng * Kg + M * Ng * (2 if (a.flags & F_ACCUM) else 1))
-            self._prof_end('gemm_%s_mfma_%s_%s' % ('bf16x3' if x3 else 'f32', variant, ('nt', 'nn', 'tn')[mode]), e0, flops, shape, ob)
+                variant = '128x128' if tiles_l >= 1000 else '64x64'
+        else:
+            v = self.lib.dlsg_gemm_variant(C.byref(a))
+            variant = {0: '64x64', 1: '128x64', 2: '128x128', 3: 'skinny_64x32' if M <= 64 else 'skinny_128x32', 4: '256x256',
+                       5: '256x128', 6: '256x256+rest', 7: 'streamk_256x256'}[v]
+        ks = sorted(set(a.g[i].K for i in range(len(groups))))
+        ns_ = sorted(set(grp_[2].shape[-1] for grp_ in groups))
+        shape = '%s M=%d N=%s K=%s groups=%d batch=%d' % (('NT', 'NN', 'TN')[mode], M, '/'.join(map(str, ns_)), '/'.join(map(str, ks)),
+                                                          len(groups), nb)
+        ob = 0
+        for i, grp_ in enumerate(groups):
+            Ng = grp_[2].shape[-1]
+            Kg = a.g[i].K
+            ob += 4 * nb * (M * Kg + Ng * Kg + M * Ng * (2 if (a.flags & F_ACCUM) else 1))
+        self._prof_end('gemm_%s_mfma_%s_%s' % ('bf16x3' if x3 else 'f32', variant, ('nt', 'nn', 'tn')[mode]), e0, flops, shape, ob)
 
     def slab_reduce(self, slabs, out, bias=None, flags=0):
         S, rows, n = slabs.shape
@@ -550,8 +557,24 @@
         b.dq, b.lddq, b.accum_dq = _p(dq), dq.stride(0), int(accum_dq)
         self._check(self.lib.dlsg_decatt_bwd(C.byref(b), self._stream()), 'dlsg_decatt_bwd')
 
+    cotenant = os.environ.get('DLSG_COTENANT', '1') != '0'
+    COTENANT_MAX_ROWS = 64
+
+    def dec_cotenant_supported(self, B, ntiles):
+        return bool(self.cotenant) and not self.extra_flags and 1 <= B <= self.COTENANT_MAX_ROWS and B + ntiles <= self.device_cus()
+
+    def _co_args(self, co):
+        if co is None:
+            return None
+        mode, groups = co
+        a, M, N, nb = self._gemm_args(mode, groups)
+        a.ws, a.ws_bytes = None, 0
+        if self.flop_count is not None:
+            self.flop_count += 2.0 * M * nb * sum(grp_[2].shape[-1] * a.g[i].K for i, grp_ in enumerate(groups))
+        return C.byref(a)
+
     def dec_mid_fwd(self, slabs, addend, b_ih, b_hh, c_prev, c, h, gates, lnq, qcur, st_q, p_q, site_q, Kp, Vp, lnc, cpre,
-                    ctx, st_c, alpha, p_att, site_att, scale, seed=0, eps=1e-5, kv_div=1):
+                    ctx, st_c, alpha, p_att, site_att, scale, seed=0, eps=1e-5, kv_div=1, co=None):
         a = abi.dlsg_dec_mid_args()
         a.kv_div = kv_div
         assert Kp[0].size(0) * max(1, kv_div) == c.size(0), (Kp[0].shape, c.shape, kv_div)
@@ -572,6 +595,9 @@
         a.B, a.Q, a.H, a.P, a.nstream = c.size(0), c.size(1), Vp[0].size(2), Kp[0].size(1), ns
         a.scale, a.eps = scale, eps
         a.seed, a.seed_ptr = _seed(seed)
+        if co is not None:
+            self._check(self.lib.dlsg_dec_mid_fwd_co(C.byref(a), self._co_args(co), self._stream()), 'dlsg_dec_mid_fwd_co')
+            return
         self._check(self.lib.dlsg_dec_mid_fwd(C.byref(a), self._stream()), 'dlsg_dec_mid_fwd')
 
     DEC_TAIL_SAMPLE_MAX_WEIGHTS = 1 << 21
@@ -579,7 +605,7 @@
     def dec_tail_sample_supported(self, V, D):
         return V * D <= self.DEC_TAIL_SAMPLE_MAX_WEIGHTS
 
-    def dec_tail_fwd(self, slabs, b_ih, b_hh, c_prev, c, hd, gates, ln, dout, st_l, p, site, seed=0, eps=1e-5, sample=None):
+    def dec_tail_fwd(self, slabs, b_ih, b_hh, c_prev, c, hd, gates, ln, dout, st_l, p, site, seed=0, eps=1e-5, sample=None, co=None):
         a = abi.dlsg_dec_tail_args()
         if sample is not None:
             sm = sample
@@ -597,10 +623,13 @@
         a.ln_g, a.ln_b, a.dout, a.st_l, a.p, a.site = _p(ln[0]), _p(ln[1]), _p(dout), _p(st_l), p, site
         a.B, a.D, a.eps = c.size(0), c.size(1), eps
         a.seed, a.seed_ptr = _seed(seed)
+        if co is not None:
+            self._check(self.lib.dlsg_dec_tail_fwd_co(C.byref(a), self._co_args(co), self._stream()), 'dlsg_dec_tail_fwd_co')
+            return
         self._check(self.lib.dlsg_dec_tail_fwd(C.byref(a), self._stream()), 'dlsg_dec_tail_fwd')
 
     def dec_mid_bwd(self, slabs, dlh_rec, cpre, st_c, lnc_g, part_c, dcpre, p_att, site_att, Kp, Vp, alpha, dalpha, ds, qh,
-                    st_q, lnq_g, part_q, p_q, site_q, rec_slabs, gates, c, c_prev, dc, dgates, scale, seed=0):
+                    st_q, lnq_g, part_q, p_q, site_q, rec_slabs, gates, c, c_prev, dc, dgates, scale, seed=0, co=None):
         a = abi.dlsg_dec_mid_bwd_args()
         ns = len(Kp)
         B, Q = c.shape
@@ -626,6 +655,9 @@
         a.gates, a.c, a.c_prev, a.dc, a.dgates = _p(gates), _p(c), _p(c_prev), _p(dc), _p(dgates)
         a.B, a.Q, a.H, a.D, a.P, a.nstream, a.scale = B, Q, H, D, P, ns, scale
         a.seed, a.seed_ptr = _seed(seed)
+        if co is not None:
+            self._check(self.lib.dlsg_dec_mid_bwd_co(C.byref(a), self._co_args(co), self._stream()), 'dlsg_dec_mid_bwd_co')
+            return
         self._check(self.lib.dlsg_dec_mid_bwd(C.byref(a), self._stream()), 'dlsg_dec_mid_bwd')
 
     def decatt_cache_grads(self, alpha, ds, qcur, dcpre, dKp, dVp):
@@ -803,9 +835,14 @@
         a.B, a.H, a.p, a.site = B, H, p, site
         a.seed, a.seed_ptr = _seed(seed)
 
-    def lstm_pw_bwd(self, gates, c, dgates, B, H, **kw):
+    def lstm_pw_bwd(self, gates, c, dgates, B, H, rec=None, **kw):
         a = abi.dlsg_lstm_pw_bwd_args()
         self._pw_bwd_args(a, gates, c, dgates, B, H, **kw)
+        if rec is not None:
+            assert rec.dim() == 3 and rec.shape[1:] == (B, H) and rec.stride(2) == 1
+            self._check(self.lib.dlsg_lstm_pw_bwd_rec(C.byref(a), _p(rec), rec.size(0), i64(rec.stride(0)), i64(rec.stride(1)),
+                                                      self._stream()), 'dlsg_lstm_pw_bwd_rec')
+            return
         self._check(self.lib.dlsg_lstm_pw_bwd(C.byref(a), self._stream()), 'dlsg_lstm_pw_bwd')
 
     def lstm_pw_bwd_multi(self, calls):
diff --git a/include/dlsg.h b/include/dlsg.h
--- a/include/dlsg.h
+++ b/include/dlsg.h
@@ -215,6 +215,7 @@
     uint64_t seed; const uint64_t* seed_ptr;
 } dlsg_dec_mid_args;
 int dlsg_dec_mid_fwd(const dlsg_dec_mid_args* a, void* stream);
+int dlsg_dec_mid_fwd_co(const dlsg_dec_mid_args* a, const dlsg_gemm_args* co, void* stream);
 typedef struct {
     const float* slabs; int32_t nslab; int32_t pad_; int64_t slab_stride;
     const float* b_ih; const float* b_hh;
@@ -232,6 +233,7 @@
     int64_t s_row0; float s_p; float pad2_;
 } dlsg_dec_tail_args;
 int dlsg_dec_tail_fwd(const dlsg_dec_tail_args* a, void* stream);
+int dlsg_dec_tail_fwd_co(const dlsg_dec_tail_args* a, const dlsg_gemm_args* co, void* stream);
 typedef struct {
     const float* slabs; int32_t nslab; int32_t write_rec; int64_t slab_stride;
     float* dlh_rec;
@@ -254,6 +256,7 @@
     uint64_t seed; const uint64_t* seed_ptr;
 } dlsg_dec_mid_bwd_args;
 int dlsg_dec_mid_bwd(const dlsg_dec_mid_bwd_args* a, void* stream);
+int dlsg_dec_mid_bwd_co(const dlsg_dec_mid_bwd_args* a, const dlsg_gemm_args* co, void* stream);
 typedef struct {
     const float* alpha; const float* ds;
     const float* qcur;
@@ -296,6 +299,8 @@
 } dlsg_lstm_pw_bwd_args;
 int dlsg_lstm_pw_bwd(const dlsg_lstm_pw_bwd_args* a, void* stream);
 int dlsg_lstm_pw_bwd_n(const dlsg_lstm_pw_bwd_args* a, int count, void* stream);
+int dlsg_lstm_pw_bwd_rec(const dlsg_lstm_pw_bwd_args* a, const float* rec_slabs, int rec_nslab, int64_t rec_slab_stride, int64_t rec_ld,
+                         void* stream);
 
 int dlsg_mean_rows_fwd(const float* x, float* out, int64_t ldo, int B, int P, int H, void* stream);
 int dlsg_mean_rows_bwd(const float* dout, int64_t lddo, float* dx, int B, int P, int H, int accum, void* stream);
```

Measured after the change: 4908 clips/s. 1.4% lower.
